# wangxb29/PPST

Hardware: AMD Instinct MI355X
Metric: 512x512 portrait swaps/sec/GPU (higher is better)
Workload: dtype bf16x3 (fp32 split into hi+lo bf16, 3 MFMA passes, fp32 accumulate); 1 GPU; simple_swapping 512x512 batch=8 per GPU, generator+encoders forward only (BASELINE configs[1]); image_parallel=1 batch per rank, no data-path collective

## Files before the change

include/ppst_hip.h:

```cpp
#ifndef PPST_HIP_H
#define PPST_HIP_H

#include <stddef.h>
#include <stdint.h>

#ifdef __cplusplus
extern "C" {
#endif

#define PPST_OK 0
#define PPST_EINVAL (-1)
#define PPST_EUNSUPPORTED (-2)
#define PPST_ENULL (-3)

enum { PPST_F32 = 0, PPST_F16 = 1, PPST_BF16 = 2, PPST_F64 = 3  };

enum { PPST_PAD_ZERO = 0, PPST_PAD_REFLECT = 1, PPST_PAD_REPLICATE = 2 };

enum { PPST_ACT_NONE = 0, PPST_ACT_LRELU = 1 , PPST_ACT_PRELU = 2 };

#define PPST_ABI_VERSION 3
int ppst_version(void);

#define PPST_ST_F32 0
#define PPST_ST_F16 1
#define PPST_ST_BF16 2

int ppst_upfirdn2d(const void* x, const void* k, void* y,
                   int major, int in_h, int in_w, int minor, int kh, int kw,
                   int up_x, int up_y, int down_x, int down_y,
                   int pad_x0, int pad_x1, int pad_y0, int pad_y1,
                   int dtype, void* stream);

int ppst_blur_nhwc(const void* x, const void* k, void* y, int B, int in_h, int in_w, int C,
                   int ksize, int pad0, int pad1, int pad_mode, int down, int s2d,
                   const void* in_scale_shift, int in_act, void* stream);
int ppst_blur_nhwc_st(const void* x, const void* k, void* y, int B, int in_h, int in_w, int C,
                      int ksize, int pad0, int pad1, int pad_mode, int down, int s2d,
                      const void* in_scale_shift, int in_act, int st , void* stream);

int ppst_fused_bias_act(const void* x, const void* b, const void* ref, void* y,
                        int64_t n, int step_b, int size_b, int act, int grad,
                        float alpha, float scale, int dtype, void* stream);

int ppst_nchw_to_nhwc(const void* x, void* y, int B, int C, int H, int W, void* stream);
int ppst_nhwc_to_nchw(const void* x, void* y, int B, int C, int H, int W, void* stream);


typedef struct ppst_conv_step {
  int32_t chan_off;
  int32_t dy, dx;
  int32_t new_chunk;
} ppst_conv_step;

int64_t ppst_conv_pack_up9_bytes(int cout, int cin);
int ppst_conv_pack_up9(const void* w, int64_t sn, int64_t sc, int64_t sy, int64_t sx, float scale, int cout, int cin,
                       void* out, void* stream);
int ppst_conv_pack_k64(const void* w, int64_t sn, int64_t sc, int64_t sy, int64_t sx, float scale, int cout, int bn,
                       const int32_t* src_c, const int32_t* src_ky, const int32_t* src_kx, int nsteps, int n_groups,
                       int precision, int dual, void* out, void* stream);
int ppst_conv_pack_dual(const void* w, int64_t sn, int64_t sc, int64_t sy, int64_t sx, float scale, int cout,
                        const int32_t* src_c, const int32_t* src_ky, const int32_t* src_kx, int nsteps, int n_groups,
                        int precision, void* out, void* stream);
int ppst_conv_pack(const void* w, int64_t sn, int64_t sc, int64_t sy, int64_t sx,
                   float scale, int cout, int bn,
                   const int32_t* src_c, const int32_t* src_ky, const int32_t* src_kx,
                   int nsteps, int n_groups, int precision, void* out, void* stream);
typedef struct ppst_pack_job {
  const void* w;
  int64_t sn, sc, sy, sx;
  const int32_t* src_c;
  const int32_t* src_ky;
  const int32_t* src_kx;
  void* out;
  int64_t total;
  int64_t block0;
  float scale;
  int32_t cout, bn, nsteps, n_groups, x3, f16, nblocks;
  int32_t dual;
} ppst_pack_job;
typedef struct ppst_upscale_job {
  const void* w;
  void* out;
  int64_t total, block0;
  float scale;
  int32_t cout, cin, nblocks;
} ppst_upscale_job;
int ppst_pack_job_blocks(int64_t total);
int ppst_conv_pack_batch(const void* jobs, int njobs, int total_blocks, void* stream);
int ppst_upscale_weight_batch(const void* jobs, int njobs, int total_blocks, void* stream);

int ppst_upscale_weight(const void* w, void* out, int cout, int cin, float scale, void* stream);
int ppst_dgrad_s2d_stack_weight(const void* w, void* out, int cout, int cin, void* stream);
int ppst_depth_to_space_st(const void* x, void* y, int B, int th, int tw, int oh, int ow, int C, int st, void* stream);

#define PPST_KSPLIT_SCRATCH_BYTES ((size_t)256 * 512 * 128 * 4)
#define PPST_KSPLIT_FLAG_WORDS 4096

typedef struct ppst_conv_args {
  const void* x;
  const void* wpack;
  const void* steps;
  void* y;
  const void* bias;
  const void* noise;
  const void* prelu;
  void* stats;
  const void* residual;
  float noise_weight;
  float out_scale;
  int32_t B, in_h, in_w, in_ld;
  int32_t out_h, out_w, out_ld, cout;
  int32_t nsteps, n_groups;
  int32_t pad_mode;
  int32_t in_off_y, in_off_x;
  int32_t out_sy, out_sx;
  int32_t act;
  int32_t precision;
  int32_t res_ld;
  int32_t tile_h, tile_w;
  int32_t halo;
  int32_t bn;
  const void* in_scale_shift;
  const void* in_prelu;
  int32_t in_c, in_act;
  int32_t flop_steps;
  int32_t tile_rows;
  int32_t a_slots;
  int32_t early_a;
  int32_t variant;
  int32_t in_presplit;
  int32_t dual_b;
  int32_t io_st;
  int32_t k64;
  const void* in_res;
  int32_t in_res_ld;
  int32_t ksplit;
  const int32_t* ksplit_starts;
  void* ksplit_scratch;
  unsigned* ksplit_flags;
  uint32_t ksplit_epoch;
} ppst_conv_args;

int ppst_conv2d_mfma(const ppst_conv_args* a, void* stream);
int64_t ppst_conv_pack_wino_bytes(int cout, int cin);
int ppst_conv_pack_wino(const void* w, int64_t sn, int64_t sc, int64_t sy, int64_t sx, float scale, int cout, int cin,
                        void* out, void* stream);
int ppst_presplit(const void* x, void* y, int64_t npix, int C, int x_ld, int y_ld, void* stream);
int ppst_has_experiments(void);
int ppst_conv2d_f32(const ppst_conv_args* a, const void* w, int64_t sn, int64_t sc, int64_t sy, int64_t sx, float wscale,
                    const int32_t* src_c, const int32_t* src_ky, const int32_t* src_kx, void* stream);
int ppst_conv_tiles(int tile_h, int tile_w, int tile_rows);

int ppst_conv1x1_small_cin(const void* x, const void* w, const void* bias, void* y,
                           int64_t npix, int cin, int in_ld, int cout, float wscale,
                           int act, void* stream);
int ppst_conv1x1_small_cin_st(const void* x, const void* w, const void* bias, void* y,
                              int64_t npix, int cin, int in_ld, int cout, float wscale,
                              int act, int y_st , void* stream);
int ppst_conv1x1_small_cout(const void* x, const void* w, const void* bias, void* y,
                            int64_t npix, int cin, int cout, float wscale, void* stream);
int ppst_conv1x1_small_cout_st(const void* x, const void* w, const void* bias, void* y,
                               int64_t npix, int cin, int cout, float wscale, int x_st , void* stream);
int ppst_torgb_apply_st(const void* x, const void* scale_shift, const void* res, int res_ld, float out_scale, const void* w,
                        const void* bias, void* y, int B, int H, int W, int cin, float wscale, int x_st, void* stream);

int ppst_in_stats(const void* x, void* partial, int B, int H, int W, int C, int ld,
                  int rep_pad, int* n_partials, void* stream);
int ppst_in_finalize(const void* partial, int n_partials, const void* style,
                     int style_ld ,
                     const void* post_bias ,
                     void* scale_shift , int B, int C, double count,
                     float eps, void* stream);
int ppst_affine_act(const void* x, const void* scale_shift, const void* res,
                    const void* res_scale_shift , void* y,
                    int B, int64_t hw, int C, int x_ld, int res_ld, int y_ld,
                    int act , const void* prelu,
                    float out_scale,
                    int res_up2_w ,
                    void* stream);
int ppst_affine_act_st(const void* x, const void* scale_shift, const void* res, const void* res_scale_shift, void* y,
                       int B, int64_t hw, int C, int x_ld, int res_ld, int y_ld, int act, const void* prelu,
                       float out_scale, int res_up2_w, int x_st, int y_st, void* stream);
int ppst_affine_act_stats(const void* x, const void* scale_shift, const void* res,
                          const void* res_scale_shift, void* y, void* partial,
                          int B, int H, int W, int C, int x_ld, int res_ld, int y_ld,
                          int act, const void* prelu, float out_scale, int rep_pad,
                          int res_up2 , void* stream);
int ppst_upsample_nearest2(const void* x, void* y, int B, int H, int W, int C, void* stream);
int ppst_upsample_nearest2_st(const void* x, void* y, int B, int H, int W, int C, int st, void* stream);

int64_t ppst_gap_gmp_ws(int B, int64_t hw, int C);
int ppst_gap_gmp(const void* x, const void* mask, void* out, void* ws, int B, int H, int W,
                 int C, int ld, void* stream);
int ppst_gap_gmp_st(const void* x, const void* mask, void* out, void* ws, int B, int H, int W,
                    int C, int ld, int x_st, void* stream);
int ppst_avgpool(const void* x, void* y, int B, int H, int W, int C, int x_ld, int f,
                 int y_ld, void* stream);
int ppst_bilinear(const void* x, void* y, int B, int H, int W, int C, int x_ld,
                  int OH, int OW, int y_ld, void* stream);
int ppst_head_tail(const void* x, const void* scale_shift, const void* prelu, void* feat, void* feat1,
                   int B, int H, int W, int C, int x_ld, int feat_ld, int feat1_ld, int P, int D, int act,
                   void* stream);
int ppst_maxpool2(const void* x, void* y, int B, int H, int W, int C, void* stream);

int ppst_linear(const void* x, const void* w, const void* bias, void* y,
                int B, int K, int N, float wscale, float bscale, int relu_in, int act,
                void* stream);
int ppst_l2norm_rows(const void* x, void* y, int B, int K, float eps, int mode, void* stream);
int ppst_lerp(const void* a, const void* b, void* y, int64_t n, float r, void* stream);
int ppst_spatial_modulation(const void* x, const void* scale, const void* bias, void* y,
                            int B, int64_t hw, int C, void* stream);
int ppst_spatial_modulation_st(const void* x, const void* scale, const void* bias, void* y,
                               int B, int64_t hw, int C, int y_st , void* stream);

int ppst_rselfcorr(const void* fea, void* out, int B, int H, int W, int C, int out_ld,
                   void* stream);
int ppst_corr_prep(const void* fea, void* out, int B, int P, int C, int ncenter, void* stream);
int ppst_unfold_rows(const void* x, void* out, int B, int H, int W, int C, int k, void* stream);
int ppst_unfold_rows_bwd(const void* g, void* dx, int B, int H, int W, int C, int k, void* stream);
int ppst_gemm_nt_f32(const void* A, const void* Bm, void* C, int batch, int M, int N, int K,
                     float alpha, void* stream);
int ppst_gemm_nn_f32(const void* A, const void* Bm, void* C, int batch, int M, int N, int K,
                     int ldb, int ldc, void* stream);
int ppst_gemm_nt_split(const void* A, const void* Bm, void* C, int batch, int M, int N, int K,
                       float alpha, int passes, void* stream);
int ppst_gemm_nn_split(const void* A, const void* Bm, void* C, int batch, int M, int N, int K,
                       int ldb, int ldc, int passes, void* stream);
int ppst_softmax_rows(void* x, int64_t rows, int cols, float div, void* stream);
int ppst_unfold_patches(const void* x, void* y, int B, int C, int H, int W, int s, void* stream);
int ppst_fold_patches(const void* x, void* y, int B, int C, int H, int W, int s, void* stream);

int ppst_resample_u8(const void* x, void* y, int B, int in_h, int in_w, int C, int out_size, int horizontal,
                     const void* bounds, const void* coef, int ksize, void* stream);
int ppst_u8_to_tensor(const void* x, void* y, int B, int H, int W, int C, float mean, float stdv, void* stream);

int ppst_tensor2im_u8(const void* x, void* y, int B, int C, int H, int W, void* stream);
int64_t ppst_guided_filter_ws(int B, int H, int W);
int ppst_guided_filter(const void* guide_u8, const void* src_u8, void* out, void* out_u8,
                       int B, int H, int W, int r, float eps, void* work, void* stream);
int ppst_guided_filter_tune(int vs1, int vs2);

int64_t ppst_smooth_local_affine_ws(int B, int H, int W);
int ppst_smooth_local_affine(const void* output, const void* input, void* result, void* model_ws, void* filtered_model,
                             int B, int H, int W, int patch_radius, int filter_radius, float sigma1, float sigma2,
                             void* stream);

int ppst_conv_wgrad_f32(const void* x, const void* dy, const void* steps, const void* chunk_start,
                        void* partial, int B, int in_h, int in_w, int in_ld, int oh, int ow,
                        int dy_ld, int cout, int nsteps, int nchunks, int splits, void* stream);
int ppst_conv_wgrad_bf16x3(const void* x, const void* dy, const void* steps, const void* chunk_start,
                           void* partial, int B, int in_h, int in_w, int in_ld, int oh, int ow,
                           int dy_ld, int cout, int nsteps, int nchunks, int splits, void* stream);
int ppst_conv_wgrad_tr(const void* x, const void* dy, const void* steps, const void* chunk_start, void* partial, void* csum,
                       int B, int in_h, int in_w, int in_ld, int oh, int ow, int dy_ld, int cout, int nsteps, int nchunks,
                       int splits, void* stream);
int ppst_conv_wgrad_tr2(const void* x, const void* dy, const void* steps, const void* chunk_start, void* partial, void* csum,
                        int B, int in_h, int in_w, int in_ld, int oh, int ow, int dy_ld, int cout, int nsteps, int nchunks,
                        int splits, int max_taps, int min_taps, int halo, int passes, void* stream);
int ppst_wgrad_scatter(const void* partial, const void* src_c, const void* src_ky, const void* src_kx,
                       void* dw, int64_t sn, int64_t sc, int64_t sy, int64_t sx, int cout, int nsteps,
                       int splits, float scale, int accumulate, const void* csum, void* db, int csum_rows, int db_accumulate,
                       void* stream);
int64_t ppst_wgrad_small_cin_ws(int64_t npix, int cin, int cout);
int ppst_wgrad_small_cin(const void* x, const void* dy, void* dw, void* ws, int64_t npix, int cin,
                         int in_ld, int cout, float scale, int accumulate, void* stream);
int64_t ppst_colsum_ws(int64_t rows, int C);
int ppst_colsum(const void* x, void* out, void* ws, int64_t rows, int C, int ld, float scale,
                int accumulate, void* stream);
int ppst_linear_wgrad(const void* dy, const void* x, void* dw, int B, int N, int K, float scale,
                      int accumulate, void* stream);
int64_t ppst_linear_dgrad_ws(int B, int N, int K);
int ppst_linear_dgrad(const void* dy, const void* w, void* dx, void* ws, int B, int N, int K, float scale,
                      void* stream);
int ppst_linear_wgrad_fused(const void* dy, const void* x, void* dw, void* db, int B, int N, int K, float scale, float bscale,
                            int accumulate, int b_accumulate, int relu_in, void* stream);
int ppst_linear_dgrad_gate(const void* dy, const void* w, void* dx, void* ws, const void* gate, int B, int N, int K, float scale,
                           void* stream);
int64_t ppst_l1_mean_ws(int64_t n);
int ppst_l1_mean(const void* a, const void* b, void* out, void* ws, int64_t n, float weight, void* stream);
int ppst_rscl_loss(const void* q, const void* k, const void* k0, const void* queue, void* out, void* ws,
                   int n, int n0, int C, int K, float nce_T, void* stream);
int ppst_lsgan(const void* pred, void* loss, void* grad, int n, float target, float weight, void* stream);
int ppst_adam_step(void* p, const void* g, void* m, void* v, int64_t n, float lr, float beta1,
                   float beta2, float eps, int step, void* stream);

int ppst_in_finalize_train(const void* partial, int n_partials, const void* style, int style_ld, const void* post_bias,
                           void* scale_shift, void* mean_rstd, int B, int C, double count, float eps, void* stream);
int ppst_dual_stats(const void* g, const void* y, const void* gate, void* partial, int B, int64_t hw, int C, int g_ld, int y_ld,
                    int gate_ld, int* n_partials, void* stream);
int ppst_in_bwd_finalize(const void* partial, int n_partials, const void* mean_rstd, const void* style, int style_ld, void* coef,
                         void* dstyle, int B, int C, double count, void* stream);
int ppst_in_bwd_apply(const void* g, const void* y, const void* gate, const void* coef, void* dx, int B, int64_t hw, int C, int g_ld,
                      int y_ld, int gate_ld, int dx_ld, int post_gate, void* stream);
int64_t ppst_prelu_bwd_ws(int64_t total_elements);
int ppst_prelu_bwd(const void* g, const void* y, const void* scale_shift, const void* res, const void* prelu, void* gpre, void* ws,
                   int B, int64_t hw, int C, int g_ld, int y_ld, int res_ld, void* stream);
int ppst_sum_partials(const void* partial, void* out, int n, float scale, void* stream);
int ppst_pad2d(const void* x, void* y, int B, int H, int W, int C, int x_ld, int py0, int py1, int px0, int px1, int mode,
               void* stream);
int ppst_pad2d_bwd(const void* dy, void* dx, int B, int H, int W, int C, int py0, int py1, int px0, int px1, int mode, void* stream);
int ppst_bilinear_bwd(const void* dy, void* dx, int B, int H, int W, int C, int dx_ld, int OH, int OW, int dy_ld, void* stream);
int ppst_avgpool_bwd(const void* dy, void* dx, int B, int H, int W, int C, int dx_ld, int f, int dy_ld, void* stream);
int ppst_gap_gmp_bwd(const void* x, const void* mask, const void* v, const void* g, void* dx, void* arg_ws , int B,
                     int64_t hw, int C, int ld, int accumulate, void* stream);
int64_t ppst_gap_gmp_multi_ws(int B, int64_t hw, int C, int heads);
int ppst_gap_gmp_multi(const void* x, const void* masks, void* out, void* ws, int B, int H, int W, int C, int ld, int nm,
                       int with_plain, int x_st, void* stream);
int ppst_gap_gmp_multi_bwd(const void* x, const void* masks, const void* v, const void* g, void* dx, void* arg_ws, int B, int64_t hw,
                           int C, int ld, int nm, int with_plain, int accumulate, int st , void* stream);
int ppst_l2norm_rows_bwd(const void* g, const void* x, void* dx, int B, int K, float eps, int mode, void* stream);
int ppst_softmax_rows_bwd(const void* p, void* g, int64_t rows, int cols, float div, void* stream);
int ppst_corr_prep_bwd(const void* g, const void* x, void* dx, int64_t rows, int C, int ncenter, float eps, void* stream);
int ppst_l1_grad(const void* a, const void* b, void* da, int64_t n, float weight, void* stream);
int ppst_rscl_loss_bwd(const void* q, const void* k, const void* k0, const void* queue, const void* gout, void* dq, int n, int n0,
                       int C, int K, float nce_T, void* stream);
int ppst_rselfcorr_bwd(const void* fea, const void* dout, void* dfea, int B, int H, int W, int C, int dout_ld, void* stream);
int ppst_scale_by(const void* x, const void* s, void* y, int64_t n, void* stream);
int64_t ppst_noise_wgrad_ws(int64_t npix);
int ppst_noise_wgrad(const void* dpre, const void* noise, void* out, void* ws, int64_t npix, int C, int ld, int accumulate, void* stream);
int ppst_upscale_weight_bwd(const void* dw4, void* dw, int cout, int cin, float scale, int accumulate, void* stream);
int ppst_space_to_depth(const void* x, void* y, int B, int H, int W, int C, int x_ld, void* stream);

int ppst_prof_enable(int on);
int ppst_prof_dropped(void);
int ppst_prof_collect(double* ms, int64_t* launches, double* flop);
int ppst_prof_detail(int idx, double* ms, double* flop, int32_t* info);
int ppst_wgrad_flop_steps(int flop_steps);

int ppst_dual_stats_st(const void* g, const void* y, const void* gate, void* partial, int B, int64_t hw, int C, int g_ld, int y_ld,
                       int gate_ld, int* n_partials, int st, void* stream);
int ppst_in_bwd_apply_st(const void* g, const void* y, const void* gate, const void* coef, void* dx, int B, int64_t hw, int C, int g_ld,
                         int y_ld, int gate_ld, int dx_ld, int post_gate, int st, void* stream);
int ppst_pad2d_st(const void* x, void* y, int B, int H, int W, int C, int x_ld, int py0, int py1, int px0, int px1, int mode, int st,
                  void* stream);
int ppst_pad2d_bwd_st(const void* dy, void* dx, int B, int H, int W, int C, int py0, int py1, int px0, int px1, int mode, int st,
                      void* stream);
int ppst_bilinear_bwd_st(const void* dy, void* dx, int B, int H, int W, int C, int dx_ld, int OH, int OW, int dy_ld, int st, void* stream);
int ppst_gap_gmp_bwd_st(const void* x, const void* mask, const void* v, const void* g, void* dx, void* arg_ws, int B, int64_t hw, int C,
                        int ld, int accumulate, int st, void* stream);
int ppst_noise_wgrad_st(const void* dpre, const void* noise, void* out, void* ws, int64_t npix, int C, int ld, int accumulate, int st,
                        void* stream);
int ppst_space_to_depth_st(const void* x, void* y, int B, int H, int W, int C, int x_ld, int st, void* stream);
int ppst_colsum_st(const void* x, void* out, void* ws, int64_t rows, int C, int ld, float scale, int accumulate, int st, void* stream);
int ppst_wgrad_small_cin_st(const void* x, const void* dy, void* dw, void* ws, int64_t npix, int cin, int in_ld, int cout, float scale,
                            int accumulate, int dy_st, void* stream);
int ppst_conv_wgrad_tr2_st(const void* x, const void* dy, const void* steps, const void* chunk_start, void* partial, void* csum, int B,
                           int in_h, int in_w, int in_ld, int oh, int ow, int dy_ld, int cout, int nsteps, int nchunks, int splits,
                           int max_taps, int min_taps, int halo, int passes, int st, void* stream);

#ifdef __cplusplus
}
#endif
#endif
```

ppst_amd/_lib.py:

```python
import ctypes
import os

import torch

HERE = os.path.dirname(os.path.abspath(__file__))
LIB_PATH = os.environ.get("PPST_HIP_LIB") or os.path.join(HERE, "libppst_hip.so")

if not os.path.exists(LIB_PATH):
    raise ImportError(
        "ppst_amd: %s is missing -- build it with `python -m ppst_amd.build` "
        "(hipcc --offload-arch=gfx950). There is no CPU fallback." % LIB_PATH)

lib = ctypes.CDLL(LIB_PATH)

vp, i32, i64, f32, f64 = ctypes.c_void_p, ctypes.c_int, ctypes.c_int64, ctypes.c_float, ctypes.c_double


class PackJob(ctypes.Structure):
    _fields_ = [("w", vp), ("sn", i64), ("sc", i64), ("sy", i64), ("sx", i64), ("src_c", vp), ("src_ky", vp), ("src_kx", vp),
                ("out", vp), ("total", i64), ("block0", i64), ("scale", f32), ("cout", i32), ("bn", i32), ("nsteps", i32),
                ("n_groups", i32), ("x3", i32), ("f16", i32), ("nblocks", i32), ("dual", i32)]


class UpscaleJob(ctypes.Structure):
    _fields_ = [("w", vp), ("out", vp), ("total", i64), ("block0", i64), ("scale", f32), ("cout", i32), ("cin", i32), ("nblocks", i32)]


class ConvArgs(ctypes.Structure):
    _fields_ = [
        ("x", vp), ("wpack", vp), ("steps", vp), ("y", vp), ("bias", vp), ("noise", vp),
        ("prelu", vp), ("stats", vp), ("residual", vp),
        ("noise_weight", f32), ("out_scale", f32),
        ("B", i32), ("in_h", i32), ("in_w", i32), ("in_ld", i32),
        ("out_h", i32), ("out_w", i32), ("out_ld", i32), ("cout", i32),
        ("nsteps", i32), ("n_groups", i32), ("pad_mode", i32),
        ("in_off_y", i32), ("in_off_x", i32), ("out_sy", i32), ("out_sx", i32),
        ("act", i32), ("precision", i32), ("res_ld", i32), ("tile_h", i32), ("tile_w", i32),
        ("halo", i32), ("bn", i32), ("in_scale_shift", vp), ("in_prelu", vp), ("in_c", i32), ("in_act", i32),
        ("flop_steps", i32), ("tile_rows", i32), ("a_slots", i32), ("early_a", i32), ("variant", i32), ("in_presplit", i32), ("dual_b", i32), ("io_st", i32), ("k64", i32),
        ("in_res", vp), ("in_res_ld", i32), ("ksplit", i32), ("ksplit_starts", vp),
        ("ksplit_scratch", vp), ("ksplit_flags", vp), ("ksplit_epoch", ctypes.c_uint32),
    ]


_SIGS = {
    "ppst_version": (i32, []),
    "ppst_guided_filter_tune": (i32, [i32, i32]),
    "ppst_upfirdn2d": (i32, [vp, vp, vp] + [i32] * 14 + [i32, vp]),
    "ppst_blur_nhwc": (i32, [vp, vp, vp] + [i32] * 10 + [vp, i32, vp]),
    "ppst_blur_nhwc_st": (i32, [vp, vp, vp] + [i32] * 10 + [vp, i32, i32, vp]),
    "ppst_fused_bias_act": (i32, [vp, vp, vp, vp, i64, i32, i32, i32, i32, f32, f32, i32, vp]),
    "ppst_nchw_to_nhwc": (i32, [vp, vp, i32, i32, i32, i32, vp]),
    "ppst_nhwc_to_nchw": (i32, [vp, vp, i32, i32, i32, i32, vp]),
    "ppst_conv_pack": (i32, [vp, i64, i64, i64, i64, f32, i32, i32, vp, vp, vp, i32, i32, i32, vp, vp]),
    "ppst_conv_pack_k64": (i32, [vp, i64, i64, i64, i64, f32, i32, i32, vp, vp, vp, i32, i32, i32, i32, vp, vp]),
    "ppst_conv_pack_up9_bytes": (i64, [i32, i32]),
    "ppst_conv_pack_up9": (i32, [vp, i64, i64, i64, i64, f32, i32, i32, vp, vp]),
    "ppst_conv_pack_wino_bytes": (i64, [i32, i32]),
    "ppst_conv_pack_wino": (i32, [vp, i64, i64, i64, i64, f32, i32, i32, vp, vp]),
    "ppst_conv_pack_dual": (i32, [vp, i64, i64, i64, i64, f32, i32, vp, vp, vp, i32, i32, i32, vp, vp]),
    "ppst_upscale_weight": (i32, [vp, vp, i32, i32, f32, vp]),
    "ppst_dgrad_s2d_stack_weight": (i32, [vp, vp, i32, i32, vp]),
    "ppst_depth_to_space_st": (i32, [vp, vp, i32, i32, i32, i32, i32, i32, i32, vp]),
    "ppst_pack_job_blocks": (i32, [i64]),
    "ppst_conv_pack_batch": (i32, [vp, i32, i32, vp]),
    "ppst_upscale_weight_batch": (i32, [vp, i32, i32, vp]),
    "ppst_conv2d_mfma": (i32, [ctypes.POINTER(ConvArgs), vp]),
    "ppst_has_experiments": (i32, []),
    "ppst_presplit": (i32, [vp, vp, i64, i32, i32, i32, vp]),
    "ppst_conv2d_f32": (i32, [ctypes.POINTER(ConvArgs), vp, i64, i64, i64, i64, f32, vp, vp, vp, vp]),
    "ppst_conv_tiles": (i32, [i32, i32, i32]),
    "ppst_conv1x1_small_cin": (i32, [vp, vp, vp, vp, i64, i32, i32, i32, f32, i32, vp]),
    "ppst_conv1x1_small_cin_st": (i32, [vp, vp, vp, vp, i64, i32, i32, i32, f32, i32, i32, vp]),
    "ppst_conv1x1_small_cout": (i32, [vp, vp, vp, vp, i64, i32, i32, f32, vp]),
    "ppst_conv1x1_small_cout_st": (i32, [vp, vp, vp, vp, i64, i32, i32, f32, i32, vp]),
    "ppst_torgb_apply_st": (i32, [vp, vp, vp, i32, f32, vp, vp, vp, i32, i32, i32, i32, f32, i32, vp]),
    "ppst_in_stats": (i32, [vp, vp, i32, i32, i32, i32, i32, i32, ctypes.POINTER(i32), vp]),
    "ppst_in_finalize": (i32, [vp, i32, vp, i32, vp, vp, i32, i32, f64, f32, vp]),
    "ppst_affine_act": (i32, [vp, vp, vp, vp, vp, i32, i64, i32, i32, i32, i32, i32, vp, f32, i32, vp]),
    "ppst_affine_act_st": (i32, [vp, vp, vp, vp, vp, i32, i64, i32, i32, i32, i32, i32, vp, f32, i32, i32, i32, vp]),
    "ppst_affine_act_stats": (i32, [vp, vp, vp, vp, vp, vp, i32, i32, i32, i32, i32, i32, i32, i32, vp, f32, i32, i32, vp]),
    "ppst_upsample_nearest2": (i32, [vp, vp, i32, i32, i32, i32, vp]),
    "ppst_upsample_nearest2_st": (i32, [vp, vp, i32, i32, i32, i32, i32, vp]),
    "ppst_gap_gmp_ws": (i64, [i32, i64, i32]),
    "ppst_gap_gmp": (i32, [vp, vp, vp, vp, i32, i32, i32, i32, i32, vp]),
    "ppst_gap_gmp_st": (i32, [vp, vp, vp, vp, i32, i32, i32, i32, i32, i32, vp]),
    "ppst_avgpool": (i32, [vp, vp, i32, i32, i32, i32, i32, i32, i32, vp]),
    "ppst_bilinear": (i32, [vp, vp, i32, i32, i32, i32, i32, i32, i32, i32, vp]),
    "ppst_head_tail": (i32, [vp, vp, vp, vp, vp] + [i32] * 10 + [vp]),
    "ppst_maxpool2": (i32, [vp, vp, i32, i32, i32, i32, vp]),
    "ppst_linear": (i32, [vp, vp, vp, vp, i32, i32, i32, f32, f32, i32, i32, vp]),
    "ppst_l2norm_rows": (i32, [vp, vp, i32, i32, f32, i32, vp]),
    "ppst_lerp": (i32, [vp, vp, vp, i64, f32, vp]),
    "ppst_spatial_modulation": (i32, [vp, vp, vp, vp, i32, i64, i32, vp]),
    "ppst_spatial_modulation_st": (i32, [vp, vp, vp, vp, i32, i64, i32, i32, vp]),
    "ppst_rselfcorr": (i32, [vp, vp, i32, i32, i32, i32, i32, vp]),
    "ppst_corr_prep": (i32, [vp, vp, i32, i32, i32, i32, vp]),
    "ppst_gemm_nt_f32": (i32, [vp, vp, vp, i32, i32, i32, i32, f32, vp]),
    "ppst_gemm_nn_f32": (i32, [vp, vp, vp, i32, i32, i32, i32, i32, i32, vp]),
    "ppst_unfold_rows": (i32, [vp, vp, i32, i32, i32, i32, i32, vp]),
    "ppst_unfold_rows_bwd": (i32, [vp, vp, i32, i32, i32, i32, i32, vp]),
    "ppst_gemm_nt_split": (i32, [vp, vp, vp, i32, i32, i32, i32, f32, i32, vp]),
    "ppst_gemm_nn_split": (i32, [vp, vp, vp, i32, i32, i32, i32, i32, i32, i32, vp]),
    "ppst_softmax_rows": (i32, [vp, i64, i32, f32, vp]),
    "ppst_unfold_patches": (i32, [vp, vp, i32, i32, i32, i32, i32, vp]),
    "ppst_fold_patches": (i32, [vp, vp, i32, i32, i32, i32, i32, vp]),
    "ppst_tensor2im_u8": (i32, [vp, vp, i32, i32, i32, i32, vp]),
    "ppst_resample_u8": (i32, [vp, vp, i32, i32, i32, i32, i32, i32, vp, vp, i32, vp]),
    "ppst_u8_to_tensor": (i32, [vp, vp, i32, i32, i32, i32, f32, f32, vp]),
    "ppst_guided_filter_ws": (i64, [i32, i32, i32]),
    "ppst_guided_filter": (i32, [vp, vp, vp, vp, i32, i32, i32, i32, f32, vp, vp]),
    "ppst_smooth_local_affine_ws": (i64, [i32, i32, i32]),
    "ppst_smooth_local_affine": (i32, [vp, vp, vp, vp, vp, i32, i32, i32, i32, i32, f32, f32, vp]),
    "ppst_conv_wgrad_f32": (i32, [vp, vp, vp, vp, vp] + [i32] * 11 + [vp]),
    "ppst_conv_wgrad_bf16x3": (i32, [vp, vp, vp, vp, vp] + [i32] * 11 + [vp]),
    "ppst_conv_wgrad_tr": (i32, [vp, vp, vp, vp, vp, vp, i32, i32, i32, i32, i32, i32, i32, i32, i32, i32, i32, vp]),
    "ppst_conv_wgrad_tr2": (i32, [vp, vp, vp, vp, vp, vp, i32, i32, i32, i32, i32, i32, i32, i32, i32, i32, i32, i32, i32, i32, i32, vp]),
    "ppst_wgrad_scatter": (i32, [vp, vp, vp, vp, vp, i64, i64, i64, i64, i32, i32, i32, f32, i32, vp, vp, i32, i32, vp]),
    "ppst_wgrad_small_cin_ws": (i64, [i64, i32, i32]),
    "ppst_wgrad_small_cin": (i32, [vp, vp, vp, vp, i64, i32, i32, i32, f32, i32, vp]),
    "ppst_colsum_ws": (i64, [i64, i32]),
    "ppst_colsum": (i32, [vp, vp, vp, i64, i32, i32, f32, i32, vp]),
    "ppst_linear_wgrad": (i32, [vp, vp, vp, i32, i32, i32, f32, i32, vp]),
    "ppst_linear_dgrad_ws": (i64, [i32, i32, i32]),
    "ppst_linear_dgrad": (i32, [vp, vp, vp, vp, i32, i32, i32, f32, vp]),
    "ppst_linear_wgrad_fused": (i32, [vp, vp, vp, vp, i32, i32, i32, f32, f32, i32, i32, i32, vp]),
    "ppst_linear_dgrad_gate": (i32, [vp, vp, vp, vp, vp, i32, i32, i32, f32, vp]),
    "ppst_lsgan": (i32, [vp, vp, vp, i32, f32, f32, vp]),
    "ppst_l1_mean_ws": (i64, [i64]),
    "ppst_l1_mean": (i32, [vp, vp, vp, vp, i64, f32, vp]),
    "ppst_rscl_loss": (i32, [vp, vp, vp, vp, vp, vp, i32, i32, i32, i32, f32, vp]),
    "ppst_adam_step": (i32, [vp, vp, vp, vp, i64, f32, f32, f32, f32, i32, vp]),
    "ppst_in_finalize_train": (i32, [vp, i32, vp, i32, vp, vp, vp, i32, i32, f64, f32, vp]),
    "ppst_dual_stats": (i32, [vp, vp, vp, vp, i32, i64, i32, i32, i32, i32, ctypes.POINTER(i32), vp]),
    "ppst_in_bwd_finalize": (i32, [vp, i32, vp, vp, i32, vp, vp, i32, i32, f64, vp]),
    "ppst_in_bwd_apply": (i32, [vp, vp, vp, vp, vp, i32, i64, i32, i32, i32, i32, i32, i32, vp]),
    "ppst_prelu_bwd_ws": (i64, [i64]),
    "ppst_prelu_bwd": (i32, [vp, vp, vp, vp, vp, vp, vp, i32, i64, i32, i32, i32, i32, vp]),
    "ppst_sum_partials": (i32, [vp, vp, i32, f32, vp]),
    "ppst_pad2d": (i32, [vp, vp] + [i32] * 10 + [vp]),
    "ppst_pad2d_bwd": (i32, [vp, vp] + [i32] * 9 + [vp]),
    "ppst_bilinear_bwd": (i32, [vp, vp] + [i32] * 8 + [vp]),
    "ppst_avgpool_bwd": (i32, [vp, vp] + [i32] * 7 + [vp]),
    "ppst_gap_gmp_bwd": (i32, [vp, vp, vp, vp, vp, vp, i32, i64, i32, i32, i32, vp]),
    "ppst_gap_gmp_multi_ws": (i64, [i32, i64, i32, i32]),
    "ppst_gap_gmp_multi": (i32, [vp, vp, vp, vp, i32, i32, i32, i32, i32, i32, i32, i32, vp]),
    "ppst_gap_gmp_multi_bwd": (i32, [vp, vp, vp, vp, vp, vp, i32, i64, i32, i32, i32, i32, i32, i32, vp]),
    "ppst_gap_gmp_bwd_st": (i32, [vp, vp, vp, vp, vp, vp, i32, i64, i32, i32, i32, i32, vp]),
    "ppst_dual_stats_st": (i32, [vp, vp, vp, vp, i32, i64, i32, i32, i32, i32, ctypes.POINTER(i32), i32, vp]),
    "ppst_in_bwd_apply_st": (i32, [vp, vp, vp, vp, vp, i32, i64, i32, i32, i32, i32, i32, i32, i32, vp]),
    "ppst_pad2d_st": (i32, [vp, vp] + [i32] * 11 + [vp]),
    "ppst_pad2d_bwd_st": (i32, [vp, vp] + [i32] * 10 + [vp]),
    "ppst_bilinear_bwd_st": (i32, [vp, vp] + [i32] * 9 + [vp]),
    "ppst_noise_wgrad_st": (i32, [vp, vp, vp, vp, i64, i32, i32, i32, i32, vp]),
    "ppst_space_to_depth_st": (i32, [vp, vp, i32, i32, i32, i32, i32, i32, vp]),
    "ppst_colsum_st": (i32, [vp, vp, vp, i64, i32, i32, f32, i32, i32, vp]),
    "ppst_wgrad_small_cin_st": (i32, [vp, vp, vp, vp, i64, i32, i32, i32, f32, i32, i32, vp]),
    "ppst_conv_wgrad_tr2_st": (i32, [vp, vp, vp, vp, vp, vp] + [i32] * 16 + [vp]),
    "ppst_l2norm_rows_bwd": (i32, [vp, vp, vp, i32, i32, f32, i32, vp]),
    "ppst_softmax_rows_bwd": (i32, [vp, vp, i64, i32, f32, vp]),
    "ppst_corr_prep_bwd": (i32, [vp, vp, vp, i64, i32, i32, f32, vp]),
    "ppst_l1_grad": (i32, [vp, vp, vp, i64, f32, vp]),
    "ppst_scale_by": (i32, [vp, vp, vp, i64, vp]),
    "ppst_rscl_loss_bwd": (i32, [vp, vp, vp, vp, vp, vp, i32, i32, i32, i32, f32, vp]),
    "ppst_rselfcorr_bwd": (i32, [vp, vp, vp, i32, i32, i32, i32, i32, vp]),
    "ppst_noise_wgrad_ws": (i64, [i64]),
    "ppst_noise_wgrad": (i32, [vp, vp, vp, vp, i64, i32, i32, i32, vp]),
    "ppst_upscale_weight_bwd": (i32, [vp, vp, i32, i32, f32, i32, vp]),
    "ppst_space_to_depth": (i32, [vp, vp, i32, i32, i32, i32, i32, vp]),
    "ppst_prof_enable": (i32, [i32]),
    "ppst_prof_dropped": (i32, []),
    "ppst_wgrad_flop_steps": (i32, [i32]),
    "ppst_prof_collect": (i32, [ctypes.POINTER(f64), ctypes.POINTER(i64), ctypes.POINTER(f64)]),
    "ppst_prof_detail": (i32, [i32, ctypes.POINTER(f64), ctypes.POINTER(f64), ctypes.POINTER(i32)]),
}

for _name, (_res, _args) in _SIGS.items():
    _fn = getattr(lib, _name)
    _fn.restype = _res
    _fn.argtypes = _args

ABI_VERSION = 3
if lib.ppst_version() != ABI_VERSION:
    raise ImportError("ppst_amd: %s reports ABI revision %d, this binding is written for %d -- rebuild the library "
                      "(python -m ppst_amd.build)" % (LIB_PATH, lib.ppst_version(), ABI_VERSION))

_ERR = {-1: "PPST_EINVAL (bad size / flag combination)", -2: "PPST_EUNSUPPORTED", -3: "PPST_ENULL"}


def check(rc, what):
    if rc != 0:
        raise RuntimeError("%s failed: %s" % (what, _ERR.get(rc, "hipError_t %d" % rc)))


def exported_symbols():
    return sorted(_SIGS)
```

ppst_amd/build.py:

```python
import os
import subprocess
import sys
from concurrent.futures import ThreadPoolExecutor

HERE = os.path.dirname(os.path.abspath(__file__))
CSRC = os.path.join(HERE, "csrc")
OBJ = os.path.join(HERE, "csrc", "_obj")
LIB = os.path.join(HERE, "libppst_hip.so")
EXPERIMENTS = os.environ.get("PPST_EXPERIMENTS") == "1"
SOURCES = ["upfirdn2d.hip", "fused_bias_act.hip", "elementwise.hip", "linear.hip", "conv_mfma.hip", "conv_mfma2.hip", "conv1x1.hip", "conv_wino.hip", "conv_f32.hip",
           "corr.hip", "guided_filter.hip", "train.hip", "train_g.hip", "imageio.hip", "smooth_filter.hip"] + (["conv_ksplit.hip"] if EXPERIMENTS else [])
FLAGS = ["--offload-arch=gfx950", "-O3", "-fPIC", "-std=c++17", "-Wno-unused-result"] + (["-DPPST_EXPERIMENTS"] if EXPERIMENTS else [])
FILE_FLAGS = {"conv_wino.hip": ["-fno-slp-vectorize"]}
MODE_STAMP = os.path.join(HERE, ".libmode")


def _hipcc():
    for c in (os.environ.get("HIPCC"), "/opt/rocm/bin/hipcc", "hipcc"):
        if c and (os.path.isabs(c) and os.path.exists(c) or not os.path.isabs(c)):
            return c
    return "hipcc"


HEADERS = [os.path.join(CSRC, "common.h"), os.path.join(CSRC, "rscl_common.h"), os.path.join(HERE, "..", "include", "ppst_hip.h")]


def _stale(target, deps):
    return not os.path.exists(target) or any(os.path.getmtime(d) > os.path.getmtime(target) for d in deps)


def _mode():
    return "experiments" if EXPERIMENTS else "production"


def _lib_flavour():
    try:
        return open(MODE_STAMP).read().strip()
    except OSError:
        pass
    if not os.path.exists(LIB):
        return None
    try:
        return "experiments" if b"conv_ksplit_kernel" in open(LIB, "rb").read() else "production"
    except OSError:
        return None


def _mode_changed():
    have = _lib_flavour()
    if have is None:
        return os.path.exists(LIB)
    return have != _mode()


def needs_build():
    return (_mode_changed() or _stale(LIB, [os.path.join(CSRC, s) for s in SOURCES] + HEADERS) or
            any(_stale(os.path.join(OBJ, s.replace(".hip", ".o")), [os.path.join(CSRC, s)]) for s in SOURCES if os.path.isdir(OBJ)))


def build(force=False, verbose=True):
    if not force and not needs_build():
        return LIB
    os.makedirs(OBJ, exist_ok=True)
    force = force or _mode_changed()
    hipcc = _hipcc()

    def cc(src):
        obj = os.path.join(OBJ, src.replace(".hip", ".o"))
        if not force and not _stale(obj, [os.path.join(CSRC, src)] + HEADERS):
            return obj
        cmd = [hipcc] + FLAGS + FILE_FLAGS.get(src, []) + ["-c", os.path.join(CSRC, src), "-o", obj]
        r = subprocess.run(cmd, capture_output=True, text=True)
        if r.returncode != 0:
            raise RuntimeError("hipcc failed for %s:\n%s" % (src, r.stderr))
        return obj

    order = sorted(SOURCES, key=lambda f: 0 if f.startswith("conv") else 1)
    with ThreadPoolExecutor(max_workers=8) as ex:
        objs = dict(zip(order, ex.map(cc, order)))
    cmd = [hipcc, "--offload-arch=gfx950", "-shared", "-fPIC", "-o", LIB] + [objs[s_] for s_ in SOURCES]
    r = subprocess.run(cmd, capture_output=True, text=True)
    if r.returncode != 0:
        raise RuntimeError("link failed:\n%s" % r.stderr)
    with open(MODE_STAMP, "w") as f:
        f.write(_mode() + "\n")
    if verbose:
        print("built", LIB, "(%s)" % _mode())
    return LIB


if __name__ == "__main__":
    build(force="--force" in sys.argv)
```

ppst_amd/csrc/conv1x1.hip:

```cpp
#include "common.h"

struct C1Args {
  const float* x;
  const unsigned char* wpack;
  const int4* steps;
  float* y;
  const float* bias;
  const float* noise;
  const float* prelu;
  float* stats;
  const float* residual;
  float noise_weight, out_scale;
  int B, hw, in_ld, out_ld, cout, nsteps, act, res_ld, n_tiles, tiles;
  int in_h, in_w, out_h, out_w, tiles_x, pad_mode;
  const float* in_ss;
  const float* in_prelu;
  int in_c, in_act;
  const float* in_res;
  int in_res_ld;
};

#define C1_GROUP 8
#define C1_BLOB 8192

typedef _Float16 __attribute__((ext_vector_type(8))) c1_half8;
template <int PREC>
__device__ __forceinline__ void c1_cvt(float v, unsigned short& h, unsigned short& l) {
  if (PREC == 0) split_bf16(v, h, l);
  else if (PREC == 3) { h = __builtin_bit_cast(unsigned short, (_Float16)v); l = 0; }
  else { h = f2bf(v); l = 0; }
}
template <int PREC>
__device__ __forceinline__ void c1_cvt8(const float (&v)[8], bf16x8& hi, bf16x8& lo) {
  if (PREC == 3) {
#pragma unroll
    for (int j = 0; j < 8; ++j) {
      unsigned short h, l;
      c1_cvt<PREC>(v[j], h, l);
      hi[j] = (short)h;
      lo[j] = (short)l;
    }
    return;
  }
  uint2 h0, l0 = make_uint2(0u, 0u), h1, l1 = make_uint2(0u, 0u);
  if (PREC == 0) {
    split_bf16x4(make_float4(v[0], v[1], v[2], v[3]), h0, l0);
    split_bf16x4(make_float4(v[4], v[5], v[6], v[7]), h1, l1);
  } else {
    h0 = f2bf_x4(make_float4(v[0], v[1], v[2], v[3]));
    h1 = f2bf_x4(make_float4(v[4], v[5], v[6], v[7]));
  }
  hi = __builtin_bit_cast(bf16x8, make_uint4(h0.x, h0.y, h1.x, h1.y));
  lo = __builtin_bit_cast(bf16x8, make_uint4(l0.x, l0.y, l1.x, l1.y));
}
template <int IOS>
__device__ __forceinline__ void c1_unpack8(float4 r, float (&v)[8]) {
  const float4 a = st_unpack4<IOS>(make_uint2(__float_as_uint(r.x), __float_as_uint(r.y)));
  const float4 b = st_unpack4<IOS>(make_uint2(__float_as_uint(r.z), __float_as_uint(r.w)));
  v[0] = a.x; v[1] = a.y; v[2] = a.z; v[3] = a.w; v[4] = b.x; v[5] = b.y; v[6] = b.z; v[7] = b.w;
}
template <int PREC>
__device__ __forceinline__ f32x4 c1_mfma(bf16x8 bh, bf16x8 bl, bf16x8 xh, bf16x8 xl, f32x4 acc) {
  if (PREC == 0) {
    acc = __builtin_amdgcn_mfma_f32_16x16x32_bf16(bh, xl, acc, 0, 0, 0);
    acc = __builtin_amdgcn_mfma_f32_16x16x32_bf16(bl, xh, acc, 0, 0, 0);
    return __builtin_amdgcn_mfma_f32_16x16x32_bf16(bh, xh, acc, 0, 0, 0);
  }
  if (PREC == 3) return __builtin_amdgcn_mfma_f32_16x16x32_f16(__builtin_bit_cast(c1_half8, bh), __builtin_bit_cast(c1_half8, xh), acc, 0, 0, 0);
  return __builtin_amdgcn_mfma_f32_16x16x32_bf16(bh, xh, acc, 0, 0, 0);
}

__device__ __forceinline__ int c1_pad(int i, int n, int mode) {
  if (mode == PPST_PAD_REFLECT) {
    if (i < 0) i = -i;
    if (i >= n) i = 2 * (n - 1) - i;
  }
  return i < 0 ? 0 : (i >= n ? n - 1 : i);
}

template <int MT, int NT, bool TAPS, bool SPEC = true, int IOS = PPST_ST_F32>
__device__ __forceinline__ void c1_epilogue(const C1Args& a, f32x4 (&acc)[MT][NT], float (&red)[8][NT > 4 ? 128 : 64][2], int b, int mblk,
                                            int ntile, int pbase, int oy0, int ox, int tid, int wave, int r16, int g) {
  const int act = a.act & 0xff;
  const bool res_after = (a.act >> 8) & 1;
  const float slope = (act == PPST_ACT_PRELU && a.prelu) ? a.prelu[0] : 0.f;
  float4 s1[NT], s2[NT];
#pragma unroll
  for (int nt = 0; nt < NT; ++nt) { s1[nt] = make_float4(0.f, 0.f, 0.f, 0.f); s2[nt] = s1[nt]; }
  const int64_t img = (int64_t)b * (TAPS ? a.out_h * a.out_w : a.hw);
  constexpr int ES = IOS == PPST_ST_F32 ? 4 : 2;
  unsigned char* const yb = (unsigned char*)a.y + img * a.out_ld * ES;
  const float* const nzb = a.noise ? a.noise + img : nullptr;
  const unsigned char* const rb = a.residual ? (const unsigned char*)a.residual + img * a.res_ld * ES : nullptr;
  const int nbase = ntile * (NT > 4 ? 128 : 64) + g * 4;
  float nzv[MT];
  float4 bva[NT];
  const __amdgpu_buffer_rsrc_t nrs = __builtin_amdgcn_make_buffer_rsrc((void*)(nzb ? (const void*)nzb : (const void*)yb), 0,
                                                                       nzb ? (TAPS ? a.out_h * a.out_w : a.hw) * 4 : 0, 0x00020000);
#pragma unroll
  for (int mt = 0; mt < MT; ++mt) {
    const int p = pbase + mt * 16 + r16;
    const bool ok = TAPS ? (oy0 + mt < a.out_h && ox < a.out_w) : p < a.hw;
    nzv[mt] = a.noise_weight * __builtin_bit_cast(float, __builtin_amdgcn_raw_buffer_load_b32(
                                   nrs, ok ? (TAPS ? (oy0 + mt) * a.out_w + ox : p) * 4 : (int)0x80000000, 0, 0));
  }
#pragma unroll
  for (int nt = 0; nt < NT; ++nt)
    bva[nt] = __builtin_bit_cast(float4, __builtin_amdgcn_raw_buffer_load_b128(__builtin_amdgcn_make_buffer_rsrc((void*)(a.bias ? (const void*)a.bias : (const void*)a.y), 0, a.bias ? a.cout * 4 : 0, 0x00020000), (nbase + nt * 16) * 4, 0, 0));
  auto epi_passes = [&](auto act_c, auto res_c) {
#pragma clang fp contract(off)
    const int ACT = act_c.value, RES = res_c.value;
#pragma unroll
  for (int mt = 0; mt < MT; ++mt) {
    const int p = pbase + mt * 16 + r16;
    if (TAPS ? (oy0 + mt >= a.out_h || ox >= a.out_w) : p >= a.hw) continue;
    const int pin = TAPS ? (oy0 + mt) * a.out_w + ox : p;
    const int yo = pin * a.out_ld, ro = pin * a.res_ld;
    const float nz = nzv[mt];
#pragma unroll
    for (int nt = 0; nt < NT; ++nt) {
      const int n0 = nbase + nt * 16;
      if (n0 >= a.cout) continue;
      float4 rv = make_float4(0.f, 0.f, 0.f, 0.f);
      const float4 bv = bva[nt];
      if (RES) rv = st_ld4<IOS>(rb, ro + n0);
      float o[4] = {acc[mt][nt][0] + bv.x + nz, acc[mt][nt][1] + bv.y + nz, acc[mt][nt][2] + bv.z + nz, acc[mt][nt][3] + bv.w + nz};
      const float r4[4] = {rv.x, rv.y, rv.z, rv.w};
#pragma unroll
      for (int c = 0; c < 4; ++c) {
        float t = o[c];
        if (RES == 1) t += r4[c];
        if (ACT == PPST_ACT_LRELU) t = (t > 0.f ? t : t * 0.2f) * 1.41421356237309515f;
        else if (ACT == PPST_ACT_PRELU) t = t >= 0.f ? t : t * slope;
        if (RES == 2) t += r4[c];
        o[c] = t * a.out_scale;
      }
      st_st4<IOS>(yb, yo + n0, make_float4(o[0], o[1], o[2], o[3]));
      s1[nt].x += o[0]; s1[nt].y += o[1]; s1[nt].z += o[2]; s1[nt].w += o[3];
      s2[nt].x += o[0] * o[0]; s2[nt].y += o[1] * o[1]; s2[nt].z += o[2] * o[2]; s2[nt].w += o[3] * o[3];
    }
  }
  };
  {
    const int resm = a.residual ? (res_after ? 2 : 1) : 0;
#define EPI_GO(A_)                                                                                    \
  do {                                                                                                \
    if (resm == 0) epi_passes(EpiC<A_>{}, EpiC<0>{});                                                 \
    else if (resm == 1) epi_passes(EpiC<A_>{}, EpiC<1>{});                                            \
    else epi_passes(EpiC<A_>{}, EpiC<2>{});                                                           \
  } while (0)
    if (!SPEC) epi_passes(EpiR{act}, EpiR{resm});
    else if (act == PPST_ACT_LRELU) EPI_GO(PPST_ACT_LRELU);
    else if (act == PPST_ACT_PRELU) EPI_GO(PPST_ACT_PRELU);
    else EPI_GO(PPST_ACT_NONE);
#undef EPI_GO
  }
  if (a.stats) {
#pragma unroll
    for (int nt = 0; nt < NT; ++nt) {
      float4 u = s1[nt], w = s2[nt];
      float* uv[8] = {&u.x, &u.y, &u.z, &u.w, &w.x, &w.y, &w.z, &w.w};
#pragma unroll
      for (int q = 0; q < 8; ++q) {
        float t = *uv[q];
        t += __builtin_bit_cast(float, __builtin_amdgcn_mov_dpp(__builtin_bit_cast(int, t), 0xB1, 0xf, 0xf, true));
        t += __builtin_bit_cast(float, __builtin_amdgcn_mov_dpp(__builtin_bit_cast(int, t), 0x4E, 0xf, 0xf, true));
        t += __builtin_bit_cast(float, __builtin_amdgcn_mov_dpp(__builtin_bit_cast(int, t), 0x141, 0xf, 0xf, true));
        t += __builtin_bit_cast(float, __builtin_amdgcn_mov_dpp(__builtin_bit_cast(int, t), 0x140, 0xf, 0xf, true));
        *uv[q] = t;
      }
      if (r16 == 0) {
        float* r = &red[wave][nt * 16 + g * 4][0];
        r[0] = u.x; r[1] = w.x; r[2] = u.y; r[3] = w.y; r[4] = u.z; r[5] = w.z; r[6] = u.w; r[7] = w.w;
      }
    }
    __syncthreads();
    if (tid < (NT > 4 ? 128 : 64)) {
      const int n = ntile * (NT > 4 ? 128 : 64) + tid;
      if (n < a.cout) {
        float t0 = 0.f, t1 = 0.f;
#pragma unroll
        for (int wv = 0; wv < 8; ++wv) { t0 += red[wv][tid][0]; t1 += red[wv][tid][1]; }
        float* o = a.stats + (((int64_t)b * a.tiles + mblk) * a.cout + n) * 2;
        o[0] = t0;
        o[1] = t1;
      }
    }
  }
}

template <int INSS, bool TAPS = false, int NT_ = 4, int PREC = 0, int IOS = PPST_ST_F32>
__global__ __launch_bounds__(512, 4) void conv1x1_stream_kernel(C1Args a) {
  constexpr int MT = 2, NT = NT_;
  constexpr bool X3 = PREC == 0;
  static_assert(IOS == PPST_ST_F32 || IOS == (PREC == 3 ? PPST_ST_F16 : PREC == 1 ? PPST_ST_BF16 : -1), "half storage: single-pass modes");
  constexpr int ES = IOS == PPST_ST_F32 ? 4 : 2;
  constexpr int BLOB1 = X3 ? C1_BLOB : C1_BLOB / 2;
  __shared__ uint4 sB[C1_GROUP * BLOB1 / 16];
  __shared__ float red[8][64][2];

  const int nwg = gridDim.x;
  int wid;
  {
    int id = blockIdx.x, q = nwg >> 3, r = nwg & 7, xcd = id & 7;
    wid = (xcd < r ? xcd * (q + 1) : r * (q + 1) + (xcd - r) * q) + (id >> 3);
  }
  const int ntile = wid % a.n_tiles;
  int mblk = wid / a.n_tiles;
  const int b = mblk / a.tiles;
  mblk -= b * a.tiles;
  const int tid = threadIdx.x, lane = tid & 63, wave = __builtin_amdgcn_readfirstlane(tid >> 6);
  const int r16 = lane & 15, g = lane >> 4;
  const int pbase = mblk * 256 + wave * 32;
  const int tyi = TAPS ? mblk / a.tiles_x : 0, txi = TAPS ? mblk - tyi * a.tiles_x : 0;
  const int oy0 = tyi * 16 + wave * 2, ox = txi * 16 + r16;
  const unsigned char* xb = (const unsigned char*)a.x + (int64_t)b * (TAPS ? a.in_h * a.in_w : a.hw) * a.in_ld * ES;
  const unsigned char* wblob = a.wpack + (int64_t)ntile * a.nsteps * BLOB1;
#if defined(__HIP_DEVICE_COMPILE__)
  typedef const __attribute__((address_space(4))) int4* StepPtr;
#else
  typedef const int4* StepPtr;
#endif
  StepPtr steps = (StepPtr)a.steps;

  int64_t aoff[MT];
  bool pok[MT];
#pragma unroll
  for (int mt = 0; mt < MT; ++mt) {
    const int p = pbase + mt * 16 + r16;
    pok[mt] = TAPS ? true : p < a.hw;
    aoff[mt] = TAPS ? 0 : (int64_t)(pok[mt] ? p : 0) * a.in_ld + g * 8;
  }
  const float in_slope = (INSS && a.in_act == PPST_ACT_PRELU && a.in_prelu) ? a.in_prelu[0] : 0.f;
  auto in_act = [&](float t) -> float {
    if (a.in_act == PPST_ACT_LRELU) return (t > 0.f ? t : t * 0.2f) * 1.41421356237309515f;
    if (a.in_act == PPST_ACT_PRELU) return t >= 0.f ? t : t * in_slope;
    return t;
  };

  f32x4 acc[MT][NT];
#pragma unroll
  for (int i = 0; i < MT; ++i)
#pragma unroll
    for (int j = 0; j < NT; ++j) acc[i][j] = (f32x4){0.f, 0.f, 0.f, 0.f};

  float4 raw[MT][2], ss[4];
  float4 rres[INSS == 2 ? MT : 1][2];
  auto a_load = [&](int4 d) {
    const int chan = d.x;
    if (TAPS) {
      int ix = ox + d.z;
      bool xok = ix >= 0 && ix < a.in_w;
      ix = c1_pad(ix, a.in_w, a.pad_mode);
#pragma unroll
      for (int mt = 0; mt < MT; ++mt) {
        int iy = oy0 + mt + d.y;
        const bool yok = iy >= 0 && iy < a.in_h;
        iy = c1_pad(iy, a.in_h, a.pad_mode);
        pok[mt] = a.pad_mode != PPST_PAD_ZERO || (xok && yok);
        aoff[mt] = ((int64_t)iy * a.in_w + ix) * a.in_ld + g * 8;
      }
    }
#pragma unroll
    for (int mt = 0; mt < MT; ++mt) {
      const float4* p = (const float4*)(xb + (aoff[mt] + chan) * ES);
      raw[mt][0] = p[0];
      if (IOS == PPST_ST_F32) raw[mt][1] = p[1];
      if (INSS == 2) {
        const int pp = pbase + mt * 16 + r16;
        const float4* q = (const float4*)(a.in_res + ((int64_t)b * a.hw + (pok[mt] ? pp : 0)) * a.in_res_ld + g * 8 + chan);
        rres[mt][0] = q[0];
        rres[mt][1] = q[1];
      }
    }
    if (INSS) {
      const float4* q = (const float4*)(a.in_ss + ((int64_t)b * a.in_c + chan + g * 8) * 2);
      ss[0] = q[0]; ss[1] = q[1]; ss[2] = q[2]; ss[3] = q[3];
    }
  };
  a_load(steps[0]);

  for (int s0 = 0; s0 < a.nsteps; s0 += C1_GROUP) {
    const int ng = a.nsteps - s0 < C1_GROUP ? a.nsteps - s0 : C1_GROUP;
    if (s0) __syncthreads();
    for (int i = tid; i < ng * (BLOB1 / 16); i += 512) sB[i] = ((const uint4*)(wblob + (int64_t)s0 * BLOB1))[i];
    __syncthreads();
    for (int sl = 0; sl < ng; ++sl) {
      const int s = s0 + sl;
      bf16x8 ah[MT], al[MT];
      bool vok[MT];
#pragma unroll
      for (int mt = 0; mt < MT; ++mt) vok[mt] = pok[mt];
#pragma unroll
      for (int mt = 0; mt < MT; ++mt) {
        if (IOS != PPST_ST_F32 && !INSS) {
          const float4 z = vok[mt] ? raw[mt][0] : make_float4(0.f, 0.f, 0.f, 0.f);
          ah[mt] = __builtin_bit_cast(bf16x8, z);
          al[mt] = ah[mt];
          continue;
        }
        float v[8] = {raw[mt][0].x, raw[mt][0].y, raw[mt][0].z, raw[mt][0].w, raw[mt][1].x, raw[mt][1].y, raw[mt][1].z, raw[mt][1].w};
        if (IOS != PPST_ST_F32) c1_unpack8<IOS>(raw[mt][0], v);
        if (INSS) {
          const float sc[8] = {ss[0].x, ss[0].z, ss[1].x, ss[1].z, ss[2].x, ss[2].z, ss[3].x, ss[3].z};
          const float sh[8] = {ss[0].y, ss[0].w, ss[1].y, ss[1].w, ss[2].y, ss[2].w, ss[3].y, ss[3].w};
#pragma unroll
          for (int j = 0; j < 8; ++j) {
            float t = sc[j] * v[j] + sh[j];
            if (INSS == 2) {
              const float4 r4 = rres[mt][j >> 2];
              t += (j & 3) == 0 ? r4.x : (j & 3) == 1 ? r4.y : (j & 3) == 2 ? r4.z : r4.w;
            }
            v[j] = in_act(t);
          }
        }
#pragma unroll
        for (int j = 0; j < 8; ++j)
          if (!vok[mt]) v[j] = 0.f;
        c1_cvt8<PREC>(v, ah[mt], al[mt]);
      }
      if (s + 1 < a.nsteps) a_load(steps[s + 1]);
      const unsigned char* bs = (const unsigned char*)sB + sl * BLOB1 + g * 1024 + r16 * 16;
#pragma unroll
      for (int nt = 0; nt < NT; ++nt) {
        const bf16x8 bh = *(const bf16x8*)(bs + nt * 256);
        bf16x8 bl = bh;
        if (X3) bl = *(const bf16x8*)(bs + nt * 256 + 4096);
#pragma unroll
        for (int mt = 0; mt < MT; ++mt) acc[mt][nt] = c1_mfma<PREC>(bh, bl, ah[mt], al[mt], acc[mt][nt]);
      }
    }
  }

  c1_epilogue<MT, NT, TAPS, X3, IOS>(a, acc, red, b, mblk, ntile, pbase, oy0, ox, tid, wave, r16, g);
}

#define C3_GROUP 9
template <int CTRL>
__device__ __forceinline__ bf16x8 c3_shift(bf16x8 edge, bf16x8 centre) {
  typedef int __attribute__((ext_vector_type(4))) i4;
  const i4 e = __builtin_bit_cast(i4, edge), c = __builtin_bit_cast(i4, centre);
  i4 r;
#pragma unroll
  for (int i = 0; i < 4; ++i) r[i] = __builtin_amdgcn_update_dpp(e[i], c[i], CTRL, 0xf, 0xf, false);
  return __builtin_bit_cast(bf16x8, r);
}

template <bool INSS, int NT_, int PREC = 0, int IOS = PPST_ST_F32>
__global__ __launch_bounds__(512, NT_ > 4 ? 2 : 4) void conv3x3_direct_kernel(C1Args a) {
  constexpr int MT = 2, NT = NT_;
  constexpr bool X3 = PREC == 0;
  static_assert(IOS == PPST_ST_F32 || IOS == (PREC == 3 ? PPST_ST_F16 : PREC == 1 ? PPST_ST_BF16 : -1), "half storage: single-pass modes");
  constexpr int ES = IOS == PPST_ST_F32 ? 4 : 2;
  constexpr int PSTR = (NT > 4 ? 128 : 64) * 16;
  constexpr int BLOB = (X3 ? 8 : 4) * PSTR;
  __shared__ uint4 sB[C3_GROUP * BLOB / 16];
  __shared__ float red[8][NT > 4 ? 128 : 64][2];
  const int tid = threadIdx.x, lane = tid & 63, wave = __builtin_amdgcn_readfirstlane(tid >> 6);
  const int r16 = lane & 15, g = lane >> 4;
  const int total = a.B * a.tiles * a.n_tiles;
  const int per = (total + (int)gridDim.x - 1) / (int)gridDim.x;
  const int w_beg = blockIdx.x * per, w_end = w_beg + per < total ? w_beg + per : total;
  const int nchunks = a.nsteps / 9;
  const bool keep_b = nchunks == 1 && a.n_tiles == 1;
  for (int wid = w_beg; wid < w_end; ++wid) {
  const int ntile = wid % a.n_tiles;
  int mblk = wid / a.n_tiles;
  const int b = mblk / a.tiles;
  mblk -= b * a.tiles;
  const int tyi = mblk / a.tiles_x, txi = mblk - tyi * a.tiles_x;
  const int oy0 = tyi * 16 + wave * 2, ox = txi * 16 + r16;
  const unsigned char* xb = (const unsigned char*)a.x + (int64_t)b * a.in_h * a.in_w * a.in_ld * ES;
  const unsigned char* wblob = a.wpack + (int64_t)ntile * a.nsteps * BLOB;
  if (wid > w_beg) __syncthreads();
#if defined(__HIP_DEVICE_COMPILE__)
  typedef const __attribute__((address_space(4))) int4* StepPtr;
#else
  typedef const int4* StepPtr;
#endif
  StepPtr steps = (StepPtr)a.steps;
  const float in_slope = (INSS && a.in_act == PPST_ACT_PRELU && a.in_prelu) ? a.in_prelu[0] : 0.f;
  auto in_act = [&](float t) -> float {
    if (a.in_act == PPST_ACT_LRELU) return (t > 0.f ? t : t * 0.2f) * 1.41421356237309515f;
    if (a.in_act == PPST_ACT_PRELU) return t >= 0.f ? t : t * in_slope;
    return t;
  };
  const int xe_raw = r16 == 0 ? ox - 1 : (r16 == 15 ? ox + 1 : ox);
  const bool cx_ok = ox < a.in_w, ex_ok = xe_raw >= 0 && xe_raw < a.in_w;
  const int cx = c1_pad(ox, a.in_w, a.pad_mode), ex = c1_pad(xe_raw, a.in_w, a.pad_mode);

  f32x4 acc[MT][NT];
#pragma unroll
  for (int i = 0; i < MT; ++i)
#pragma unroll
    for (int j = 0; j < NT; ++j) acc[i][j] = (f32x4){0.f, 0.f, 0.f, 0.f};

  float4 rawc[2], rawe[2], ss[4];
  bool okc = false, oke = false;
  auto row_load = [&](int chan, int r) {
    int iy = oy0 - 1 + r;
    const bool yok = iy >= 0 && iy < a.in_h;
    iy = c1_pad(iy, a.in_h, a.pad_mode);
    okc = a.pad_mode != PPST_PAD_ZERO || (yok && cx_ok);
    oke = a.pad_mode != PPST_PAD_ZERO || (yok && ex_ok);
    const float4* pc = (const float4*)(xb + (((int64_t)iy * a.in_w + cx) * a.in_ld + chan + g * 8) * ES);
    const float4* pe = (const float4*)(xb + (((int64_t)iy * a.in_w + ex) * a.in_ld + chan + g * 8) * ES);
    rawc[0] = pc[0];
    rawe[0] = pe[0];
    if (IOS == PPST_ST_F32) { rawc[1] = pc[1]; rawe[1] = pe[1]; }
  };
  auto ss_load = [&](int chan) {
    if (INSS) {
      const float4* q = (const float4*)(a.in_ss + ((int64_t)b * a.in_c + chan + g * 8) * 2);
      ss[0] = q[0]; ss[1] = q[1]; ss[2] = q[2]; ss[3] = q[3];
    }
  };
  auto convert = [&](const float4 (&raw)[2], bool ok, bf16x8& hi, bf16x8& lo) {
    if (IOS != PPST_ST_F32 && !INSS) {
      hi = __builtin_bit_cast(bf16x8, ok ? raw[0] : make_float4(0.f, 0.f, 0.f, 0.f));
      lo = hi;
      return;
    }
    float v[8] = {raw[0].x, raw[0].y, raw[0].z, raw[0].w, raw[1].x, raw[1].y, raw[1].z, raw[1].w};
    if (IOS != PPST_ST_F32) c1_unpack8<IOS>(raw[0], v);
    if (INSS) {
      const float sc[8] = {ss[0].x, ss[0].z, ss[1].x, ss[1].z, ss[2].x, ss[2].z, ss[3].x, ss[3].z};
      const float sh[8] = {ss[0].y, ss[0].w, ss[1].y, ss[1].w, ss[2].y, ss[2].w, ss[3].y, ss[3].w};
#pragma unroll
      for (int j = 0; j < 8; ++j) v[j] = in_act(sc[j] * v[j] + sh[j]);
    }
#pragma unroll
    for (int j = 0; j < 8; ++j)
      if (!ok) v[j] = 0.f;
    c1_cvt8<PREC>(v, hi, lo);
  };

  int chan = steps[0].x;
  ss_load(chan);
  row_load(chan, 0);
  for (int c = 0; c < nchunks; ++c) {
    if (!keep_b || wid == w_beg) {
      if (c) __syncthreads();
      for (int i = tid; i < C3_GROUP * (BLOB / 16); i += 512) sB[i] = ((const uint4*)(wblob + (int64_t)c * C3_GROUP * BLOB))[i];
      __syncthreads();
    }
    const int chan_next = c + 1 < nchunks ? steps[(c + 1) * 9].x : chan;
#pragma unroll
    for (int r = 0; r < 4; ++r) {
      bf16x8 ch, cl, eh, el;
      convert(rawc, okc, ch, cl);
      convert(rawe, oke, eh, el);
      if (r < 3) row_load(chan, r + 1);
      else if (c + 1 < nchunks) { ss_load(chan_next); row_load(chan_next, 0); }
#pragma unroll
      for (int dxi = 0; dxi < 3; ++dxi) {
        const bf16x8 fh = dxi == 0 ? c3_shift<0x111>(eh, ch) : (dxi == 1 ? ch : c3_shift<0x101>(eh, ch));
        const bf16x8 fl = dxi == 0 ? c3_shift<0x111>(el, cl) : (dxi == 1 ? cl : c3_shift<0x101>(el, cl));
#pragma unroll
        for (int mt = 0; mt < MT; ++mt) {
          const int dyi = r - mt;
          if (dyi < 0 || dyi > 2) continue;
          const unsigned char* bs = (const unsigned char*)sB + (dyi * 3 + dxi) * BLOB + g * PSTR + r16 * 16;
#pragma unroll
          for (int nt = 0; nt < NT; ++nt) {
            const bf16x8 bh = *(const bf16x8*)(bs + nt * 256);
            bf16x8 bl = bh;
            if (X3) bl = *(const bf16x8*)(bs + nt * 256 + 4 * PSTR);
            acc[mt][nt] = c1_mfma<PREC>(bh, bl, fh, fl, acc[mt][nt]);
          }
        }
        __builtin_amdgcn_sched_barrier(0);
      }
    }
    chan = chan_next;
  }
  c1_epilogue<MT, NT, true, (X3 && NT <= 4), IOS>(a, acc, red, b, mblk, ntile, 0, oy0, ox, tid, wave, r16, g);
  }
}

static inline int64_t blocks_of(const ppst_conv_args* a, int tiles, int n_tiles) { return (int64_t)a->B * tiles * n_tiles; }
int ppst_conv1x1_stream_launch(const ppst_conv_args* a, int n_tiles, int tiles, hipStream_t st) {
  C1Args k;
  k.x = (const float*)a->x; k.wpack = (const unsigned char*)a->wpack; k.steps = (const int4*)a->steps; k.y = (float*)a->y;
  k.bias = (const float*)a->bias; k.noise = (const float*)a->noise; k.prelu = (const float*)a->prelu;
  k.stats = (float*)a->stats; k.residual = (const float*)a->residual;
  k.noise_weight = a->noise_weight; k.out_scale = a->out_scale;
  k.B = a->B; k.hw = a->out_h * a->out_w; k.in_ld = a->in_ld; k.out_ld = a->out_ld; k.cout = a->cout; k.nsteps = a->nsteps;
  k.act = a->act; k.res_ld = a->res_ld; k.n_tiles = n_tiles; k.tiles = tiles;
  k.in_ss = (const float*)a->in_scale_shift; k.in_prelu = (const float*)a->in_prelu; k.in_c = a->in_c; k.in_act = a->in_act;
  k.in_res = (const float*)a->in_res; k.in_res_ld = a->in_res_ld;
  if ((int64_t)tiles * 256 < k.hw) return PPST_EINVAL;
  if (k.in_res) {
    PPST_LAUNCH((conv1x1_stream_kernel<2, false, 4, 0, PPST_ST_F32>), dim3((unsigned)blocks_of(a, tiles, n_tiles)), dim3(512), 0, st, k);
    return PPST_LAUNCH_CHECK();
  }
  const int64_t blocks = (int64_t)a->B * tiles * n_tiles;
  if (blocks > 0x7fffffff) return PPST_EINVAL;
#define LS(PREC_, IOS_)                                                                                               \
  do {                                                                                                                \
    if (k.in_ss) PPST_LAUNCH((conv1x1_stream_kernel<1, false, 4, PREC_, IOS_>), dim3((unsigned)blocks), dim3(512), 0, st, k);   \
    else PPST_LAUNCH((conv1x1_stream_kernel<0, false, 4, PREC_, IOS_>), dim3((unsigned)blocks), dim3(512), 0, st, k);          \
  } while (0)
  if (a->precision == 1) { if (a->io_st) LS(1, PPST_ST_BF16); else LS(1, PPST_ST_F32); }
  else if (a->precision == 3) { if (a->io_st) LS(3, PPST_ST_F16); else LS(3, PPST_ST_F32); }
  else LS(0, PPST_ST_F32);
#undef LS
  return PPST_LAUNCH_CHECK();
}

int ppst_conv_direct_launch(const ppst_conv_args* a, int n_tiles, int tiles_y, int tiles_x, hipStream_t st) {
  C1Args k;
  k.x = (const float*)a->x; k.wpack = (const unsigned char*)a->wpack; k.steps = (const int4*)a->steps; k.y = (float*)a->y;
  k.bias = (const float*)a->bias; k.noise = (const float*)a->noise; k.prelu = (const float*)a->prelu;
  k.stats = (float*)a->stats; k.residual = (const float*)a->residual;
  k.noise_weight = a->noise_weight; k.out_scale = a->out_scale;
  k.B = a->B; k.hw = a->out_h * a->out_w; k.in_ld = a->in_ld; k.out_ld = a->out_ld; k.cout = a->cout; k.nsteps = a->nsteps;
  k.act = a->act; k.res_ld = a->res_ld; k.n_tiles = n_tiles; k.tiles = tiles_y * tiles_x;
  k.in_ss = (const float*)a->in_scale_shift; k.in_prelu = (const float*)a->in_prelu; k.in_c = a->in_c; k.in_act = a->in_act;
  k.in_h = a->in_h; k.in_w = a->in_w; k.out_h = a->out_h; k.out_w = a->out_w; k.tiles_x = tiles_x; k.pad_mode = a->pad_mode;
  const int64_t blocks = (int64_t)a->B * k.tiles * n_tiles;
  if (blocks > 0x7fffffff) return PPST_EINVAL;
  const bool nt2 = a->cout <= 32;
#define LD(INSS_, PREC_, IOS_)                                                                                       \
  do {                                                                                                               \
    if (nt2) PPST_LAUNCH((conv1x1_stream_kernel<INSS_, true, 2, PREC_, IOS_>), dim3((unsigned)blocks), dim3(512), 0, st, k);       \
    else PPST_LAUNCH((conv1x1_stream_kernel<INSS_, true, 4, PREC_, IOS_>), dim3((unsigned)blocks), dim3(512), 0, st, k);           \
  } while (0)
#define LDP(PREC_, IOS_) do { if (k.in_ss) LD(1, PREC_, IOS_); else LD(0, PREC_, IOS_); } while (0)
  if (a->precision == 1) { if (a->io_st) LDP(1, PPST_ST_BF16); else LDP(1, PPST_ST_F32); }
  else if (a->precision == 3) { if (a->io_st) LDP(3, PPST_ST_F16); else LDP(3, PPST_ST_F32); }
  else LDP(0, PPST_ST_F32);
#undef LDP
#undef LD
  return PPST_LAUNCH_CHECK();
}

int ppst_conv3x3_direct_launch(const ppst_conv_args* a, int n_tiles, int tiles_y, int tiles_x, hipStream_t st) {
  if (a->nsteps % 9) return PPST_EINVAL;
  C1Args k;
  k.x = (const float*)a->x; k.wpack = (const unsigned char*)a->wpack; k.steps = (const int4*)a->steps; k.y = (float*)a->y;
  k.bias = (const float*)a->bias; k.noise = (const float*)a->noise; k.prelu = (const float*)a->prelu;
  k.stats = (float*)a->stats; k.residual = (const float*)a->residual;
  k.noise_weight = a->noise_weight; k.out_scale = a->out_scale;
  k.B = a->B; k.hw = a->out_h * a->out_w; k.in_ld = a->in_ld; k.out_ld = a->out_ld; k.cout = a->cout; k.nsteps = a->nsteps;
  k.act = a->act; k.res_ld = a->res_ld; k.n_tiles = n_tiles; k.tiles = tiles_y * tiles_x;
  k.in_ss = (const float*)a->in_scale_shift; k.in_prelu = (const float*)a->in_prelu; k.in_c = a->in_c; k.in_act = a->in_act;
  k.in_h = a->in_h; k.in_w = a->in_w; k.out_h = a->out_h; k.out_w = a->out_w; k.tiles_x = tiles_x; k.pad_mode = a->pad_mode;
  int64_t blocks = (int64_t)a->B * k.tiles * n_tiles;
  if (blocks > 0x7fffffff) return PPST_EINVAL;
  if (a->nsteps == 9 && n_tiles == 1 && blocks > 512) blocks = 512;
  const bool nt2 = a->cout <= 32, nt8 = a->bn == 128;
#define LD3(INSS_, PREC_, IOS_)                                                                                      \
  do {                                                                                                               \
    if (nt8 && PREC_ == 0) PPST_LAUNCH((conv3x3_direct_kernel<INSS_, 8, 0>), dim3((unsigned)blocks), dim3(512), 0, st, k);   \
    else if (nt8) return PPST_EUNSUPPORTED;                                                                          \
    else if (nt2) PPST_LAUNCH((conv3x3_direct_kernel<INSS_, 2, PREC_, IOS_>), dim3((unsigned)blocks), dim3(512), 0, st, k); \
    else PPST_LAUNCH((conv3x3_direct_kernel<INSS_, 4, PREC_, IOS_>), dim3((unsigned)blocks), dim3(512), 0, st, k);          \
  } while (0)
#define LD3P(PREC_, IOS_) do { if (k.in_ss) LD3(true, PREC_, IOS_); else LD3(false, PREC_, IOS_); } while (0)
  if (a->precision == 1) { if (a->io_st) LD3P(1, PPST_ST_BF16); else LD3P(1, PPST_ST_F32); }
  else if (a->precision == 3) { if (a->io_st) LD3P(3, PPST_ST_F16); else LD3P(3, PPST_ST_F32); }
  else LD3P(0, PPST_ST_F32);
#undef LD3P
#undef LD3
  return PPST_LAUNCH_CHECK();
}
```

ppst_amd/networks/base_network.py:

```python
import math

import torch
from torch import nn

from .. import ops, weights

SQRT2 = math.sqrt(2.0)
INV_SQRT2 = 1.0 / SQRT2


class _Node(nn.Module):
    """parameter container (no behaviour)."""


def to_nhwc(x):
    if x.dim() != 4:
        raise RuntimeError("expected a 4-D NCHW tensor")
    v = x.permute(0, 2, 3, 1)
    if v.is_contiguous():
        ops._chk(v, "input")
        return v
    return ops.nchw_to_nhwc(x)


def as_nchw(x_nhwc):
    return x_nhwc.permute(0, 3, 1, 2)


class BaseNetwork(nn.Module):
    prefix = ""

    @staticmethod
    def modify_commandline_options(parser, is_train):
        return parser

    def __init__(self, opt=None, size=512, seed=0):
        super().__init__()
        self.opt = opt
        self._flat = {}
        self._cache = {}
        specs = [s for s in weights.param_specs(size=size) if s[0].startswith(self.prefix)]
        for name, shape, kind, aux in specs:
            parts = name[len(self.prefix):].split(".")
            node = self
            for part in parts[:-1]:
                if part not in node._modules:
                    node.add_module(part, _Node())
                node = node._modules[part]
            t = weights._draw(name, shape, kind, aux, seed, 0.0, 0.0)
            if kind in (weights.BLUR3, weights.BLUR4, weights.UP4):
                node.register_buffer(parts[-1], t)
            else:
                node.register_parameter(parts[-1], nn.Parameter(t, requires_grad=False))

    def p(self, name):
        t = self._flat.get(name)
        if t is None:
            node = self
            parts = name.split(".")
            for part in parts[:-1]:
                node = node._modules[part]
            t = node._parameters.get(parts[-1])
            if t is None:
                t = node._buffers[parts[-1]]
            self._flat[name] = t
        return t

    def _apply(self, fn, *a, **k):
        self._flat.clear()
        self._cache.clear()
        return super()._apply(fn, *a, **k)

    def load_state_dict(self, *a, **k):
        self._flat.clear()
        self._cache.clear()
        return super().load_state_dict(*a, **k)

    def cached(self, key, params, build):
        ver = tuple((id(t), t._version, t.data_ptr()) for t in params) + (ops.PRECISION["value"],)
        hit = self._cache.get(key)
        if hit is not None and hit[0] == ver:
            return hit[1]
        val = build()
        self._cache[key] = (ver, val)
        return val

    def plan(self, wname, kind="conv", scale=1.0):
        w = self.p(wname)
        return self.cached(("plan", wname, kind), [w], lambda: ops.ConvPlan(w, kind=kind, scale=scale))

    def refresh_plans(self):
        plans, keep = [], {}
        for key, (ver, val) in self._cache.items():
            if isinstance(key, tuple) and key and key[0] == "plan" and isinstance(val, ops.ConvPlan) and val.precision != 2 \
                    and val.wparam.data_ptr() == self.p(key[1]).data_ptr():
                plans.append(val)
                keep[key] = (ver, val)
        self._cache.clear()
        if not plans:
            return
        sig = tuple((id(pl), tuple(sorted(map(str, pl._packs)))) for pl in plans)
        hit = self.__dict__.get("_repack")
        if hit is not None and hit[0] == sig:
            ops.run_repack(hit[1])
        else:
            self.__dict__["_repack"] = (sig, ops.repack_plans(plans), plans)
        self._cache.update(keep)

    def print_architecture(self, verbose=False):
        n = sum(p.numel() for p in self.parameters())
        print("[Network %s] Total number of parameters : %.3f M" % (type(self).__name__, n / 1e6))

    def from_rgb(self, x, p, out_dtype=torch.float32):
        w = self.p(p + "Conv.weight")
        return ops.conv1x1_small_cin(x, w, self.p(p + "Act.bias"), 1.0 / math.sqrt(w.shape[1]), ops.ACT_LRELU, out_dtype=out_dtype)

    def _norm_act(self, y, st, count, act_bias=None, act=ops.ACT_NONE, **kw):
        ss = ops.in_finalize(st, count, post_bias=act_bias)
        return ops.affine_act(y, ss, act=act, **kw), ss

    def res_block(self, x, p, blur_pad_mode, norm):
        B, H, W, cin = x.shape
        k = self.p(p + "conv2.Blur.kernel")
        ks = k.shape[0]
        w1, w2, ws = self.p(p + "conv1.Conv.weight"), self.p(p + "conv2.Conv.weight"), self.p(p + "skip.Conv.weight")
        sc1 = 1.0 / math.sqrt(cin * 9)
        scs = 1.0 / math.sqrt(cin)
        conv_pad = ops.PAD_REFLECT if blur_pad_mode == ops.PAD_REFLECT else ops.PAD_ZERO
        pad_c = (ks - 2) + 2
        pad_s = (ks - 2) + 0
        xs, _ = ops.blur_nhwc(x, self.p(p + "skip.Blur.kernel"), (pad_s + 1) // 2, pad_s // 2, ops.PAD_ZERO, down=2)
        if not norm:
            y1 = self.plan(p + "conv1.Conv.weight", scale=sc1)(x, bias=self.p(p + "conv1.Act.bias"), act=ops.ACT_LRELU,
                                                                pad_mode=conv_pad)
            skip = self.plan(p + "skip.Conv.weight", scale=scs)(xs)
            xb, bhw = ops.blur_nhwc(y1, k, (pad_c + 1) // 2, pad_c // 2, blur_pad_mode, s2d=True)
            ohw = ((bhw[0] - 3) // 2 + 1, (bhw[1] - 3) // 2 + 1)
            return self.plan(p + "conv2.Conv.weight", "s2d", sc1)(
                xb, bias=self.p(p + "conv2.Act.bias"), act=ops.ACT_LRELU, residual=skip, res_after_act=True,
                out_scale=INV_SQRT2, out_hw=ohw)
        y1, st1 = self.plan(p + "conv1.Conv.weight", scale=sc1)(x, stats=True, pad_mode=conv_pad)
        ss1 = ops.in_finalize(st1, H * W, post_bias=self.p(p + "conv1.Act.bias"))
        ys, sts = self.plan(p + "skip.Conv.weight", scale=scs)(xs, stats=True)
        xb, bhw = ops.blur_nhwc(y1, k, (pad_c + 1) // 2, pad_c // 2, blur_pad_mode, s2d=True, in_ss=ss1, in_act=ops.ACT_LRELU)
        ohw = ((bhw[0] - 3) // 2 + 1, (bhw[1] - 3) // 2 + 1)
        y2, st2 = self.plan(p + "conv2.Conv.weight", "s2d", sc1)(xb, stats=True, out_hw=ohw)
        cnt = ohw[0] * ohw[1]
        ss_s = ops.in_finalize(sts, cnt)
        ss2 = ops.in_finalize(st2, cnt, post_bias=self.p(p + "conv2.Act.bias"))
        return ops.affine_act(y2, ss2, res=ys, res_scale_shift=ss_s, act=ops.ACT_LRELU, out_scale=INV_SQRT2)
```

ppst_amd/ops.py:

```python
import ctypes
import math
import os
import threading

import torch

from . import _lib
from ._lib import lib, check

PAD_ZERO, PAD_REFLECT, PAD_REPLICATE = 0, 1, 2
ACT_NONE, ACT_LRELU, ACT_PRELU = 0, 1, 2
RES_BEFORE_ACT = 1 << 8

PRECISION = {"value": 0}
TILE_ROWS = {"value": 16}
CONV_VARIANT = {"value": 2}
DUAL_CONVT = {"value": True, "min_blocks": 32}
UP9 = {"value": True, "min_blocks": 64, "min_fill": 0.85}
DIRECT_MAX = {"cout": 64, "nsteps": 40, "cout3x3": 64}
WGRAD_SPLIT = {"blocks": 1024, "min_tiles": 4}
WGRAD_X3 = {"value": True}
STREAM_1X1 = {"value": True}
KSPLIT = {"value": os.environ.get("PPST_KSPLIT", "1") != "0", "max_blocks": 256, "min_steps": 16, "variants": (0, 2, 10)}
KSPLIT_SCRATCH_BYTES = 256 * 512 * 128 * 4
KSPLIT_FLAG_WORDS = 4096
KSPLIT_128 = {"value": False, "min_blocks": 32}
TALL_TILE_128 = {"value": False, "min_blocks": 32}
TALL_TILE_SINGLE = {"value": True, "min_blocks": 64}
K64 = {"value": True}
TILE24_128 = {"value": False, "min_blocks": 32, "max_waste": 0.04}
TWO_BLOCK_128 = {"value": False}
TWO_BLOCK_8ROW = {"value": False, "min_blocks": 64}
BATCH_AWARE = {"value": False, "fill": 192}


class batch_aware:

    def __enter__(self):
        self.prev = BATCH_AWARE["value"]
        BATCH_AWARE["value"] = True

    def __exit__(self, *exc):
        BATCH_AWARE["value"] = self.prev
WINO = {"value": True, "min_blocks": 16, "fill": 0, "ksplit_fill": 64}
FUSE_TAIL = {"value": os.environ.get("PPST_FUSE_TAIL", "1") != "0", "torgb": os.environ.get("PPST_FUSE_TORGB", "0") == "1"}
FAT_MIN_BLOCKS = 32


EXPERIMENTS = bool(lib.ppst_has_experiments())


def _need_experiments(what):
    if not EXPERIMENTS:
        raise RuntimeError("%s is an experiment kernel: rebuild the library with PPST_EXPERIMENTS=1 (python -m ppst_amd.build)" % what)


def set_precision(p):
    assert p in (0, 1, 2, 3, 4)
    if p == 4:
        _need_experiments("precision 4 (two-pass fp16)")
    PRECISION["value"] = p


_raw_stream = getattr(torch._C, "_cuda_getCurrentRawStream", None)
_cur_device = getattr(torch._C, "_cuda_getDevice", None)


def _stream():
    if _raw_stream is not None and _cur_device is not None:
        return ctypes.c_void_p(_raw_stream(_cur_device()))
    return ctypes.c_void_p(torch.cuda.current_stream().cuda_stream)


def _chk(t, name="tensor"):
    if t is None:
        return
    if not isinstance(t, torch.Tensor) or not t.is_cuda:
        raise RuntimeError("%s must be a CUDA (HIP) tensor" % name)
    if t.dtype != torch.float32:
        raise RuntimeError("%s must be float32, got %s" % (name, t.dtype))


def _p(t):
    return None if t is None else ctypes.c_void_p(t.data_ptr())


_ST = {torch.float32: 0, torch.float16: 1, torch.bfloat16: 2}
HALF_STORE = {"value": os.environ.get("PPST_HALF_STORE", "1") != "0"}


def act_dtype():
    if HALF_STORE["value"] and not torch.is_grad_enabled():
        return {1: torch.bfloat16, 3: torch.float16}.get(PRECISION["value"], torch.float32)
    return torch.float32


TRAIN_HALF = {"value": os.environ.get("PPST_TRAIN_HALF", "1") != "0"}


def train_dtype():
    return torch.bfloat16 if (TRAIN_HALF["value"] and PRECISION["value"] == 1) else torch.float32


def _chk_act(t, name="activation"):
    if t is None:
        return
    if not isinstance(t, torch.Tensor) or not t.is_cuda:
        raise RuntimeError("%s must be a CUDA (HIP) tensor" % name)
    if t.dtype not in _ST:
        raise RuntimeError("%s must be float32, float16 or bfloat16, got %s" % (name, t.dtype))


def _nhwc_ld(t, name="activation", half_ok=False):
    if half_ok:
        _chk_act(t, name)
    else:
        _chk(t, name)
    B, H, W, C = t.shape
    ld = t.stride(2)
    if t.stride(3) != 1 or t.stride(1) != W * ld or (B > 1 and t.stride(0) != H * W * ld):
        raise RuntimeError("%s must be NHWC-contiguous (or a channel slice of one)" % name)
    return ld


def empty_nhwc(B, H, W, C, like):
    return torch.empty((B, H, W, C), device=like.device, dtype=torch.float32)


def nchw_to_nhwc(x):
    _chk(x, "x")
    x = x.contiguous()
    B, C, H, W = x.shape
    y = torch.empty((B, H, W, C), device=x.device, dtype=torch.float32)
    check(lib.ppst_nchw_to_nhwc(_p(x), _p(y), B, C, H, W, _stream()), "ppst_nchw_to_nhwc")
    return y


def nhwc_to_nchw(x):
    ld = _nhwc_ld(x)
    B, H, W, C = x.shape
    if ld != C:
        raise RuntimeError("nhwc_to_nchw needs a dense tensor")
    y = torch.empty((B, C, H, W), device=x.device, dtype=torch.float32)
    check(lib.ppst_nhwc_to_nchw(_p(x), _p(y), B, C, H, W, _stream()), "ppst_nhwc_to_nchw")
    return y


_DT_F64 = 3


def _chk_op(t, name):
    if t is None:
        return
    if not isinstance(t, torch.Tensor) or not t.is_cuda:
        raise RuntimeError("%s must be a CUDA (HIP) tensor" % name)
    if t.dtype not in _ST and t.dtype != torch.float64:
        raise RuntimeError("%s must be float32, float16, bfloat16 or float64, got %s" % (name, t.dtype))


def upfirdn2d_raw(x4, kernel, up_x, up_y, down_x, down_y, px0, px1, py0, py1):
    _chk_op(x4, "input")
    _chk_op(kernel, "kernel")
    x4 = x4.contiguous()
    f64 = x4.dtype == torch.float64
    kernel = (kernel.double() if f64 else kernel.float()).contiguous()
    major, in_h, in_w, minor = x4.shape
    kh, kw = kernel.shape
    out_h = (in_h * up_y + py0 + py1 - kh + down_y) // down_y
    out_w = (in_w * up_x + px0 + px1 - kw + down_x) // down_x
    y = torch.empty((major, out_h, out_w, minor), device=x4.device, dtype=x4.dtype)
    check(lib.ppst_upfirdn2d(_p(x4), _p(kernel), _p(y), major, in_h, in_w, minor, kh, kw, up_x, up_y, down_x, down_y,
                             px0, px1, py0, py1, _DT_F64 if f64 else _ST[x4.dtype], _stream()), "ppst_upfirdn2d")
    return y


def blur_nhwc(x, kernel, pad0, pad1, pad_mode=PAD_ZERO, down=1, s2d=False, in_ss=None, in_act=ACT_NONE):
    ld = _nhwc_ld(x, half_ok=True)
    B, H, W, C = x.shape
    if ld != C:
        raise RuntimeError("blur_nhwc needs a dense tensor")
    _chk(kernel, "kernel")
    ks = kernel.shape[0]
    oh = (H + pad0 + pad1 - ks + down) // down
    ow = (W + pad0 + pad1 - ks + down) // down
    if s2d:
        y = torch.empty((B, (oh + 1) // 2, (ow + 1) // 2, 4 * C), device=x.device, dtype=x.dtype)
    else:
        y = torch.empty((B, oh, ow, C), device=x.device, dtype=x.dtype)
    _chk(in_ss, "in_ss")
    check(lib.ppst_blur_nhwc_st(_p(x), _p(kernel.contiguous()), _p(y), B, H, W, C, ks, pad0, pad1, pad_mode, down,
                                1 if s2d else 0, _p(in_ss), in_act, _ST[x.dtype], _stream()), "ppst_blur_nhwc")
    return y, (oh, ow)


def fused_bias_act_raw(x, b, ref, act, grad, alpha, scale):
    _chk_op(x, "input")
    x = x.contiguous()
    b = None if (b is None or b.numel() == 0) else b.to(x.dtype).contiguous()
    ref = None if (ref is None or ref.numel() == 0) else ref.to(x.dtype).contiguous()
    _chk_op(b, "bias")
    _chk_op(ref, "refer")
    y = torch.empty_like(x)
    step_b = 1
    for i in range(2, x.dim()):
        step_b *= x.size(i)
    size_b = b.numel() if b is not None else 1
    check(lib.ppst_fused_bias_act(_p(x), _p(b), _p(ref), _p(y), x.numel(), step_b, size_b, act, grad, float(alpha),
                                  float(scale), _DT_F64 if x.dtype == torch.float64 else _ST[x.dtype], _stream()), "ppst_fused_bias_act")
    return y


class ConvPlan:

    _GEOMETRY = {}
    _GEOM_ATTRS = ("kind", "cout", "cin", "k", "bn", "n_groups", "halo", "src", "max_chan", "wstrides", "nsteps", "flop_steps",
                   "early_a", "ksplit_ok", "chunk_starts0", "chunk_starts0_k64", "steps", "src_dev", "chunk_start", "chunks_per_group", "w4_shape", "max_chunk_steps",
                   "min_chunk_steps", "full_cover", "steps_dual", "src_dual", "steps_up9", "steps_k64", "src_k64", "steps_dual_k64",
                   "src_dual_k64")

    def __init__(self, weight, kind="conv", scale=1.0, chan_base=0, precision=None):
        _chk(weight, "weight")
        w = weight.detach().contiguous()
        gkey = (kind, tuple(w.shape), int(chan_base), str(w.device))
        geom = ConvPlan._GEOMETRY.get(gkey)
        if geom is None:
            self._build(w, kind, scale, chan_base, precision)
            ConvPlan._GEOMETRY[gkey] = {a: getattr(self, a) for a in ConvPlan._GEOM_ATTRS if hasattr(self, a)}
            return
        self.__dict__.update(geom)
        self.precision = PRECISION["value"] if precision is None else precision
        self.wparam, self.up_scale = w, float(scale)
        cout, cin, k, _ = w.shape
        if kind in ("convT", "dgradT"):
            wsrc = torch.empty((cin, cout, 4, 4), device=w.device, dtype=torch.float32)
            check(lib.ppst_upscale_weight(_p(w), _p(wsrc), cout, cin, float(scale), _stream()), "ppst_upscale_weight")
            if kind == "dgradT":
                self.fwd_scale = float(scale)
            scale = 1.0
        elif kind == "dgrad":
            wsrc = w.view(-1)[k * k - 1:]
        elif kind == "dgrad_s2ds":
            wsrc = torch.empty((4 * cin, cout, 2, 2), device=w.device, dtype=torch.float32)
            check(lib.ppst_dgrad_s2d_stack_weight(_p(w), _p(wsrc), cout, cin, _stream()), "ppst_dgrad_s2d_stack_weight")
        else:
            wsrc = w
        self.scale = float(scale)
        self.wsrc = wsrc
        if self.precision == 2:
            self.wpack = None
            return
        self._packs = {}
        self.wpack = self.pack_for(self.bn)

    def _build(self, w, kind, scale, chan_base, precision):
        self.kind = kind
        self.wparam, self.up_scale = w, float(scale)
        self.precision = PRECISION["value"] if precision is None else precision
        cout, cin, k, _ = w.shape
        assert cin % 32 == 0, "fused conv needs Cin % 32 == 0 (got %d)" % cin
        self.cout, self.cin, self.k = cout, cin, k
        self.bn = 128 if cout >= 128 else 64
        steps, src = [], []
        nchunk = cin // 32
        if kind == "conv":
            assert k in (1, 3)
            self.n_groups = 1
            self.halo = 0 if k == 1 else 1
            for c in range(nchunk):
                first = True
                for ky in range(k):
                    for kx in range(k):
                        steps.append((chan_base + 32 * c, ky - k // 2, kx - k // 2, 1 if first else 0))
                        src.append((32 * c, ky, kx))
                        first = False
            sn, sc, sy, sx = cin * k * k, k * k, k, 1
            wsrc = w
        elif kind == "s2d":
            assert k == 3
            self.n_groups = 1
            self.halo = 1
            for py in range(2):
                for px in range(2):
                    for c in range(nchunk):
                        first = True
                        for ey in range(2):
                            for ex in range(2):
                                ky, kx = 2 * ey + py, 2 * ex + px
                                if ky > 2 or kx > 2:
                                    continue
                                steps.append(((py * 2 + px) * cin + 32 * c, ey, ex, 1 if first else 0))
                                src.append((32 * c, ky, kx))
                                first = False
                        if py == 1 and px == 1:
                            steps.append(((py * 2 + px) * cin + 32 * c, 0, 0, 0))
                            src.append((-1, 0, 0))
            sn, sc, sy, sx = cin * 9, 9, 3, 1
            wsrc = w
        elif kind == "convT":
            assert k == 3
            self.n_groups = 4
            self.halo = 1
            wsrc = torch.empty((cin, cout, 4, 4), device=w.device, dtype=torch.float32)
            check(lib.ppst_upscale_weight(_p(w), _p(wsrc), cout, cin, float(scale), _stream()), "ppst_upscale_weight")
            scale = 1.0
            taps = {0: [(-1, 3), (0, 1)], 1: [(0, 2), (1, 0)]}
            for a in range(2):
                for b in range(2):
                    for c in range(nchunk):
                        first = True
                        for dy, ky in taps[a]:
                            for dx, kx in taps[b]:
                                steps.append((chan_base + 32 * c, dy, dx, 1 if first else 0))
                                src.append((32 * c, ky, kx))
                                first = False
            sn, sc, sy, sx = 16, cout * 16, 4, 1
            if cout % 128 == 0 and chan_base % 1 == 0:
                dsteps, dsrc = [], []
                for a in range(2):
                    for c in range(nchunk):
                        first = True
                        for dy, ky in taps[a]:
                            for j in range(2):
                                (dx0, kx0), (dx1, kx1) = taps[0][j], taps[1][j]
                                dsteps.append((chan_base + 32 * c, dy, (dx0 + 1) | ((dx1 + 1) << 8), 1 if first else 0))
                                dsrc.append((32 * c, ky, kx0 | (kx1 << 8)))
                                first = False
                self._dual_tmp = (dsteps, dsrc)
            if cout % 64 == 0:
                self._up9_tmp = [(chan_base + 32 * c, dy, dx, 1 if (dy, dx) == (0, 0) else 0)
                                 for c in range(nchunk) for dy, dx in ((0, 0), (-1, 0), (0, -1), (-1, -1))]
        elif kind == "dgrad":
            assert k in (1, 3)
            self.n_groups = 1
            self.halo = 0 if k == 1 else 1
            nchunk = cout // 32
            assert cout % 32 == 0
            for c in range(nchunk):
                first = True
                for ky in range(k):
                    for kx in range(k):
                        steps.append((32 * c, ky - k // 2, kx - k // 2, 1 if first else 0))
                        src.append((32 * c, ky, kx))
                        first = False
            wsrc = w.view(-1)[k * k - 1:]
            sn, sc, sy, sx = k * k, cin * k * k, -k, -1
            self.cout, self.cin = cin, cout
            cout, cin = cin, cout
            self.bn = 128 if cout >= 128 else 64
        elif kind == "dgrad_s2d":
            assert k == 3 and cout % 32 == 0
            self.n_groups = 4
            self.halo = 1
            taps = {0: [(0, 0), (-1, 2)], 1: [(0, 1)]}
            for py in range(2):
                for px in range(2):
                    for c in range(cout // 32):
                        tl = [(dy, dx, ky, kx) for dy, ky in taps[py] for dx, kx in taps[px]]
                        for i in range(4):
                            if i < len(tl):
                                dy, dx, ky, kx = tl[i]
                                steps.append((32 * c, dy, dx, 1 if i == 0 else 0))
                                src.append((32 * c, ky, kx))
                            else:
                                steps.append((32 * c, 0, 0, 0))
                                src.append((-1, 0, 0))
            wsrc = w
            sn, sc, sy, sx = 9, cin * 9, 3, 1
            self.cout, self.cin = cin, cout
            cout, cin = cin, cout
            self.bn = 128 if cout >= 128 else 64
        elif kind == "dgrad_s2ds":
            assert k == 3 and cout % 32 == 0
            self.n_groups = 1
            self.halo = 1
            for c in range(cout // 32):
                for i, (ty, tx) in enumerate(((0, 0), (0, 1), (1, 0), (1, 1))):
                    steps.append((32 * c, -ty, -tx, 1 if i == 0 else 0))
                    src.append((32 * c, ty, tx))
            wsrc = torch.empty((4 * cin, cout, 2, 2), device=w.device, dtype=torch.float32)
            check(lib.ppst_dgrad_s2d_stack_weight(_p(w), _p(wsrc), cout, cin, _stream()), "ppst_dgrad_s2d_stack_weight")
            sn, sc, sy, sx = cout * 4, 4, 2, 1
            self.cout, self.cin = 4 * cin, cout
            cout, cin = 4 * cin, cout
            self.bn = 128 if cout >= 128 else 64
        elif kind == "dgradT":
            assert k == 3 and cout % 32 == 0
            self.n_groups = 1
            self.halo = 1
            wsrc = torch.empty((cin, cout, 4, 4), device=w.device, dtype=torch.float32)
            check(lib.ppst_upscale_weight(_p(w), _p(wsrc), cout, cin, float(scale), _stream()), "ppst_upscale_weight")
            self.fwd_scale = float(scale)
            scale = 1.0
            taps = {0: [(0, 1), (1, 3)], 1: [(-1, 0), (0, 2)]}
            for py in range(2):
                for px in range(2):
                    for c in range(cout // 32):
                        first = True
                        for dqy, ky in taps[py]:
                            for dqx, kx in taps[px]:
                                steps.append(((py * 2 + px) * cout + 32 * c, dqy, dqx, 1 if first else 0))
                                src.append((32 * c, ky, kx))
                                first = False
            sn, sc, sy, sx = cout * 16, 16, 4, 1
            self.w4_shape = (cin, cout, 4, 4)
            self.cout, self.cin = cin, cout
            cout, cin = cin, cout
            self.bn = 128 if cout >= 128 else 64
        else:
            raise ValueError(kind)
        self.src = src
        self.max_chan = max(t[0] for t in steps)
        self.wstrides = (sn, sc, sy, sx)
        self.nsteps = len(steps) // self.n_groups
        self.flop_steps = sum(1 for t in src if t[0] >= 0) // self.n_groups
        live = [tuple(t[:3]) for t in src if t[0] >= 0]
        target = math.prod(self.w4_shape) if kind == "dgradT" else w.numel()
        self.full_cover = bool(self.n_groups == 1 and len(set(live)) == len(live) and len(live) * 32 * cout == target)
        dev = w.device
        ns_ = self.nsteps

        def encode(steps_):
            enc, chunk_idx = [], -1
            for i, (c_, dy_, dx_, f_) in enumerate(steps_):
                if i % ns_ == 0:
                    chunk_idx = -1
                chunk_idx += 1 if f_ else 0
                nxt = steps_[i + 1] if (i + 1) % ns_ != 0 else None
                w_ = f_ | ((2 | (nxt[0] << 8)) if (nxt is not None and nxt[3]) else 0) | ((chunk_idx & 1) << 2)
                enc.append((c_, dy_, dx_, w_))
            return enc
        enc = encode(steps)
        starts = [i for i, t in enumerate(steps) if t[3] == 1] + [len(steps)]
        lens = [b_ - a_ for a_, b_ in zip(starts[:-1], starts[1:])]
        self.chunk_starts0 = [i for i in starts if i < ns_] + [ns_]
        self.chunk_starts0_k64 = None
        self.early_a = 1 if (min(lens) >= 2 and ns_ >= 3) else 0
        self.max_chunk_steps = max(lens)
        self.min_chunk_steps = min(lens)
        self.ksplit_ok = bool(self.early_a and all(l_ >= 3 or (a_ % ns_) % 2 == 0 for a_, l_ in zip(starts[:-1], lens)))
        self.steps = torch.tensor(enc + [(0, 0, 0, 0)] * 4, dtype=torch.int32, device=dev).contiguous()
        self.steps_dual = self.src_dual = None
        dual = self.__dict__.pop("_dual_tmp", None)
        if dual is not None:
            self.steps_dual = torch.tensor(encode(dual[0]) + [(0, 0, 0, 0)] * 4, dtype=torch.int32, device=dev).contiguous()
            sd_ = torch.tensor(dual[1], dtype=torch.int32, device=dev)
            self.src_dual = (sd_[:, 0].contiguous(), sd_[:, 1].contiguous(), sd_[:, 2].contiguous())
        self.steps_k64 = self.src_k64 = self.steps_dual_k64 = self.src_dual_k64 = None

        def k64_tables(steps_, src_, ngroups):
            per = len(steps_) // ngroups
            keep, chunk = [], -1
            for i, t in enumerate(steps_):
                if i % per == 0:
                    chunk = -1
                chunk += 1 if t[3] else 0
                if chunk % 2 == 0:
                    keep.append(i)
            st = [steps_[i] for i in keep]
            per2 = len(st) // ngroups
            enc2, ci = [], -1
            for i, (c_, dy_, dx_, f_) in enumerate(st):
                if i % per2 == 0:
                    ci = -1
                ci += 1 if f_ else 0
                nxt = st[i + 1] if (i + 1) % per2 != 0 else None
                enc2.append((c_, dy_, dx_, f_ | ((2 | (nxt[0] << 8)) if (nxt is not None and nxt[3]) else 0) | ((ci & 1) << 2)))
            if ngroups == self.n_groups:
                self.chunk_starts0_k64 = [i for i, t in enumerate(st[:per2]) if t[3]] + [per2]
            sr = torch.tensor([src_[i] for i in keep], dtype=torch.int32, device=dev)
            return (torch.tensor(enc2 + [(0, 0, 0, 0)] * 4, dtype=torch.int32, device=dev).contiguous(),
                    (sr[:, 0].contiguous(), sr[:, 1].contiguous(), sr[:, 2].contiguous()))
        if kind in ("conv", "s2d", "convT") and self.halo == 1 and cin % 64 == 0 and cout >= 128 and self.early_a:
            self.steps_k64, self.src_k64 = k64_tables(steps, src, self.n_groups)
            if dual is not None:
                self.steps_dual_k64, self.src_dual_k64 = k64_tables(dual[0], dual[1], 2)
        up9 = self.__dict__.pop("_up9_tmp", None)
        self.steps_up9 = None
        if up9 is not None:
            self.steps_up9 = torch.tensor(encode(up9) + [(0, 0, 0, 0)] * 4, dtype=torch.int32, device=dev).contiguous()
        s = torch.tensor(src, dtype=torch.int32, device=dev)
        src_c, src_ky, src_kx = s[:, 0].contiguous(), s[:, 1].contiguous(), s[:, 2].contiguous()
        self.src_dev = (src_c, src_ky, src_kx)
        cs = [i for i, t in enumerate(steps) if t[3] == 1] + [len(steps)]
        self.chunk_start = torch.tensor(cs, dtype=torch.int32, device=dev)
        self.chunks_per_group = (len(cs) - 1) // self.n_groups
        self.scale = float(scale)
        self.wsrc = wsrc
        if self.precision == 2:
            self.wpack = None
            return
        self._packs = {}
        self.wpack = self.pack_for(self.bn)

    def pack_for(self, bn):
        hit = self._packs.get(bn)
        if hit is not None:
            return hit
        cout = self.cout
        sn, sc, sy, sx = self.wstrides
        src_c, src_ky, src_kx = self.src_dev
        n_tiles = (cout + bn - 1) // bn
        npl = 8 if self.precision == 0 else 4
        wpack = torch.empty(self.n_groups * n_tiles * self.nsteps * npl * bn * 8, dtype=torch.int16, device=self.steps.device)
        check(lib.ppst_conv_pack(_p(self.wsrc), sn, sc, sy, sx, float(self.scale), cout, bn, _p(src_c), _p(src_ky), _p(src_kx),
                                 self.nsteps, self.n_groups, self.precision, _p(wpack), _stream()), "ppst_conv_pack")
        self._packs[bn] = wpack
        return wpack

    def pack_dual(self):
        hit = self._packs.get("dual")
        if hit is not None:
            return hit
        sn, sc, sy, sx = self.wstrides
        c_, ky_, kx_ = self.src_dual
        n_tiles = (self.cout + 127) // 128
        npl = 8 if self.precision == 0 else 4
        wpack = torch.empty(2 * n_tiles * self.nsteps * npl * 256 * 8, dtype=torch.int16, device=self.steps.device)
        check(lib.ppst_conv_pack_dual(_p(self.wsrc), sn, sc, sy, sx, float(self.scale), self.cout, _p(c_), _p(ky_), _p(kx_),
                                      self.nsteps, 2, self.precision, _p(wpack), _stream()), "ppst_conv_pack_dual")
        self._packs["dual"] = wpack
        return wpack

    def pack_k64(self, bn, dual=False):
        key = "k64_dual" if dual else "k64_%d" % bn
        hit = self._packs.get(key)
        if hit is not None:
            return hit
        sn, sc, sy, sx = self.wstrides
        c_, ky_, kx_ = self.src_dual_k64 if dual else self.src_k64
        ng = 2 if dual else self.n_groups
        nst = c_.numel() // ng
        n_tiles = (self.cout + (bn // 2 if dual else bn) - 1) // (bn // 2 if dual else bn)
        wpack = torch.empty(ng * n_tiles * nst * 8 * bn * 8, dtype=torch.int16, device=self.steps.device)
        check(lib.ppst_conv_pack_k64(_p(self.wsrc), sn, sc, sy, sx, float(self.scale), self.cout, bn, _p(c_), _p(ky_), _p(kx_), nst, ng,
                                     self.precision, 1 if dual else 0, _p(wpack), _stream()), "ppst_conv_pack_k64")
        self._packs[key] = wpack
        return wpack

    def pack_up9(self):
        hit = self._packs.get("up9")
        if hit is not None:
            return hit
        w = self.wparam
        nbytes = lib.ppst_conv_pack_up9_bytes(self.cout, self.cin)
        wpack = torch.empty(nbytes // 2, dtype=torch.int16, device=self.steps.device)
        check(lib.ppst_conv_pack_up9(_p(w), self.cin * 9, 9, 3, 1, float(self.up_scale), self.cout, self.cin, _p(wpack), _stream()),
              "ppst_conv_pack_up9")
        self._packs["up9"] = wpack
        return wpack

    def pack_wino(self):
        hit = self._packs.get("wino")
        if hit is not None:
            return hit
        sn, sc, sy, sx = self.wstrides
        nbytes = lib.ppst_conv_pack_wino_bytes(self.cout, self.cin)
        wpack = torch.empty(nbytes // 2, dtype=torch.int16, device=self.steps.device)
        check(lib.ppst_conv_pack_wino(_p(self.wsrc), sn, sc, sy, sx, float(self.scale), self.cout, self.cin, _p(wpack), _stream()),
              "ppst_conv_pack_wino")
        self._packs["wino"] = wpack
        return wpack

    def takes_in_res(self, H, W):
        return (self.precision == 0 and self.kind == "conv" and self.k == 1 and
                self.choose_kernel(H, W, H, W, H, W, 1)[0] == 4)

    def wino_ok(self, th, tw, oh, ow, H, W, osy):
        return (self.precision == 0 and self.kind in ("conv", "dgrad") and self.k == 3 and self.cout >= 128 and osy == 1
                and (th, tw) == (oh, ow) == (H, W)
                and ((th + 15) // 16) * ((tw + 15) // 16) * ((self.cout + 127) // 128) >= WINO["min_blocks"])

    def choose_kernel(self, th, tw, oh, ow, H, W, osy, B=None, allow_up9=True):
        rows = TILE_ROWS["value"]
        variant, bn = 0, self.bn
        single = self.precision in (1, 3)
        if self.precision not in (0, 1, 3):
            return variant, bn, rows
        if WINO["value"] and self.wino_ok(th, tw, oh, ow, H, W, osy):
            wblocks = ((th + 15) // 16) * ((tw + 15) // 16) * ((self.cout + 127) // 128) * (B or 1)
            aware_b = BATCH_AWARE["value"] and B is not None
            if not (aware_b and (wblocks < WINO["fill"] or (KSPLIT["value"] and 0 in KSPLIT["variants"] and self.cout <= 256
                                                             and wblocks <= WINO["ksplit_fill"]))):
                return 10, 128, 16
        tiles16 = ((th + 15) // 16) * ((tw + 15) // 16) * self.n_groups
        cv = CONV_VARIANT["value"]
        if cv in (1, 3) or TWO_BLOCK_128["value"] or KSPLIT_128["value"] or TILE24_128["value"] or TALL_TILE_128["value"]:
            _need_experiments("the requested conv variant")
        if (UP9["value"] and allow_up9 and self.kind == "convT" and self.precision == 0 and getattr(self, "steps_up9", None) is not None
                and self.early_a and ((th + 14) // 15) * ((tw + 14) // 15) * (self.cout // 64) >= UP9["min_blocks"]
                and th * tw >= UP9["min_fill"] * (((th + 14) // 15) * 15) * (((tw + 14) // 15) * 15)):
            return "up9", 256, 15
        if (DUAL_CONVT["value"] and self.kind == "convT" and getattr(self, "steps_dual", None) is not None
                and self.cout % 256 != 0 and CONV_VARIANT["value"] == 2 and self.early_a
                and ((th + 15) // 16) * ((tw + 15) // 16) * 2 * (self.cout // 128) >= DUAL_CONVT["min_blocks"]):
            return "dual", 256, 16
        n256_ok = self.cout % 256 == 0 and tiles16 * (self.cout // 256) >= FAT_MIN_BLOCKS
        aware = BATCH_AWARE["value"] and B is not None and not single and self.bn == 128 and self.early_a and self.halo == 1
        if aware and n256_ok and tiles16 * (self.cout // 256) * B < BATCH_AWARE["fill"]:
            n256_ok = False
        small = (aware and tiles16 * ((self.cout + 127) // 128) * B < BATCH_AWARE["fill"]
                 and not (KSPLIT["value"] and 0 in KSPLIT["variants"]))
        if cv == 1 and not single and self.early_a and self.cout >= 128:
            variant, bn = 1, (256 if n256_ok else 128)
        elif cv in (2, 3) and self.early_a:
            force3 = cv == 3
            if n256_ok and not force3:
                variant, bn = 2, 256
            elif single:
                if (self.bn == 128 and self.halo == 1 and self.n_groups == 1 and TALL_TILE_SINGLE["value"] and
                        ((th + 31) // 32) * ((tw + 15) // 16) * ((self.cout + 127) // 128) >= TALL_TILE_SINGLE["min_blocks"]):
                    variant, rows = 7, 32
            elif self.bn == 128 and (force3 or (TWO_BLOCK_128["value"] and
                                                tiles16 * ((self.cout + 127) // 128) >= 2 * FAT_MIN_BLOCKS)):
                variant = 3
            elif (self.bn == 128 and self.halo == 1 and (small or (TWO_BLOCK_8ROW["value"] and
                  ((th + 7) // 8) * ((tw + 15) // 16) * self.n_groups * ((self.cout + 127) // 128) >= TWO_BLOCK_8ROW["min_blocks"]))):
                rows = 8
            elif (self.bn == 128 and KSPLIT_128["value"] and getattr(self, "ksplit_ok", False)
                  and tiles16 * ((self.cout + 127) // 128) >= KSPLIT_128["min_blocks"]):
                variant = 8
            elif (self.bn == 128 and TILE24_128["value"] and ((th + 23) // 24) * 24 <= th * (1.0 + TILE24_128["max_waste"]) and
                  ((th + 23) // 24) * ((tw + 15) // 16) * self.n_groups * ((self.cout + 127) // 128) >= TILE24_128["min_blocks"]):
                variant, rows = 9, 24
            elif (self.bn == 128 and TALL_TILE_128["value"] and
                  ((th + 31) // 32) * ((tw + 15) // 16) * self.n_groups * ((self.cout + 127) // 128) >= TALL_TILE_128["min_blocks"]):
                variant, rows = 7, 32
        same = (th, tw) == (oh, ow)
        if STREAM_1X1["value"] and self.halo == 0 and self.n_groups == 1 and osy == 1 and same and (oh, ow) == (H, W):
            variant, bn, rows = 4, 64, TILE_ROWS["value"]
        elif (self.halo == 1 and self.n_groups == 1 and osy == 1 and same and self.cout <= DIRECT_MAX["cout"]
              and self.nsteps <= DIRECT_MAX["nsteps"]):
            variant, bn, rows = (6 if (self.kind in ("conv", "dgrad") and self.k == 3) else 5), 64, TILE_ROWS["value"]
        elif (not single and self.kind in ("conv", "dgrad") and self.k == 3 and 64 < self.cout <= DIRECT_MAX["cout3x3"] and same):
            variant, bn, rows = 6, 128, TILE_ROWS["value"]
        return variant, bn, rows

    def _ksplit(self, variant, a, skip):
        if (skip or variant not in KSPLIT["variants"] or a.in_presplit
                or not (a.tile_rows == 16 or (variant == 0 and a.tile_rows == 8))):
            return 0, None
        cs = self.chunk_starts0_k64 if a.k64 else self.chunk_starts0
        if cs is None or cs[-1] != a.nsteps:
            return 0, None
        if a.dual_b or (variant == 2 and ((self.precision == 0) != (a.io_st == 0) or (a.k64 and not a.halo))):
            return 0, None
        n_tiles = -(-self.cout // a.bn)
        blocks = a.B * lib.ppst_conv_tiles(a.tile_h, a.tile_w, a.tile_rows) * a.n_groups * n_tiles
        max_s, min_steps = {0: (8, KSPLIT["min_steps"]), 2: (4, 24), 10: (2, 36)}[variant]
        return _ksplit_choice(blocks, cs, KSPLIT["max_blocks"], min_steps, max_s)

    def __call__(self, x, bias=None, noise=None, noise_weight=0.0, act=ACT_NONE, prelu=None, stats=False,
                 residual=None, out=None, out_scale=1.0, pad_mode=PAD_ZERO, out_hw=None, res_after_act=False,
                 in_ss=None, in_act=ACT_NONE, in_prelu=None, presplit=False, in_res=None):
        in_ld = _nhwc_ld(x, "conv input", half_ok=True)
        B, H, W, xc = x.shape
        if x.dtype != torch.float32 and {torch.float16: 3, torch.bfloat16: 1}[x.dtype] != self.precision:
            raise RuntimeError("conv input stored as %s needs a plan of the matching single-pass precision mode (plan: mode %d)"
                               % (x.dtype, self.precision))
        need_c = self.max_chan + 32
        if xc < need_c:
            raise RuntimeError("conv input has %d channels (pixel stride %d); the %s plan reads %d" % (xc, in_ld, self.kind, need_c))
        if in_ss is not None and (in_ss.dim() != 3 or in_ss.shape[0] != B or in_ss.shape[1] < need_c or in_ss.shape[2] != 2
                                  or not in_ss.is_contiguous()):
            raise RuntimeError("in_ss must be a contiguous (B=%d, >=%d, 2) table, got %s" % (B, need_c, tuple(in_ss.shape)))
        if self.kind == "convT":
            th, tw, oh, ow, osy = H, W, 2 * H, 2 * W, 2
        elif self.kind == "dgrad_s2d":
            oh, ow = out_hw
            th, tw, osy = (oh + 1) // 2, (ow + 1) // 2, 2
        elif self.kind in ("s2d", "dgrad_s2ds"):
            oh, ow = out_hw
            th, tw, osy = oh, ow, 1
        else:
            th, tw, oh, ow, osy = H, W, H, W, 1
        if out is None:
            out = torch.empty((B, oh, ow, self.cout), device=x.device, dtype=x.dtype)
        out_ld = _nhwc_ld(out, "conv output", half_ok=True)
        if out.dtype != x.dtype or (residual is not None and residual.dtype != x.dtype):
            raise RuntimeError("conv input, residual and output share one storage type (ppst_conv_args.io_st): got %s / %s / %s"
                               % (x.dtype, None if residual is None else residual.dtype, out.dtype))
        if tuple(out.shape) != (B, oh, ow, self.cout):
            raise RuntimeError("conv output must be %s, got %s" % ((B, oh, ow, self.cout), tuple(out.shape)))
        if noise is not None and (noise.numel() != B * oh * ow or not noise.is_contiguous()):
            raise RuntimeError("noise must be a contiguous (B,1,%d,%d) tensor with B = %d rows, got %s" % (oh, ow, B, tuple(noise.shape)))
        if residual is not None and tuple(residual.shape) != (B, oh, ow, self.cout):
            raise RuntimeError("residual must match the output shape %s, got %s" % ((B, oh, ow, self.cout), tuple(residual.shape)))
        for t, n in ((bias, "bias"), (noise, "noise"), (prelu, "prelu")):
            _chk(t, n)
        up9_ok = in_ss is None and residual is None and act != ACT_PRELU and pad_mode == PAD_ZERO
        variant, bn, rows = self.choose_kernel(th, tw, oh, ow, H, W, osy, B, allow_up9=up9_ok)
        if variant == 10 and in_ss is not None and self.cin > 1024:
            WINO["value"], prev = False, WINO["value"]
            try:
                variant, bn, rows = self.choose_kernel(th, tw, oh, ow, H, W, osy, B, allow_up9=up9_ok)
            finally:
                WINO["value"] = prev
        k64 = (K64["value"] and x.dtype != torch.float32 and self.precision in (1, 3) and variant in (2, 7, "dual")
               and (self.steps_dual_k64 if variant == "dual" else self.steps_k64) is not None)
        if k64 and variant == 7:
            variant, rows = 9, 24
        st = None
        if stats:
            tiles = lib.ppst_conv_tiles(th, tw, rows)
            st = torch.empty((B, (1 if variant == "up9" else self.n_groups) * tiles, self.cout, 2), device=x.device, dtype=torch.float32)
        a = _lib.ConvArgs()
        dual, up9 = variant == "dual", variant == "up9"
        if dual:
            variant = 2
        if up9:
            variant = 11
        if k64:
            wp = self.pack_k64(bn, dual)
            steps_t = self.steps_dual_k64 if dual else self.steps_k64
        else:
            wp = None if self.precision == 2 else (self.pack_wino() if variant == 10 else self.pack_up9() if up9 else self.pack_dual() if dual
                                                   else self.pack_for(bn))
            steps_t = self.steps_up9 if up9 else self.steps_dual if dual else self.steps
        a.x, a.wpack, a.steps, a.y = _p(x), _p(wp), _p(steps_t), _p(out)
        a.k64 = 1 if k64 else 0
        a.variant = variant
        a.dual_b = 1 if dual else 0
        a.bias, a.noise, a.prelu, a.stats = _p(bias), _p(noise), _p(prelu), _p(st)
        a.residual = _p(residual)
        a.res_ld = _nhwc_ld(residual, "residual", half_ok=True) if residual is not None else 0
        a.io_st = _ST[x.dtype]
        a.noise_weight, a.out_scale = float(noise_weight), float(out_scale)
        a.B, a.in_h, a.in_w, a.in_ld = B, H, W, in_ld
        a.out_h, a.out_w, a.out_ld, a.cout = oh, ow, out_ld, self.cout
        a.nsteps, a.n_groups, a.pad_mode = (self.nsteps // 2 if k64 else self.nsteps), (1 if up9 else 2 if dual else self.n_groups), pad_mode
        a.in_off_y = a.in_off_x = 0
        a.out_sy = a.out_sx = osy
        a.act, a.precision = act | (0x100 if res_after_act else 0), self.precision
        a.tile_h, a.tile_w, a.halo, a.bn, a.tile_rows = th, tw, self.halo, bn, rows
        _chk(in_ss, "in_ss"); _chk(in_prelu, "in_prelu")
        a.in_scale_shift, a.in_prelu, a.in_act = _p(in_ss), _p(in_prelu), in_act
        a.in_c = in_ss.shape[1] if in_ss is not None else 0
        if in_res is not None:
            if variant != 4 or in_ss is None or self.precision != 0 or x.dtype != torch.float32:
                raise RuntimeError("in_res needs a 1x1 plan on the streaming kernel (ops.STREAM_1X1), in_ss, precision 0 and fp32 storage")
            if tuple(in_res.shape) != tuple(x.shape):
                raise RuntimeError("in_res must have the conv input's shape %s, got %s" % (tuple(x.shape), tuple(in_res.shape)))
            a.in_res, a.in_res_ld = _p(in_res), _nhwc_ld(in_res, "in_res")
        a.flop_steps = self.flop_steps
        a.a_slots = min(3, self.chunks_per_group)
        a.early_a = self.early_a
        if presplit:
            _need_experiments("pre-split conv input")
            if variant != 0 or bn != 128 or in_ss is not None or self.nsteps // max(1, self.chunks_per_group) < 4:
                raise RuntimeError("pre-split input: tile kernel (bn 128) plans with chunks of >= 4 steps and no in_ss only")
            a.in_presplit = 1
        ks_S, ks_cuts = self._ksplit(variant, a, self.precision == 2) if (KSPLIT["value"] and BATCH_AWARE["value"]) else (0, None)
        stream = _stream()
        if ks_S:
            ks_arr = (ctypes.c_int32 * (ks_S + 1))(*ks_cuts)
            a.ksplit, a.ksplit_starts = ks_S, ctypes.cast(ks_arr, ctypes.c_void_p)
            a.ksplit_scratch, a.ksplit_flags, a.ksplit_epoch = _ksplit_next(stream)
        if self.precision == 2:
            sn, sc, sy, sx = self.wstrides
            c_, ky_, kx_ = self.src_dev
            check(lib.ppst_conv2d_f32(ctypes.byref(a), _p(self.wsrc), sn, sc, sy, sx, self.scale, _p(c_), _p(ky_), _p(kx_), stream),
                  "ppst_conv2d_f32")
        else:
            check(lib.ppst_conv2d_mfma(ctypes.byref(a), stream), "ppst_conv2d_mfma")
        if stats:
            return out, st
        return out


class _KsWorkspace:
    __slots__ = ("scratch", "flags", "ptrs", "launches")

    def __init__(self):
        self.scratch = torch.empty(KSPLIT_SCRATCH_BYTES, dtype=torch.uint8, device="cuda")
        self.flags = torch.zeros(KSPLIT_FLAG_WORDS, dtype=torch.int32, device="cuda")
        self.ptrs = self.scratch.data_ptr(), self.flags.data_ptr()
        self.launches = 0


_ks_ws = {}
_ks_lock = threading.Lock()


def _ks_key(stream):
    return (_cur_device() if _cur_device is not None else torch.cuda.current_device()), stream.value


def _ksplit_next(stream):
    key = _ks_key(stream)
    with _ks_lock:
        ws = _ks_ws.get(key)
        if ws is None:
            ws = _ks_ws[key] = _KsWorkspace()
        ws.launches += 1
        epoch = (ws.launches - 1) % 0xFFFFFFFF + 1
    return ws.ptrs + (epoch,)


def ksplit_launches():
    ws = _ks_ws.get(_ks_key(_stream()))
    return ws.launches if ws is not None else 0


def ksplit_check():
    ws = _ks_ws.get(_ks_key(_stream()))
    if ws is None:
        torch.cuda.current_stream().synchronize()
        return True
    marker = ws.flags[KSPLIT_FLAG_WORDS - 1:]
    if marker.item() == 0:
        return True
    marker.zero_()
    return False


def _ksplit_choice(blocks, chunk_starts, max_blocks, min_steps, max_s=8):
    nsteps = chunk_starts[-1]
    for S in (8, 4, 2):
        if S > max_s or blocks * S > max_blocks or (S - 1) * blocks > 256 or len(chunk_starts) - 1 < S:
            continue
        cuts = [0]
        for i in range(1, S):
            t = i * nsteps / S
            cuts.append(min(chunk_starts, key=lambda c: (abs(c - t), c)))
        cuts.append(nsteps)
        if all(b_ - a_ >= min_steps for a_, b_ in zip(cuts[:-1], cuts[1:])):
            return S, cuts
    return 0, None


def repack_plans(plans):
    import numpy as np
    up, pk, wino = [], [], []
    for pl in plans:
        if pl.precision == 2:
            continue
        if pl.kind == "dgrad_s2ds":
            wino.append(("s2ds", pl.wparam, pl.wsrc, pl.wparam.shape[0], pl.wparam.shape[1], None))
        if pl.kind in ("convT", "dgradT"):
            cin4, cout4 = pl.wsrc.shape[0], pl.wsrc.shape[1]
            up.append((pl.wparam.data_ptr(), pl.wsrc.data_ptr(), cin4 * cout4 * 16, float(pl.up_scale), cout4, cin4))
        sn, sc, sy, sx = pl.wstrides
        c_, ky_, kx_ = pl.src_dev
        for bn, wpack in pl._packs.items():
            if bn == "wino":
                wino.append((pl.wsrc, pl.wstrides, float(pl.scale), pl.cout, pl.cin, wpack))
                continue
            if isinstance(bn, str) and bn.startswith("k64_"):
                kd = bn == "k64_dual"
                kc, kky, kkx = pl.src_dual_k64 if kd else pl.src_k64
                kbn = 256 if kd else int(bn[4:])
                kng = 2 if kd else pl.n_groups
                knt = (pl.cout + (kbn // 2 if kd else kbn) - 1) // (kbn // 2 if kd else kbn)
                pk.append((pl.wsrc.data_ptr(), sn, sc, sy, sx, kc.data_ptr(), kky.data_ptr(), kkx.data_ptr(), wpack.data_ptr(),
                           kng * knt * (kc.numel() // kng) * 4 * kbn, float(pl.scale), pl.cout, kbn, kc.numel() // kng, kng,
                           2, 1 if pl.precision == 3 else 0, 1 if kd else 0))
                continue
            if bn == "up9":
                wino.append(("up9", pl.wparam, float(pl.up_scale), pl.cout, pl.cin, wpack))
                continue
            if bn == "dual":
                dc, dky, dkx = pl.src_dual
                pk.append((pl.wsrc.data_ptr(), sn, sc, sy, sx, dc.data_ptr(), dky.data_ptr(), dkx.data_ptr(), wpack.data_ptr(),
                           2 * ((pl.cout + 127) // 128) * pl.nsteps * 4 * 256, float(pl.scale), pl.cout, 256, pl.nsteps, 2,
                           1 if pl.precision == 0 else 0, 1 if pl.precision == 3 else 0, 1))
                continue
            n_tiles = (pl.cout + bn - 1) // bn
            pk.append((pl.wsrc.data_ptr(), sn, sc, sy, sx, c_.data_ptr(), ky_.data_ptr(), kx_.data_ptr(), wpack.data_ptr(),
                       pl.n_groups * n_tiles * pl.nsteps * 4 * bn, float(pl.scale), pl.cout, bn, pl.nsteps, pl.n_groups,
                       1 if pl.precision == 0 else 0, 1 if pl.precision in (3, 4) else 0, 0))
    dev = plans[0].steps.device if plans else None

    def table(cls, rows, fill):
        if not rows:
            return None, 0
        arr = (cls * len(rows))()
        b0 = 0
        for j, r in zip(arr, rows):
            nb = lib.ppst_pack_job_blocks(fill(j, r))
            j.block0, j.nblocks = b0, nb
            b0 += nb
        buf = torch.frombuffer(bytearray(bytes(arr)), dtype=torch.uint8).to(dev)
        return buf, b0

    def fill_up(j, r):
        j.w, j.out, j.total, j.scale, j.cout, j.cin = r
        return j.total

    def fill_pk(j, r):
        (j.w, j.sn, j.sc, j.sy, j.sx, j.src_c, j.src_ky, j.src_kx, j.out, j.total, j.scale, j.cout, j.bn, j.nsteps, j.n_groups,
         j.x3, j.f16, j.dual) = r
        return j.total
    tu, nbu = table(_lib.UpscaleJob, up, fill_up)
    tp, nbp = table(_lib.PackJob, pk, fill_pk)
    tables = (tu, len(up), nbu, tp, len(pk), nbp, wino)
    run_repack(tables)
    return tables


def run_repack(tables):
    tu, nu, nbu, tp, npk, nbp, wino = tables
    if nu:
        check(lib.ppst_upscale_weight_batch(_p(tu), nu, nbu, _stream()), "ppst_upscale_weight_batch")
    for e in wino:
        if isinstance(e[0], str) and e[0] == "s2ds":
            check(lib.ppst_dgrad_s2d_stack_weight(_p(e[1]), _p(e[2]), e[3], e[4], _stream()), "ppst_dgrad_s2d_stack_weight")
    if npk:
        check(lib.ppst_conv_pack_batch(_p(tp), npk, nbp, _stream()), "ppst_conv_pack_batch")
    for wsrc, strides, scale, cout, cin, wpack in wino:
        if isinstance(wsrc, str) and wsrc == "s2ds":
            continue
        if isinstance(wsrc, str):
            check(lib.ppst_conv_pack_up9(_p(strides), cin * 9, 9, 3, 1, scale, cout, cin, _p(wpack), _stream()), "ppst_conv_pack_up9")
            continue
        sn, sc, sy, sx = strides
        check(lib.ppst_conv_pack_wino(_p(wsrc), sn, sc, sy, sx, scale, cout, cin, _p(wpack), _stream()), "ppst_conv_pack_wino")


def _grad_out(out, shape, like):
    if out is None:
        return torch.empty(shape, device=like.device, dtype=torch.float32)
    n = 1
    for d in shape:
        n *= d
    if out.numel() != n or not out.is_contiguous() or out.dtype != torch.float32 or not out.is_cuda:
        raise RuntimeError("gradient destination must be a contiguous float32 CUDA tensor of %d elements, got %s" % (n, tuple(out.shape)))
    return out


WGRAD_TR = {"value": True, "blocks": 256, "min_tiles": 8, "form": 2, "blocks2": 512, "pair": True, "bf16_single_pass": True, "exact": True, "nohalo": True}


def presplit(x):
    ld = _nhwc_ld(x)
    B, H, W, C = x.shape
    y = torch.empty((B, H, W, C), device=x.device, dtype=torch.float32)
    check(lib.ppst_presplit(_p(x), _p(y), B * H * W, C, ld, C, _stream()), "ppst_presplit")
    return y


def conv_wgrad(plan, x, dy, splits=None, out=None, accumulate=False, bias_out=None, bias_accumulate=False, want_bias=False, dy_scale=1.0):
    assert plan.kind in ("conv", "s2d", "dgradT")
    assert dy_scale == 1.0 or not (want_bias or bias_out is not None)
    in_ld = _nhwc_ld(x, "x", half_ok=True)
    dy_ld = _nhwc_ld(dy, "dy", half_ok=True)
    half = x.dtype != torch.float32 or dy.dtype != torch.float32
    if half and not (x.dtype == dy.dtype == torch.bfloat16 and PRECISION["value"] == 1 and WGRAD_X3["value"] and WGRAD_TR["value"]
                     and WGRAD_TR["form"] == 2 and WGRAD_TR["bf16_single_pass"]):
        raise RuntimeError("conv_wgrad on half-stored operands: both bfloat16, precision mode 1, the single-pass transposed-read kernel "
                           "(got %s / %s, mode %d)" % (x.dtype, dy.dtype, PRECISION["value"]))
    B, H, W, _ = x.shape
    _, oh, ow, cout = dy.shape
    assert cout == plan.cout
    nchunks = plan.chunk_start.numel() - 1
    want_bias = want_bias or bias_out is not None
    aligned = cout % 4 == 0 and dy_ld % 4 == 0 and in_ld % 4 == 0 and x.data_ptr() % 16 == 0 and dy.data_ptr() % 16 == 0
    if half and not (aligned and cout % 8 == 0 and dy_ld % 8 == 0 and in_ld % 8 == 0):
        raise RuntimeError("conv_wgrad on bfloat16 operands needs channel counts / strides divisible by 8 and 16-byte aligned tensors")
    x3 = WGRAD_X3["value"] and plan.precision != 2 and aligned
    use_tr = x3 and WGRAD_TR["value"]
    per = nchunks * ((cout + 127) // 128)
    tiles_total = B * ((oh + 1) // 2) * ((ow + 31) // 32)
    csum = None
    if use_tr:
        form2 = WGRAD_TR["form"] == 2
        if form2 and WGRAD_TR["pair"] and plan.max_chunk_steps <= 4 and nchunks % 2 == 0:
            per = (nchunks // 2) * ((cout + 127) // 128)
            if (WGRAD_TR["nohalo"] and WGRAD_TR["exact"] and plan.kind == "conv" and plan.k == 1 and plan.halo == 0 and nchunks % 4 == 0
                    and (H, W) == (oh, ow)):
                per = (nchunks // 4) * ((cout + 127) // 128)
        if form2:
            gz = splits if splits is not None else max(1, min(max(1, WGRAD_TR["blocks2"] // per), max(1, tiles_total // WGRAD_TR["min_tiles"]), 2048))
            splits = gz
        else:
            gz = splits // 2 if splits is not None else max(1, min(max(1, WGRAD_TR["blocks"] // per), max(1, tiles_total // WGRAD_TR["min_tiles"]), 1024))
            splits = 2 * gz
        if want_bias:
            csum = torch.empty((gz, cout), device=x.device, dtype=torch.float32)
    elif splits is None:
        splits = max(1, min((WGRAD_SPLIT["blocks"] + per - 1) // per, max(1, tiles_total // WGRAD_SPLIT["min_tiles"]), 2048))
    partial = torch.empty((splits, plan.nsteps, cout, 32), device=x.device, dtype=torch.float32)
    if PROF_ON["value"]:
        lib.ppst_wgrad_flop_steps(int(plan.flop_steps))
    if use_tr:
        if WGRAD_TR["form"] == 2:
            check(lib.ppst_conv_wgrad_tr2_st(_p(x), _p(dy), _p(plan.steps), _p(plan.chunk_start), _p(partial), _p(csum), B, H, W, in_ld, oh, ow,
                                             dy_ld, cout, plan.nsteps, nchunks, splits, plan.max_chunk_steps if WGRAD_TR["pair"] else 0,
                                             plan.min_chunk_steps if WGRAD_TR["exact"] else 0,
                                             0 if (WGRAD_TR["nohalo"] and plan.kind == "conv" and plan.k == 1 and plan.halo == 0) else 1,
                                             1 if (PRECISION["value"] == 1 and WGRAD_TR["bf16_single_pass"]) else 3,
                                             _ST[x.dtype], _stream()), "ppst_conv_wgrad_tr2")
        else:
            check(lib.ppst_conv_wgrad_tr(_p(x), _p(dy), _p(plan.steps), _p(plan.chunk_start), _p(partial), _p(csum), B, H, W, in_ld, oh, ow,
                                         dy_ld, cout, plan.nsteps, nchunks, splits, _stream()), "ppst_conv_wgrad_tr")
    else:
        fn, name = ((lib.ppst_conv_wgrad_bf16x3, "ppst_conv_wgrad_bf16x3") if x3 else (lib.ppst_conv_wgrad_f32, "ppst_conv_wgrad_f32"))
        check(fn(_p(x), _p(dy), _p(plan.steps), _p(plan.chunk_start), _p(partial), B, H, W, in_ld, oh, ow, dy_ld,
                 cout, plan.nsteps, nchunks, splits, _stream()), name)
    shape = plan.w4_shape if plan.kind == "dgradT" else (plan.cout, plan.cin, plan.k, plan.k)
    cover = getattr(plan, "full_cover", False)
    if out is None:
        dw = (torch.empty if cover else torch.zeros)(shape, device=x.device, dtype=torch.float32)
    else:
        dw = _grad_out(out, shape, x)
        if not accumulate and not cover:
            dw.zero_()
    sn, sc, sy, sx = plan.wstrides
    c_, ky_, kx_ = plan.src_dev
    db = None
    if csum is not None:
        db = _grad_out(bias_out, (cout,), x)
    check(lib.ppst_wgrad_scatter(_p(partial), _p(c_), _p(ky_), _p(kx_), _p(dw), sn, sc, sy, sx, cout, plan.nsteps, splits,
                                 plan.scale * float(dy_scale), 1 if (accumulate and out is not None) else 0, _p(csum), _p(db),
                                 csum.shape[0] if csum is not None else 0, 1 if (bias_accumulate and bias_out is not None) else 0,
                                 _stream()), "ppst_wgrad_scatter")
    if not want_bias:
        return dw
    if csum is None:
        db = colsum(dy.as_strided((dy.shape[0] * oh * ow, cout), (dy_ld, 1)), out=bias_out, accumulate=bias_accumulate)
    return dw, db


def wgrad_small_cin(x, dy, scale, out=None, accumulate=False):
    in_ld = _nhwc_ld(x)
    B, H, W, cin = x.shape
    cout = dy.shape[3]
    assert _nhwc_ld(dy, "dy", half_ok=True) == cout
    ws = torch.empty(lib.ppst_wgrad_small_cin_ws(B * H * W, cin, cout) // 4, device=x.device, dtype=torch.float32)
    dw = _grad_out(out, (cout, cin, 1, 1), x)
    check(lib.ppst_wgrad_small_cin_st(_p(x), _p(dy), _p(dw), _p(ws), B * H * W, cin, in_ld, cout, float(scale),
                                      1 if (accumulate and out is not None) else 0, _ST[dy.dtype], _stream()), "ppst_wgrad_small_cin")
    return dw


def colsum(x2d, scale=1.0, out=None, accumulate=False):
    _chk_act(x2d)
    rows, C = x2d.shape
    ld = x2d.stride(0)
    assert x2d.stride(1) == 1
    ws = torch.empty(lib.ppst_colsum_ws(rows, C) // 4, device=x2d.device, dtype=torch.float32)
    dst = _grad_out(out, (C,), x2d)
    check(lib.ppst_colsum_st(_p(x2d), _p(dst), _p(ws), rows, C, ld, float(scale), 1 if (accumulate and out is not None) else 0,
                             _ST[x2d.dtype], _stream()), "ppst_colsum")
    return dst


def linear_wgrad(dy, x, scale=1.0, out=None, accumulate=False):
    _chk(dy); _chk(x)
    dy, x = dy.contiguous(), x.contiguous()
    B, N = dy.shape
    K = x.shape[1]
    dw = _grad_out(out, (N, K), x)
    check(lib.ppst_linear_wgrad(_p(dy), _p(x), _p(dw), B, N, K, float(scale), 1 if (accumulate and out is not None) else 0, _stream()),
          "ppst_linear_wgrad")
    return dw


def linear_wgrad_fused(dy, x, scale=1.0, out=None, accumulate=False, relu_in=False, bias_out=None, bias_scale=1.0, bias_accumulate=False,
                       want_bias=False):
    _chk(dy); _chk(x)
    dy, x = dy.contiguous(), x.contiguous()
    B, N = dy.shape
    K = x.shape[1]
    dw = _grad_out(out, (N, K), x)
    db = _grad_out(bias_out, (N,), x) if (want_bias or bias_out is not None) else None
    check(lib.ppst_linear_wgrad_fused(_p(dy), _p(x), _p(dw), _p(db), B, N, K, float(scale), float(bias_scale),
                                      1 if (accumulate and out is not None) else 0, 1 if (bias_accumulate and bias_out is not None) else 0,
                                      1 if relu_in else 0, _stream()), "ppst_linear_wgrad_fused")
    return dw, db


def linear_dgrad_gate(dy, w, gate, scale=1.0):
    _chk(dy); _chk(w); _chk(gate)
    dy, w, gate = dy.contiguous(), w.detach().contiguous(), gate.contiguous()
    B, N = dy.shape
    K = w.shape[1]
    assert tuple(gate.shape) == (B, K)
    dx = torch.empty((B, K), device=dy.device, dtype=torch.float32)
    ws = torch.empty(lib.ppst_linear_dgrad_ws(B, N, K) // 4, device=dy.device, dtype=torch.float32)
    check(lib.ppst_linear_dgrad_gate(_p(dy), _p(w), _p(dx), _p(ws), _p(gate), B, N, K, float(scale), _stream()), "ppst_linear_dgrad_gate")
    return dx


def linear_dgrad(dy, w, scale=1.0):
    _chk(dy); _chk(w)
    dy, w = dy.contiguous(), w.detach().contiguous()
    B, N = dy.shape
    K = w.shape[1]
    dx = torch.empty((B, K), device=dy.device, dtype=torch.float32)
    ws = torch.empty(lib.ppst_linear_dgrad_ws(B, N, K) // 4, device=dy.device, dtype=torch.float32)
    check(lib.ppst_linear_dgrad(_p(dy), _p(w), _p(dx), _p(ws), B, N, K, float(scale), _stream()), "ppst_linear_dgrad")
    return dx


def lsgan(pred, target, weight):
    _chk(pred)
    pred = pred.contiguous()
    loss = torch.empty((1,), device=pred.device, dtype=torch.float32)
    grad = torch.empty_like(pred)
    check(lib.ppst_lsgan(_p(pred), _p(loss), _p(grad), pred.numel(), float(target), float(weight), _stream()), "ppst_lsgan")
    return loss, grad


def l1_mean(a, b, weight=1.0):
    _chk(a); _chk(b)
    a, b = a.contiguous(), b.contiguous()
    assert a.shape == b.shape
    n = a.numel()
    ws = torch.empty(lib.ppst_l1_mean_ws(n) // 4, device=a.device, dtype=torch.float32)
    out = torch.empty((1,), device=a.device, dtype=torch.float32)
    check(lib.ppst_l1_mean(_p(a), _p(b), _p(out), _p(ws), n, float(weight), _stream()), "ppst_l1_mean")
    return out


def rscl_loss(q, k, k0, queue, nce_T=0.07):
    for t in (q, k, k0, queue):
        _chk(t)
    q, k, k0, queue = q.contiguous(), k.contiguous(), k0.contiguous(), queue.contiguous()
    n, C = q.shape
    ws = torch.empty((n,), device=q.device, dtype=torch.float32)
    out = torch.empty((1,), device=q.device, dtype=torch.float32)
    check(lib.ppst_rscl_loss(_p(q), _p(k), _p(k0), _p(queue), _p(out), _p(ws), n, k0.shape[0], C, queue.shape[1], float(nce_T), _stream()),
          "ppst_rscl_loss")
    return out


def adam_step_(p, g, m, v, lr, beta1, beta2, eps, step):
    for t in (p, g, m, v):
        _chk(t)
        assert t.is_contiguous()
    check(lib.ppst_adam_step(_p(p), _p(g), _p(m), _p(v), p.numel(), float(lr), float(beta1), float(beta2), float(eps), int(step),
                             _stream()), "ppst_adam_step")


def conv1x1_small_cin(x, w, bias, wscale, act, out_dtype=torch.float32):
    ld = _nhwc_ld(x)
    B, H, W, cin = x.shape
    cout = w.shape[0]
    y = torch.empty((B, H, W, cout), device=x.device, dtype=out_dtype)
    w2 = w.detach().reshape(cout, cin).contiguous()
    check(lib.ppst_conv1x1_small_cin_st(_p(x), _p(w2), _p(bias), _p(y), B * H * W, cin, ld, cout, float(wscale), act,
                                        _ST[out_dtype], _stream()), "ppst_conv1x1_small_cin")
    return y


def conv1x1_small_cout(x, w, bias, wscale):
    ld = _nhwc_ld(x, half_ok=True)
    B, H, W, cin = x.shape
    assert ld == cin
    cout = w.shape[0]
    y = torch.empty((B, H, W, cout), device=x.device, dtype=torch.float32)
    w2 = w.detach().reshape(cout, cin).contiguous()
    check(lib.ppst_conv1x1_small_cout_st(_p(x), _p(w2), _p(bias), _p(y), B * H * W, cin, cout, float(wscale), _ST[x.dtype], _stream()),
          "ppst_conv1x1_small_cout")
    return y


def torgb_apply(x, scale_shift, res, out_scale, w, bias, wscale):
    ld = _nhwc_ld(x, half_ok=True)
    B, H, W, cin = x.shape
    if ld != cin or w.shape[0] != 3:
        raise RuntimeError("torgb_apply needs a dense input and a 3-channel weight")
    _chk(scale_shift, "scale_shift"); _chk(bias, "bias")
    res_ld = 0
    if res is not None:
        res_ld = _nhwc_ld(res, "res", half_ok=True)
        if res.dtype != x.dtype or tuple(res.shape) != (B, H // 2, W // 2, cin):
            raise RuntimeError("torgb_apply: res must be the half-resolution tensor of x's type")
    if tuple(scale_shift.shape) != (B, cin, 2) or not scale_shift.is_contiguous():
        raise RuntimeError("torgb_apply: scale_shift must be a contiguous (B, C, 2) table")
    y = torch.empty((B, H, W, 3), device=x.device, dtype=torch.float32)
    w2 = w.detach().reshape(3, cin).contiguous()
    check(lib.ppst_torgb_apply_st(_p(x), _p(scale_shift), _p(res), res_ld, float(out_scale), _p(w2), _p(bias), _p(y), B, H, W, cin,
                                  float(wscale), _ST[x.dtype], _stream()), "ppst_torgb_apply")
    return y


def upscale_weight_bwd(dw4, cout, cin, scale=1.0, out=None, accumulate=False):
    _chk(dw4)
    dw = _grad_out(out, (cout, cin, 3, 3), dw4)
    check(lib.ppst_upscale_weight_bwd(_p(dw4.contiguous()), _p(dw), cout, cin, float(scale), 1 if (accumulate and out is not None) else 0,
                                      _stream()), "ppst_upscale_weight_bwd")
    return dw


DGRAD_S2D_STACK = {"value": os.environ.get("PPST_DGRAD_S2D_STACK", "1") != "0", "max_cin": int(os.environ.get("PPST_DGRAD_S2D_MAXCIN", "64"))}


def depth_to_space(x, out_hw):
    ld = _nhwc_ld(x, "depth_to_space input", half_ok=True)
    B, th, tw, c4 = x.shape
    if ld != c4 or c4 % 4:
        raise RuntimeError("depth_to_space needs a dense tensor with 4 C channels")
    oh, ow = out_hw
    y = torch.empty((B, oh, ow, c4 // 4), device=x.device, dtype=x.dtype)
    check(lib.ppst_depth_to_space_st(_p(x), _p(y), B, th, tw, oh, ow, c4 // 4, _ST[x.dtype], _stream()), "ppst_depth_to_space_st")
    return y


def dgrad_s2d(net, wname, scale, g, out_hw):
    cin = net.p(wname).shape[1]
    per = 8 if g.dtype != torch.float32 else 4
    if DGRAD_S2D_STACK["value"] and cin <= DGRAD_S2D_STACK["max_cin"] and cin % per == 0:
        oh, ow = out_hw
        ys = net.plan(wname, "dgrad_s2ds", scale)(g, out_hw=((oh + 1) // 2, (ow + 1) // 2))
        return depth_to_space(ys, out_hw)
    return net.plan(wname, "dgrad_s2d", scale)(g, out_hw=out_hw)


def space_to_depth(x):
    ld = _nhwc_ld(x, half_ok=True)
    B, H, W, C = x.shape
    y = torch.empty((B, (H + 1) // 2, (W + 1) // 2, 4 * C), device=x.device, dtype=x.dtype)
    check(lib.ppst_space_to_depth_st(_p(x), _p(y), B, H, W, C, ld, _ST[x.dtype], _stream()), "ppst_space_to_depth")
    return y


def in_stats(x, rep_pad=False):
    ld = _nhwc_ld(x)
    B, H, W, C = x.shape
    n = ctypes.c_int(0)
    check(lib.ppst_in_stats(None, None, B, H, W, C, ld, 0, ctypes.byref(n), None), "ppst_in_stats(size)")
    part = torch.empty((B, n.value, C, 2), device=x.device, dtype=torch.float32)
    check(lib.ppst_in_stats(_p(x), _p(part), B, H, W, C, ld, 1 if rep_pad else 0, ctypes.byref(n), _stream()), "ppst_in_stats")
    return part


def in_finalize(partial, count, style=None, post_bias=None, eps=1e-5):
    _chk(partial)
    _chk(style, "style")
    _chk(post_bias, "post_bias")
    B, n, C, _ = partial.shape
    style_ld = 0
    if style is not None:
        assert style.shape == (B, 2 * C) and style.stride(1) == 1
        style_ld = style.stride(0) if B > 1 else max(style.stride(0), 2 * C)
    ss = torch.empty((B, C, 2), device=partial.device, dtype=torch.float32)
    check(lib.ppst_in_finalize(_p(partial), n, _p(style), style_ld, _p(post_bias), _p(ss), B, C, float(count), float(eps),
                               _stream()), "ppst_in_finalize")
    return ss


def in_finalize_train(partial, count, style=None, post_bias=None, eps=1e-5):
    _chk(partial); _chk(style, "style"); _chk(post_bias, "post_bias")
    B, n, C, _ = partial.shape
    style_ld = 0
    if style is not None:
        assert style.shape == (B, 2 * C) and style.stride(1) == 1
        style_ld = style.stride(0) if B > 1 else max(style.stride(0), 2 * C)
    ss = torch.empty((B, C, 2), device=partial.device, dtype=torch.float32)
    mr = torch.empty((B, C, 2), device=partial.device, dtype=torch.float32)
    check(lib.ppst_in_finalize_train(_p(partial), n, _p(style), style_ld, _p(post_bias), _p(ss), _p(mr), B, C, float(count), float(eps),
                                     _stream()), "ppst_in_finalize_train")
    return ss, mr


def dual_stats(g, y, gate=None):
    g_ld, y_ld = _nhwc_ld(g, "g", half_ok=True), _nhwc_ld(y, "y", half_ok=True)
    gate_ld = _nhwc_ld(gate, "gate", half_ok=True) if gate is not None else 0
    B, H, W, C = g.shape
    assert y.shape == g.shape
    if y.dtype != g.dtype or (gate is not None and gate.dtype != g.dtype):
        raise RuntimeError("dual_stats: g, y and gate share one storage type (got %s / %s / %s)" % (g.dtype, y.dtype, None if gate is None else gate.dtype))
    n = ctypes.c_int(0)
    check(lib.ppst_dual_stats(None, None, None, None, B, H * W, C, g_ld, y_ld, gate_ld, ctypes.byref(n), None), "ppst_dual_stats(size)")
    part = torch.empty((B, n.value, C, 2), device=g.device, dtype=torch.float32)
    check(lib.ppst_dual_stats_st(_p(g), _p(y), _p(gate), _p(part), B, H * W, C, g_ld, y_ld, gate_ld, ctypes.byref(n), _ST[g.dtype], _stream()),
          "ppst_dual_stats")
    return part


def in_bwd_finalize(partial, count, mean_rstd=None, style=None, want_dstyle=False):
    _chk(partial); _chk(mean_rstd); _chk(style)
    B, n, C, _ = partial.shape
    style_ld = 0
    if style is not None:
        assert style.shape[0] == B and style.shape[1] >= C and style.stride(1) == 1
        style_ld = style.stride(0) if B > 1 else max(style.stride(0), C)
    coef = torch.empty((B, C, 4), device=partial.device, dtype=torch.float32) if mean_rstd is not None else None
    dstyle = torch.empty((B, 2 * C), device=partial.device, dtype=torch.float32) if (want_dstyle or mean_rstd is None) else None
    check(lib.ppst_in_bwd_finalize(_p(partial), n, _p(mean_rstd), _p(style), style_ld, _p(coef), _p(dstyle), B, C, float(count),
                                   _stream()), "ppst_in_bwd_finalize")
    return coef, dstyle


def in_bwd_apply(g, y, coef, gate=None, post_gate=False):
    g_ld, y_ld = _nhwc_ld(g, "g", half_ok=True), _nhwc_ld(y, "y", half_ok=True)
    gate_ld = _nhwc_ld(gate, "gate", half_ok=True) if gate is not None else 0
    B, H, W, C = g.shape
    if y.dtype != g.dtype or (gate is not None and gate.dtype != g.dtype):
        raise RuntimeError("in_bwd_apply: g, y and gate share one storage type")
    dx = torch.empty((B, H, W, C), device=g.device, dtype=g.dtype)
    check(lib.ppst_in_bwd_apply_st(_p(g), _p(y), _p(gate), _p(coef), _p(dx), B, H * W, C, g_ld, y_ld, gate_ld, C, 1 if post_gate else 0,
                                   _ST[g.dtype], _stream()), "ppst_in_bwd_apply")
    return dx


def prelu_bwd(g, y, prelu, scale_shift=None, res=None):
    g_ld, y_ld = _nhwc_ld(g, "g"), _nhwc_ld(y, "y")
    res_ld = _nhwc_ld(res, "res") if res is not None else 0
    _chk(prelu); _chk(scale_shift)
    B, H, W, C = g.shape
    total = B * H * W * C
    ws = torch.empty(lib.ppst_prelu_bwd_ws(total) // 4, device=g.device, dtype=torch.float32)
    gpre = torch.empty((B, H, W, C), device=g.device, dtype=torch.float32)
    check(lib.ppst_prelu_bwd(_p(g), _p(y), _p(scale_shift), _p(res), _p(prelu), _p(gpre), _p(ws), B, H * W, C, g_ld, y_ld, res_ld,
                             _stream()), "ppst_prelu_bwd")
    ds = torch.empty((1,), device=g.device, dtype=torch.float32)
    check(lib.ppst_sum_partials(_p(ws), _p(ds), ws.numel(), 1.0, _stream()), "ppst_sum_partials")
    return gpre, ds


def pad2d(x, py0, py1, px0, px1, mode):
    ld = _nhwc_ld(x, half_ok=True)
    B, H, W, C = x.shape
    y = torch.empty((B, H + py0 + py1, W + px0 + px1, C), device=x.device, dtype=x.dtype)
    check(lib.ppst_pad2d_st(_p(x), _p(y), B, H, W, C, ld, py0, py1, px0, px1, mode, _ST[x.dtype], _stream()), "ppst_pad2d")
    return y


def pad2d_bwd(dy, py0, py1, px0, px1, mode):
    _chk_act(dy)
    dy = dy.contiguous()
    B, OH, OW, C = dy.shape
    H, W = OH - py0 - py1, OW - px0 - px1
    dx = torch.empty((B, H, W, C), device=dy.device, dtype=dy.dtype)
    check(lib.ppst_pad2d_bwd_st(_p(dy), _p(dx), B, H, W, C, py0, py1, px0, px1, mode, _ST[dy.dtype], _stream()), "ppst_pad2d_bwd")
    return dx


def bilinear_bwd(dy, H, W):
    dy_ld = _nhwc_ld(dy, half_ok=True)
    B, OH, OW, C = dy.shape
    dx = torch.zeros((B, H, W, C), device=dy.device, dtype=dy.dtype)
    check(lib.ppst_bilinear_bwd_st(_p(dy), _p(dx), B, H, W, C, C, OH, OW, dy_ld, _ST[dy.dtype], _stream()), "ppst_bilinear_bwd")
    return dx


def avgpool_bwd(dy, f):
    dy_ld = _nhwc_ld(dy)
    B, oh, ow, C = dy.shape
    dx = torch.empty((B, oh * f, ow * f, C), device=dy.device, dtype=torch.float32)
    check(lib.ppst_avgpool_bwd(_p(dy), _p(dx), B, oh * f, ow * f, C, C, f, dy_ld, _stream()), "ppst_avgpool_bwd")
    return dx


def gap_gmp_bwd(x, mask, v, g, out=None):
    ld = _nhwc_ld(x, half_ok=True)
    B, H, W, C = x.shape
    _chk(mask); _chk(v); _chk(g)
    acc = out is not None
    if out is None:
        out = torch.empty((B, H, W, C), device=x.device, dtype=x.dtype)
    arg = torch.empty((B, C), device=x.device, dtype=torch.int32)
    check(lib.ppst_gap_gmp_bwd_st(_p(x), _p(mask), _p(v.contiguous()), _p(g.contiguous()), _p(out), ctypes.c_void_p(arg.data_ptr()), B, H * W, C,
                                  ld, 1 if acc else 0, _ST[x.dtype], _stream()), "ppst_gap_gmp_bwd")
    return out


def gap_gmp_multi(x, masks, with_plain=True):
    ld = _nhwc_ld(x, half_ok=True)
    B, H, W, C = x.shape
    _chk(masks, "masks")
    masks = masks.contiguous()
    nm = masks.shape[3]
    assert tuple(masks.shape[:3]) == (B, H, W) and 1 <= nm <= 3
    heads = nm + (1 if with_plain else 0)
    ws = torch.empty(lib.ppst_gap_gmp_multi_ws(B, H * W, C, heads) // 4, device=x.device, dtype=torch.float32)
    out = torch.empty((heads * B, 2 * C), device=x.device, dtype=torch.float32)
    check(lib.ppst_gap_gmp_multi(_p(x), _p(masks), _p(out), _p(ws), B, H, W, C, ld, nm, 1 if with_plain else 0, _ST[x.dtype], _stream()),
          "ppst_gap_gmp_multi")
    return out


def gap_gmp_multi_bwd(x, masks, v, g, with_plain=True, out=None):
    ld = _nhwc_ld(x, half_ok=True)
    B, H, W, C = x.shape
    _chk(masks); _chk(v); _chk(g)
    masks = masks.contiguous()
    nm = masks.shape[3]
    heads = nm + (1 if with_plain else 0)
    acc = out is not None
    if out is None:
        out = torch.empty((B, H, W, C), device=x.device, dtype=x.dtype)
    arg = torch.empty((heads * B, C), device=x.device, dtype=torch.int32)
    check(lib.ppst_gap_gmp_multi_bwd(_p(x), _p(masks), _p(v.contiguous()), _p(g.contiguous()), _p(out), ctypes.c_void_p(arg.data_ptr()), B,
                                     H * W, C, ld, nm, 1 if with_plain else 0, 1 if acc else 0, _ST[x.dtype], _stream()),
          "ppst_gap_gmp_multi_bwd")
    return out


def l2norm_rows_bwd(g, x, eps, mode):
    _chk(g); _chk(x)
    g, x = g.contiguous(), x.contiguous()
    B, K = x.shape
    dx = torch.empty_like(x)
    check(lib.ppst_l2norm_rows_bwd(_p(g), _p(x), _p(dx), B, K, float(eps), mode, _stream()), "ppst_l2norm_rows_bwd")
    return dx


def softmax_rows_bwd_(p, g, div=1.0):
    _chk(p); _chk(g)
    assert p.is_contiguous() and g.is_contiguous() and p.shape == g.shape
    cols = p.shape[-1]
    check(lib.ppst_softmax_rows_bwd(_p(p), _p(g), p.numel() // cols, cols, float(div), _stream()), "ppst_softmax_rows_bwd")
    return g


def corr_prep_bwd(g, x, ncenter=256):
    _chk(g); _chk(x)
    g, x = g.contiguous(), x.contiguous()
    B, P, C = x.shape
    dx = torch.empty_like(x)
    check(lib.ppst_corr_prep_bwd(_p(g), _p(x), _p(dx), B * P, C, ncenter, 2.220446049250313e-16, _stream()), "ppst_corr_prep_bwd")
    return dx


def l1_grad(a, b, weight=1.0):
    _chk(a); _chk(b)
    a, b = a.contiguous(), b.contiguous()
    da = torch.empty_like(a)
    check(lib.ppst_l1_grad(_p(a), _p(b), _p(da), a.numel(), float(weight), _stream()), "ppst_l1_grad")
    return da


def rscl_loss_bwd(q, k, k0, queue, gout, nce_T=0.07):
    for t in (q, k, k0, queue, gout):
        _chk(t)
    q, k, k0, queue = q.contiguous(), k.contiguous(), k0.contiguous(), queue.contiguous()
    n, C = q.shape
    dq = torch.empty_like(q)
    check(lib.ppst_rscl_loss_bwd(_p(q), _p(k), _p(k0), _p(queue), _p(gout.contiguous()), _p(dq), n, k0.shape[0], C, queue.shape[1],
                                 float(nce_T), _stream()), "ppst_rscl_loss_bwd")
    return dq


def rselfcorr_bwd(fea, dout):
    ld = _nhwc_ld(fea)
    B, H, W, C = fea.shape
    assert ld == C
    dout_ld = _nhwc_ld(dout)
    dfea = torch.empty_like(fea)
    check(lib.ppst_rselfcorr_bwd(_p(fea), _p(dout), _p(dfea), B, H, W, C, dout_ld, _stream()), "ppst_rselfcorr_bwd")
    return dfea


def transpose_last2(x):
    _chk(x)
    x = x.contiguous()
    b, M, N = x.shape
    y = torch.empty((b, N, M), device=x.device, dtype=torch.float32)
    check(lib.ppst_nchw_to_nhwc(_p(x), _p(y), b, M, 1, N, _stream()), "ppst_nchw_to_nhwc")
    return y


def scale_by(x, s):
    _chk(x); _chk(s)
    x = x.contiguous()
    y = torch.empty_like(x)
    check(lib.ppst_scale_by(_p(x), _p(s.contiguous()), _p(y), x.numel(), _stream()), "ppst_scale_by")
    return y


def noise_wgrad(dpre, noise, out=None, accumulate=False):
    ld = _nhwc_ld(dpre, half_ok=True)
    B, H, W, C = dpre.shape
    _chk(noise)
    noise = noise.contiguous()
    assert noise.numel() == B * H * W
    ws = torch.empty(lib.ppst_noise_wgrad_ws(B * H * W) // 4, device=dpre.device, dtype=torch.float32)
    dst = _grad_out(out, (1,), dpre)
    check(lib.ppst_noise_wgrad_st(_p(dpre), _p(noise), _p(dst), _p(ws), B * H * W, C, ld, 1 if (accumulate and out is not None) else 0,
                                  _ST[dpre.dtype], _stream()), "ppst_noise_wgrad")
    return dst


def affine_act(x, scale_shift=None, res=None, act=ACT_NONE, prelu=None, out_scale=1.0, res_before_act=False, out=None,
               res_scale_shift=None, res_up2=False, out_dtype=None):
    x_ld = _nhwc_ld(x, half_ok=True)
    B, H, W, C = x.shape
    if out is None:
        out = torch.empty((B, H, W, C), device=x.device, dtype=out_dtype or x.dtype)
    y_ld = _nhwc_ld(out, half_ok=True)
    res_ld = _nhwc_ld(res, "res", half_ok=True) if res is not None else 0
    if res is not None and res.dtype != x.dtype:
        raise RuntimeError("affine_act: res must have the storage type of x (%s), got %s" % (x.dtype, res.dtype))
    _chk(scale_shift, "scale_shift")
    _chk(res_scale_shift, "res_scale_shift")
    _chk(prelu, "prelu")
    if res_up2:
        assert res.shape[1] * 2 == H and res.shape[2] * 2 == W
    flag = act | (RES_BEFORE_ACT if res_before_act else 0)
    check(lib.ppst_affine_act_st(_p(x), _p(scale_shift), _p(res), _p(res_scale_shift), _p(out), B, H * W, C, x_ld, res_ld, y_ld,
                                 flag, _p(prelu), float(out_scale), W if res_up2 else 0, _ST[x.dtype], _ST[out.dtype], _stream()),
          "ppst_affine_act")
    return out


def affine_act_stats(x, scale_shift=None, res=None, act=ACT_NONE, prelu=None, out_scale=1.0, res_before_act=False,
                     res_scale_shift=None, rep_pad=False, res_up2=False):
    x_ld = _nhwc_ld(x)
    B, H, W, C = x.shape
    out = torch.empty((B, H, W, C), device=x.device, dtype=torch.float32)
    res_ld = _nhwc_ld(res, "res") if res is not None else 0
    for t in (scale_shift, res_scale_shift, prelu):
        _chk(t)
    n = ctypes.c_int(0)
    check(lib.ppst_in_stats(None, None, B, H, W, C, x_ld, 0, ctypes.byref(n), None), "ppst_in_stats(size)")
    part = torch.empty((B, n.value, C, 2), device=x.device, dtype=torch.float32)
    flag = act | (RES_BEFORE_ACT if res_before_act else 0)
    check(lib.ppst_affine_act_stats(_p(x), _p(scale_shift), _p(res), _p(res_scale_shift), _p(out), _p(part), B, H, W, C, x_ld,
                                    res_ld, C, flag, _p(prelu), float(out_scale), 1 if rep_pad else 0, 1 if res_up2 else 0,
                                    _stream()),
          "ppst_affine_act_stats")
    return out, part


def upsample_nearest2(x):
    ld = _nhwc_ld(x, half_ok=True)
    B, H, W, C = x.shape
    assert ld == C
    y = torch.empty((B, 2 * H, 2 * W, C), device=x.device, dtype=x.dtype)
    check(lib.ppst_upsample_nearest2_st(_p(x), _p(y), B, H, W, C, _ST[x.dtype], _stream()), "ppst_upsample_nearest2")
    return y


def gap_gmp(x, mask=None):
    ld = _nhwc_ld(x, half_ok=True)
    B, H, W, C = x.shape
    _chk(mask, "mask")
    ws = torch.empty(lib.ppst_gap_gmp_ws(B, H * W, C) // 4, device=x.device, dtype=torch.float32)
    out = torch.empty((B, 2 * C), device=x.device, dtype=torch.float32)
    check(lib.ppst_gap_gmp_st(_p(x), _p(mask), _p(out), _p(ws), B, H, W, C, ld, _ST[x.dtype], _stream()), "ppst_gap_gmp")
    return out


def avgpool(x, f, out=None):
    x_ld = _nhwc_ld(x)
    B, H, W, C = x.shape
    if out is None:
        out = torch.empty((B, H // f, W // f, C), device=x.device, dtype=torch.float32)
    y_ld = _nhwc_ld(out)
    check(lib.ppst_avgpool(_p(x), _p(out), B, H, W, C, x_ld, f, y_ld, _stream()), "ppst_avgpool")
    return out


def bilinear(x, OH, OW, out=None):
    x_ld = _nhwc_ld(x)
    B, H, W, C = x.shape
    if out is None:
        out = torch.empty((B, OH, OW, C), device=x.device, dtype=torch.float32)
    y_ld = _nhwc_ld(out)
    check(lib.ppst_bilinear(_p(x), _p(out), B, H, W, C, x_ld, OH, OW, y_ld, _stream()), "ppst_bilinear")
    return out


def head_tail(x, scale_shift, feat, feat1, act=ACT_NONE, prelu=None):
    x_ld = _nhwc_ld(x)
    B, H, W, C = x.shape
    P, D = H // feat.shape[1], H // feat1.shape[1]
    _chk(scale_shift, "scale_shift"); _chk(prelu, "prelu")
    check(lib.ppst_head_tail(_p(x), _p(scale_shift), _p(prelu), _p(feat), _p(feat1), B, H, W, C, x_ld, _nhwc_ld(feat), _nhwc_ld(feat1),
                             P, D, act, _stream()), "ppst_head_tail")


def maxpool2(x):
    ld = _nhwc_ld(x)
    B, H, W, C = x.shape
    assert ld == C
    y = torch.empty((B, H // 2, W // 2, C), device=x.device, dtype=torch.float32)
    check(lib.ppst_maxpool2(_p(x), _p(y), B, H, W, C, _stream()), "ppst_maxpool2")
    return y


def linear(x, w, bias=None, wscale=1.0, bscale=1.0, relu_in=False, act=ACT_NONE):
    _chk(x, "x"); _chk(w, "weight"); _chk(bias, "bias")
    x = x.contiguous()
    w = w.detach().contiguous()
    B, K = x.shape
    N = w.shape[0]
    assert w.numel() == N * K
    y = torch.empty((B, N), device=x.device, dtype=torch.float32)
    check(lib.ppst_linear(_p(x), _p(w), _p(bias), _p(y), B, K, N, float(wscale), float(bscale), 1 if relu_in else 0, act,
                          _stream()), "ppst_linear")
    return y


def l2norm_rows(x, eps, mode):
    _chk(x)
    x = x.contiguous()
    B, K = x.shape
    y = torch.empty_like(x)
    check(lib.ppst_l2norm_rows(_p(x), _p(y), B, K, float(eps), mode, _stream()), "ppst_l2norm_rows")
    return y


def lerp(a, b, r):
    _chk(a); _chk(b)
    a, b = a.contiguous(), b.contiguous()
    y = torch.empty_like(a)
    check(lib.ppst_lerp(_p(a), _p(b), _p(y), a.numel(), float(r), _stream()), "ppst_lerp")
    return y


def spatial_modulation(x, scale, bias, out_dtype=torch.float32):
    ld = _nhwc_ld(x)
    B, H, W, C = x.shape
    assert ld == C
    y = torch.empty(x.shape, device=x.device, dtype=out_dtype)
    check(lib.ppst_spatial_modulation_st(_p(x), _p(scale.contiguous()), _p(bias.contiguous()), _p(y), B, H * W, C, _ST[out_dtype],
                                         _stream()), "ppst_spatial_modulation")
    return y


def rselfcorr(fea, out=None):
    ld = _nhwc_ld(fea)
    B, H, W, C = fea.shape
    assert ld == C
    if out is None:
        out = torch.empty((B, H // 4, W // 4, 256), device=fea.device, dtype=torch.float32)
    out_ld = _nhwc_ld(out)
    check(lib.ppst_rselfcorr(_p(fea), _p(out), B, H, W, C, out_ld, _stream()), "ppst_rselfcorr")
    return out


def corr_prep(fea, ncenter=256):
    _chk(fea)
    fea = fea.contiguous()
    B, P, C = fea.shape
    y = torch.empty_like(fea)
    check(lib.ppst_corr_prep(_p(fea), _p(y), B, P, C, ncenter, _stream()), "ppst_corr_prep")
    return y


def unfold_rows(x, k):
    _chk(x)
    x = x.contiguous()
    B, H, W, C = x.shape
    out = torch.empty((B, H * W, C * k * k), device=x.device, dtype=torch.float32)
    check(lib.ppst_unfold_rows(_p(x), _p(out), B, H, W, C, int(k), _stream()), "ppst_unfold_rows")
    return out


def unfold_rows_bwd(g, shape, k):
    _chk(g)
    g = g.contiguous()
    B, H, W, C = shape
    dx = torch.empty((B, H, W, C), device=g.device, dtype=torch.float32)
    check(lib.ppst_unfold_rows_bwd(_p(g), _p(dx), B, H, W, C, int(k), _stream()), "ppst_unfold_rows_bwd")
    return dx


GEMM_MODE = {"value": None}


def _gemm_passes(mode, K):
    mode = GEMM_MODE["value"] or mode or "x6"
    if mode not in ("f32", "x6", "x3"):
        raise ValueError("gemm mode %r" % (mode,))
    if mode == "f32" or PRECISION["value"] == 2:
        return 0
    if mode == "x3" and K % 32 == 0:
        return 3
    return 6 if K % 16 == 0 else 0


def gemm_nt(A, Bm, alpha=1.0, mode=None):
    _chk(A); _chk(Bm)
    A, Bm = A.contiguous(), Bm.contiguous()
    b, M, K = A.shape
    N = Bm.shape[1]
    C = torch.empty((b, M, N), device=A.device, dtype=torch.float32)
    passes = _gemm_passes(mode, K)
    if passes:
        check(lib.ppst_gemm_nt_split(_p(A), _p(Bm), _p(C), b, M, N, K, float(alpha), passes, _stream()), "ppst_gemm_nt_split")
    else:
        check(lib.ppst_gemm_nt_f32(_p(A), _p(Bm), _p(C), b, M, N, K, float(alpha), _stream()), "ppst_gemm_nt_f32")
    return C


def gemm_nn(A, Bm, mode=None):
    _chk(A); _chk(Bm)
    A, Bm = A.contiguous(), Bm.contiguous()
    b, M, K = A.shape
    N = Bm.shape[2]
    C = torch.empty((b, M, N), device=A.device, dtype=torch.float32)
    passes = _gemm_passes(mode, K) if N % 4 == 0 else 0
    if passes:
        check(lib.ppst_gemm_nn_split(_p(A), _p(Bm), _p(C), b, M, N, K, N, N, passes, _stream()), "ppst_gemm_nn_split")
    else:
        check(lib.ppst_gemm_nn_f32(_p(A), _p(Bm), _p(C), b, M, N, K, N, N, _stream()), "ppst_gemm_nn_f32")
    return C


def softmax_rows_(x, div=1.0):
    _chk(x)
    assert x.is_contiguous()
    cols = x.shape[-1]
    check(lib.ppst_softmax_rows(_p(x), x.numel() // cols, cols, float(div), _stream()), "ppst_softmax_rows")
    return x


def unfold_patches(x, s):
    _chk(x)
    x = x.contiguous()
    B, C, H, W = x.shape
    y = torch.empty((B, (H // s) * (W // s), C * s * s), device=x.device, dtype=torch.float32)
    check(lib.ppst_unfold_patches(_p(x), _p(y), B, C, H, W, s, _stream()), "ppst_unfold_patches")
    return y


def fold_patches(x, C, H, W, s):
    _chk(x)
    x = x.contiguous()
    B = x.shape[0]
    y = torch.empty((B, C, H, W), device=x.device, dtype=torch.float32)
    check(lib.ppst_fold_patches(_p(x), _p(y), B, C, H, W, s, _stream()), "ppst_fold_patches")
    return y


def tensor2im_u8(x):
    _chk(x)
    x = x.contiguous()
    B, C, H, W = x.shape
    y = torch.empty((B, H, W, C), device=x.device, dtype=torch.uint8)
    check(lib.ppst_tensor2im_u8(_p(x), _p(y), B, C, H, W, _stream()), "ppst_tensor2im_u8")
    return y


def guided_filter(guide_u8, src_u8, r=30, eps=(0.02 * 255) ** 2, want_u8=False):
    for t in (guide_u8, src_u8):
        if not t.is_cuda or t.dtype != torch.uint8:
            raise RuntimeError("guided_filter needs CUDA uint8 tensors")
    guide_u8, src_u8 = guide_u8.contiguous(), src_u8.contiguous()
    B, H, W, _ = guide_u8.shape
    ws = torch.empty(lib.ppst_guided_filter_ws(B, H, W), device=guide_u8.device, dtype=torch.uint8)
    out = torch.empty((B, 3, H, W), device=guide_u8.device, dtype=torch.float32)
    out_u8 = torch.empty((B, H, W, 3), device=guide_u8.device, dtype=torch.uint8) if want_u8 else None
    check(lib.ppst_guided_filter(_p(guide_u8), _p(src_u8), _p(out), _p(out_u8), B, H, W, r, float(eps), _p(ws), _stream()),
          "ppst_guided_filter")
    return (out, out_u8) if want_u8 else out


PROF_ON = {"value": False}


def prof_enable(on):
    PROF_ON["value"] = bool(on)
    check(lib.ppst_prof_enable(1 if on else 0), "ppst_prof_enable")


def prof_collect():
    ms, n, fl = ctypes.c_double(0), ctypes.c_int64(0), ctypes.c_double(0)
    dropped = lib.ppst_prof_dropped()
    check(lib.ppst_prof_collect(ctypes.byref(ms), ctypes.byref(n), ctypes.byref(fl)), "ppst_prof_collect")
    if dropped:
        raise RuntimeError("conv profiling pool overflowed: %d launches were not timed (use fewer --steps)" % dropped)
    return ms.value, n.value, fl.value


def prof_detail():
    out = []
    i = 0
    while True:
        ms, fl = ctypes.c_double(0), ctypes.c_double(0)
        info = (ctypes.c_int * 8)()
        if lib.ppst_prof_detail(i, ctypes.byref(ms), ctypes.byref(fl), info) != 0:
            break
        out.append((ms.value, fl.value, tuple(info)))
        i += 1
    return out
```

Baseline: 159.5 swaps/s (all GPUs).

## Fuse blur downsample into strided 3x3 conv for residual down blocks

Adds a conv_blur kernel that applies the 3x3 blur taps on the fly while computing the following stride-2 3x3 conv, so the blurred space-to-depth intermediate is never written to and read back from memory. The shared 1x1 conv helpers move into a common header so the new kernel can reuse the epilogue. A per-shape table enables the fused path only for the (32, 64, unnormalized) case by default. The grid is capped at 256 blocks, and the fused path loses the s2d conv's weight-side layout, so it may compute more per output.

After: 160.0 swaps/s (all GPUs), median of 6. About the same (+0.4%).

```diff
diff --git a/include/ppst_hip.h b/include/ppst_hip.h
--- a/include/ppst_hip.h
+++ b/include/ppst_hip.h
@@ -143,6 +143,8 @@
 } ppst_conv_args;
 
 int ppst_conv2d_mfma(const ppst_conv_args* a, void* stream);
+int ppst_conv_blur(const ppst_conv_args* a, const void* blur_k, void* stream);
+int ppst_conv_blur_tiles(int out_h, int out_w);
 int64_t ppst_conv_pack_wino_bytes(int cout, int cin);
 int ppst_conv_pack_wino(const void* w, int64_t sn, int64_t sc, int64_t sy, int64_t sx, float scale, int cout, int cin,
                         void* out, void* stream);
diff --git a/ppst_amd/_lib.py b/ppst_amd/_lib.py
--- a/ppst_amd/_lib.py
+++ b/ppst_amd/_lib.py
@@ -66,6 +66,8 @@
     "ppst_conv_pack_batch": (i32, [vp, i32, i32, vp]),
     "ppst_upscale_weight_batch": (i32, [vp, i32, i32, vp]),
     "ppst_conv2d_mfma": (i32, [ctypes.POINTER(ConvArgs), vp]),
+    "ppst_conv_blur": (i32, [ctypes.POINTER(ConvArgs), vp, vp]),
+    "ppst_conv_blur_tiles": (i32, [i32, i32]),
     "ppst_has_experiments": (i32, []),
     "ppst_presplit": (i32, [vp, vp, i64, i32, i32, i32, vp]),
     "ppst_conv2d_f32": (i32, [ctypes.POINTER(ConvArgs), vp, i64, i64, i64, i64, f32, vp, vp, vp, vp]),
diff --git a/ppst_amd/build.py b/ppst_amd/build.py
--- a/ppst_amd/build.py
+++ b/ppst_amd/build.py
@@ -8,7 +8,7 @@
 OBJ = os.path.join(HERE, "csrc", "_obj")
 LIB = os.path.join(HERE, "libppst_hip.so")
 EXPERIMENTS = os.environ.get("PPST_EXPERIMENTS") == "1"
-SOURCES = ["upfirdn2d.hip", "fused_bias_act.hip", "elementwise.hip", "linear.hip", "conv_mfma.hip", "conv_mfma2.hip", "conv1x1.hip", "conv_wino.hip", "conv_f32.hip",
+SOURCES = ["upfirdn2d.hip", "fused_bias_act.hip", "elementwise.hip", "linear.hip", "conv_mfma.hip", "conv_mfma2.hip", "conv1x1.hip", "conv_blur.hip", "conv_wino.hip", "conv_f32.hip",
            "corr.hip", "guided_filter.hip", "train.hip", "train_g.hip", "imageio.hip", "smooth_filter.hip"] + (["conv_ksplit.hip"] if EXPERIMENTS else [])
 FLAGS = ["--offload-arch=gfx950", "-O3", "-fPIC", "-std=c++17", "-Wno-unused-result"] + (["-DPPST_EXPERIMENTS"] if EXPERIMENTS else [])
 FILE_FLAGS = {"conv_wino.hip": ["-fno-slp-vectorize"]}
@@ -22,7 +22,7 @@
     return "hipcc"
 
 
-HEADERS = [os.path.join(CSRC, "common.h"), os.path.join(CSRC, "rscl_common.h"), os.path.join(HERE, "..", "include", "ppst_hip.h")]
+HEADERS = [os.path.join(CSRC, "common.h"), os.path.join(CSRC, "conv1x1_common.h"), os.path.join(CSRC, "rscl_common.h"), os.path.join(HERE, "..", "include", "ppst_hip.h")]
 
 
 def _stale(target, deps):
diff --git a/ppst_amd/csrc/conv1x1.hip b/ppst_amd/csrc/conv1x1.hip
--- a/ppst_amd/csrc/conv1x1.hip
+++ b/ppst_amd/csrc/conv1x1.hip
@@ -1,193 +1,5 @@
-#include "common.h"
-
-struct C1Args {
-  const float* x;
-  const unsigned char* wpack;
-  const int4* steps;
-  float* y;
-  const float* bias;
-  const float* noise;
-  const float* prelu;
-  float* stats;
-  const float* residual;
-  float noise_weight, out_scale;
-  int B, hw, in_ld, out_ld, cout, nsteps, act, res_ld, n_tiles, tiles;
-  int in_h, in_w, out_h, out_w, tiles_x, pad_mode;
-  const float* in_ss;
-  const float* in_prelu;
-  int in_c, in_act;
-  const float* in_res;
-  int in_res_ld;
-};
-
-#define C1_GROUP 8
-#define C1_BLOB 8192
-
-typedef _Float16 __attribute__((ext_vector_type(8))) c1_half8;
-template <int PREC>
-__device__ __forceinline__ void c1_cvt(float v, unsigned short& h, unsigned short& l) {
-  if (PREC == 0) split_bf16(v, h, l);
-  else if (PREC == 3) { h = __builtin_bit_cast(unsigned short, (_Float16)v); l = 0; }
-  else { h = f2bf(v); l = 0; }
-}
-template <int PREC>
-__device__ __forceinline__ void c1_cvt8(const float (&v)[8], bf16x8& hi, bf16x8& lo) {
-  if (PREC == 3) {
-#pragma unroll
-    for (int j = 0; j < 8; ++j) {
-      unsigned short h, l;
-      c1_cvt<PREC>(v[j], h, l);
-      hi[j] = (short)h;
-      lo[j] = (short)l;
-    }
-    return;
-  }
-  uint2 h0, l0 = make_uint2(0u, 0u), h1, l1 = make_uint2(0u, 0u);
-  if (PREC == 0) {
-    split_bf16x4(make_float4(v[0], v[1], v[2], v[3]), h0, l0);
-    split_bf16x4(make_float4(v[4], v[5], v[6], v[7]), h1, l1);
-  } else {
-    h0 = f2bf_x4(make_float4(v[0], v[1], v[2], v[3]));
-    h1 = f2bf_x4(make_float4(v[4], v[5], v[6], v[7]));
-  }
-  hi = __builtin_bit_cast(bf16x8, make_uint4(h0.x, h0.y, h1.x, h1.y));
-  lo = __builtin_bit_cast(bf16x8, make_uint4(l0.x, l0.y, l1.x, l1.y));
-}
-template <int IOS>
-__device__ __forceinline__ void c1_unpack8(float4 r, float (&v)[8]) {
-  const float4 a = st_unpack4<IOS>(make_uint2(__float_as_uint(r.x), __float_as_uint(r.y)));
-  const float4 b = st_unpack4<IOS>(make_uint2(__float_as_uint(r.z), __float_as_uint(r.w)));
-  v[0] = a.x; v[1] = a.y; v[2] = a.z; v[3] = a.w; v[4] = b.x; v[5] = b.y; v[6] = b.z; v[7] = b.w;
-}
-template <int PREC>
-__device__ __forceinline__ f32x4 c1_mfma(bf16x8 bh, bf16x8 bl, bf16x8 xh, bf16x8 xl, f32x4 acc) {
-  if (PREC == 0) {
-    acc = __builtin_amdgcn_mfma_f32_16x16x32_bf16(bh, xl, acc, 0, 0, 0);
-    acc = __builtin_amdgcn_mfma_f32_16x16x32_bf16(bl, xh, acc, 0, 0, 0);
-    return __builtin_amdgcn_mfma_f32_16x16x32_bf16(bh, xh, acc, 0, 0, 0);
-  }
-  if (PREC == 3) return __builtin_amdgcn_mfma_f32_16x16x32_f16(__builtin_bit_cast(c1_half8, bh), __builtin_bit_cast(c1_half8, xh), acc, 0, 0, 0);
-  return __builtin_amdgcn_mfma_f32_16x16x32_bf16(bh, xh, acc, 0, 0, 0);
-}
-
-__device__ __forceinline__ int c1_pad(int i, int n, int mode) {
-  if (mode == PPST_PAD_REFLECT) {
-    if (i < 0) i = -i;
-    if (i >= n) i = 2 * (n - 1) - i;
-  }
-  return i < 0 ? 0 : (i >= n ? n - 1 : i);
-}
-
-template <int MT, int NT, bool TAPS, bool SPEC = true, int IOS = PPST_ST_F32>
-__device__ __forceinline__ void c1_epilogue(const C1Args& a, f32x4 (&acc)[MT][NT], float (&red)[8][NT > 4 ? 128 : 64][2], int b, int mblk,
-                                            int ntile, int pbase, int oy0, int ox, int tid, int wave, int r16, int g) {
-  const int act = a.act & 0xff;
-  const bool res_after = (a.act >> 8) & 1;
-  const float slope = (act == PPST_ACT_PRELU && a.prelu) ? a.prelu[0] : 0.f;
-  float4 s1[NT], s2[NT];
-#pragma unroll
-  for (int nt = 0; nt < NT; ++nt) { s1[nt] = make_float4(0.f, 0.f, 0.f, 0.f); s2[nt] = s1[nt]; }
-  const int64_t img = (int64_t)b * (TAPS ? a.out_h * a.out_w : a.hw);
-  constexpr int ES = IOS == PPST_ST_F32 ? 4 : 2;
-  unsigned char* const yb = (unsigned char*)a.y + img * a.out_ld * ES;
-  const float* const nzb = a.noise ? a.noise + img : nullptr;
-  const unsigned char* const rb = a.residual ? (const unsigned char*)a.residual + img * a.res_ld * ES : nullptr;
-  const int nbase = ntile * (NT > 4 ? 128 : 64) + g * 4;
-  float nzv[MT];
-  float4 bva[NT];
-  const __amdgpu_buffer_rsrc_t nrs = __builtin_amdgcn_make_buffer_rsrc((void*)(nzb ? (const void*)nzb : (const void*)yb), 0,
-                                                                       nzb ? (TAPS ? a.out_h * a.out_w : a.hw) * 4 : 0, 0x00020000);
-#pragma unroll
-  for (int mt = 0; mt < MT; ++mt) {
-    const int p = pbase + mt * 16 + r16;
-    const bool ok = TAPS ? (oy0 + mt < a.out_h && ox < a.out_w) : p < a.hw;
-    nzv[mt] = a.noise_weight * __builtin_bit_cast(float, __builtin_amdgcn_raw_buffer_load_b32(
-                                   nrs, ok ? (TAPS ? (oy0 + mt) * a.out_w + ox : p) * 4 : (int)0x80000000, 0, 0));
-  }
-#pragma unroll
-  for (int nt = 0; nt < NT; ++nt)
-    bva[nt] = __builtin_bit_cast(float4, __builtin_amdgcn_raw_buffer_load_b128(__builtin_amdgcn_make_buffer_rsrc((void*)(a.bias ? (const void*)a.bias : (const void*)a.y), 0, a.bias ? a.cout * 4 : 0, 0x00020000), (nbase + nt * 16) * 4, 0, 0));
-  auto epi_passes = [&](auto act_c, auto res_c) {
-#pragma clang fp contract(off)
-    const int ACT = act_c.value, RES = res_c.value;
-#pragma unroll
-  for (int mt = 0; mt < MT; ++mt) {
-    const int p = pbase + mt * 16 + r16;
-    if (TAPS ? (oy0 + mt >= a.out_h || ox >= a.out_w) : p >= a.hw) continue;
-    const int pin = TAPS ? (oy0 + mt) * a.out_w + ox : p;
-    const int yo = pin * a.out_ld, ro = pin * a.res_ld;
-    const float nz = nzv[mt];
-#pragma unroll
-    for (int nt = 0; nt < NT; ++nt) {
-      const int n0 = nbase + nt * 16;
-      if (n0 >= a.cout) continue;
-      float4 rv = make_float4(0.f, 0.f, 0.f, 0.f);
-      const float4 bv = bva[nt];
-      if (RES) rv = st_ld4<IOS>(rb, ro + n0);
-      float o[4] = {acc[mt][nt][0] + bv.x + nz, acc[mt][nt][1] + bv.y + nz, acc[mt][nt][2] + bv.z + nz, acc[mt][nt][3] + bv.w + nz};
-      const float r4[4] = {rv.x, rv.y, rv.z, rv.w};
-#pragma unroll
-      for (int c = 0; c < 4; ++c) {
-        float t = o[c];
-        if (RES == 1) t += r4[c];
-        if (ACT == PPST_ACT_LRELU) t = (t > 0.f ? t : t * 0.2f) * 1.41421356237309515f;
-        else if (ACT == PPST_ACT_PRELU) t = t >= 0.f ? t : t * slope;
-        if (RES == 2) t += r4[c];
-        o[c] = t * a.out_scale;
-      }
-      st_st4<IOS>(yb, yo + n0, make_float4(o[0], o[1], o[2], o[3]));
-      s1[nt].x += o[0]; s1[nt].y += o[1]; s1[nt].z += o[2]; s1[nt].w += o[3];
-      s2[nt].x += o[0] * o[0]; s2[nt].y += o[1] * o[1]; s2[nt].z += o[2] * o[2]; s2[nt].w += o[3] * o[3];
-    }
-  }
-  };
-  {
-    const int resm = a.residual ? (res_after ? 2 : 1) : 0;
-#define EPI_GO(A_)                                                                                    \
-  do {                                                                                                \
-    if (resm == 0) epi_passes(EpiC<A_>{}, EpiC<0>{});                                                 \
-    else if (resm == 1) epi_passes(EpiC<A_>{}, EpiC<1>{});                                            \
-    else epi_passes(EpiC<A_>{}, EpiC<2>{});                                                           \
-  } while (0)
-    if (!SPEC) epi_passes(EpiR{act}, EpiR{resm});
-    else if (act == PPST_ACT_LRELU) EPI_GO(PPST_ACT_LRELU);
-    else if (act == PPST_ACT_PRELU) EPI_GO(PPST_ACT_PRELU);
-    else EPI_GO(PPST_ACT_NONE);
-#undef EPI_GO
-  }
-  if (a.stats) {
-#pragma unroll
-    for (int nt = 0; nt < NT; ++nt) {
-      float4 u = s1[nt], w = s2[nt];
-      float* uv[8] = {&u.x, &u.y, &u.z, &u.w, &w.x, &w.y, &w.z, &w.w};
-#pragma unroll
-      for (int q = 0; q < 8; ++q) {
-        float t = *uv[q];
-        t += __builtin_bit_cast(float, __builtin_amdgcn_mov_dpp(__builtin_bit_cast(int, t), 0xB1, 0xf, 0xf, true));
-        t += __builtin_bit_cast(float, __builtin_amdgcn_mov_dpp(__builtin_bit_cast(int, t), 0x4E, 0xf, 0xf, true));
-        t += __builtin_bit_cast(float, __builtin_amdgcn_mov_dpp(__builtin_bit_cast(int, t), 0x141, 0xf, 0xf, true));
-        t += __builtin_bit_cast(float, __builtin_amdgcn_mov_dpp(__builtin_bit_cast(int, t), 0x140, 0xf, 0xf, true));
-        *uv[q] = t;
-      }
-      if (r16 == 0) {
-        float* r = &red[wave][nt * 16 + g * 4][0];
-        r[0] = u.x; r[1] = w.x; r[2] = u.y; r[3] = w.y; r[4] = u.z; r[5] = w.z; r[6] = u.w; r[7] = w.w;
-      }
-    }
-    __syncthreads();
-    if (tid < (NT > 4 ? 128 : 64)) {
-      const int n = ntile * (NT > 4 ? 128 : 64) + tid;
-      if (n < a.cout) {
-        float t0 = 0.f, t1 = 0.f;
-#pragma unroll
-        for (int wv = 0; wv < 8; ++wv) { t0 += red[wv][tid][0]; t1 += red[wv][tid][1]; }
-        float* o = a.stats + (((int64_t)b * a.tiles + mblk) * a.cout + n) * 2;
-        o[0] = t0;
-        o[1] = t1;
-      }
-    }
-  }
-}
+#include "conv1x1_common.h"
+
 
 template <int INSS, bool TAPS = false, int NT_ = 4, int PREC = 0, int IOS = PPST_ST_F32>
 __global__ __launch_bounds__(512, 4) void conv1x1_stream_kernel(C1Args a) {
diff --git a/ppst_amd/csrc/conv1x1_common.h b/ppst_amd/csrc/conv1x1_common.h
--- /dev/null
+++ b/ppst_amd/csrc/conv1x1_common.h
@@ -0,0 +1,191 @@
+#pragma once
+#include "common.h"
+
+struct C1Args {
+  const float* x;
+  const unsigned char* wpack;
+  const int4* steps;
+  float* y;
+  const float* bias;
+  const float* noise;
+  const float* prelu;
+  float* stats;
+  const float* residual;
+  float noise_weight, out_scale;
+  int B, hw, in_ld, out_ld, cout, nsteps, act, res_ld, n_tiles, tiles;
+  int in_h, in_w, out_h, out_w, tiles_x, pad_mode;
+  const float* in_ss;
+  const float* in_prelu;
+  int in_c, in_act;
+  const float* in_res;
+  int in_res_ld;
+};
+
+#define C1_GROUP 8
+#define C1_BLOB 8192
+
+typedef _Float16 __attribute__((ext_vector_type(8))) c1_half8;
+template <int PREC>
+__device__ __forceinline__ void c1_cvt(float v, unsigned short& h, unsigned short& l) {
+  if (PREC == 0) split_bf16(v, h, l);
+  else if (PREC == 3) { h = __builtin_bit_cast(unsigned short, (_Float16)v); l = 0; }
+  else { h = f2bf(v); l = 0; }
+}
+template <int PREC>
+__device__ __forceinline__ void c1_cvt8(const float (&v)[8], bf16x8& hi, bf16x8& lo) {
+  if (PREC == 3) {
+#pragma unroll
+    for (int j = 0; j < 8; ++j) {
+      unsigned short h, l;
+      c1_cvt<PREC>(v[j], h, l);
+      hi[j] = (short)h;
+      lo[j] = (short)l;
+    }
+    return;
+  }
+  uint2 h0, l0 = make_uint2(0u, 0u), h1, l1 = make_uint2(0u, 0u);
+  if (PREC == 0) {
+    split_bf16x4(make_float4(v[0], v[1], v[2], v[3]), h0, l0);
+    split_bf16x4(make_float4(v[4], v[5], v[6], v[7]), h1, l1);
+  } else {
+    h0 = f2bf_x4(make_float4(v[0], v[1], v[2], v[3]));
+    h1 = f2bf_x4(make_float4(v[4], v[5], v[6], v[7]));
+  }
+  hi = __builtin_bit_cast(bf16x8, make_uint4(h0.x, h0.y, h1.x, h1.y));
+  lo = __builtin_bit_cast(bf16x8, make_uint4(l0.x, l0.y, l1.x, l1.y));
+}
+template <int IOS>
+__device__ __forceinline__ void c1_unpack8(float4 r, float (&v)[8]) {
+  const float4 a = st_unpack4<IOS>(make_uint2(__float_as_uint(r.x), __float_as_uint(r.y)));
+  const float4 b = st_unpack4<IOS>(make_uint2(__float_as_uint(r.z), __float_as_uint(r.w)));
+  v[0] = a.x; v[1] = a.y; v[2] = a.z; v[3] = a.w; v[4] = b.x; v[5] = b.y; v[6] = b.z; v[7] = b.w;
+}
+template <int PREC>
+__device__ __forceinline__ f32x4 c1_mfma(bf16x8 bh, bf16x8 bl, bf16x8 xh, bf16x8 xl, f32x4 acc) {
+  if (PREC == 0) {
+    acc = __builtin_amdgcn_mfma_f32_16x16x32_bf16(bh, xl, acc, 0, 0, 0);
+    acc = __builtin_amdgcn_mfma_f32_16x16x32_bf16(bl, xh, acc, 0, 0, 0);
+    return __builtin_amdgcn_mfma_f32_16x16x32_bf16(bh, xh, acc, 0, 0, 0);
+  }
+  if (PREC == 3) return __builtin_amdgcn_mfma_f32_16x16x32_f16(__builtin_bit_cast(c1_half8, bh), __builtin_bit_cast(c1_half8, xh), acc, 0, 0, 0);
+  return __builtin_amdgcn_mfma_f32_16x16x32_bf16(bh, xh, acc, 0, 0, 0);
+}
+
+__device__ __forceinline__ int c1_pad(int i, int n, int mode) {
+  if (mode == PPST_PAD_REFLECT) {
+    if (i < 0) i = -i;
+    if (i >= n) i = 2 * (n - 1) - i;
+  }
+  return i < 0 ? 0 : (i >= n ? n - 1 : i);
+}
+
+template <int MT, int NT, bool TAPS, bool SPEC = true, int IOS = PPST_ST_F32>
+__device__ __forceinline__ void c1_epilogue(const C1Args& a, f32x4 (&acc)[MT][NT], float (&red)[8][NT > 4 ? 128 : 64][2], int b, int mblk,
+                                            int ntile, int pbase, int oy0, int ox, int tid, int wave, int r16, int g) {
+  const int act = a.act & 0xff;
+  const bool res_after = (a.act >> 8) & 1;
+  const float slope = (act == PPST_ACT_PRELU && a.prelu) ? a.prelu[0] : 0.f;
+  float4 s1[NT], s2[NT];
+#pragma unroll
+  for (int nt = 0; nt < NT; ++nt) { s1[nt] = make_float4(0.f, 0.f, 0.f, 0.f); s2[nt] = s1[nt]; }
+  const int64_t img = (int64_t)b * (TAPS ? a.out_h * a.out_w : a.hw);
+  constexpr int ES = IOS == PPST_ST_F32 ? 4 : 2;
+  unsigned char* const yb = (unsigned char*)a.y + img * a.out_ld * ES;
+  const float* const nzb = a.noise ? a.noise + img : nullptr;
+  const unsigned char* const rb = a.residual ? (const unsigned char*)a.residual + img * a.res_ld * ES : nullptr;
+  const int nbase = ntile * (NT > 4 ? 128 : 64) + g * 4;
+  float nzv[MT];
+  float4 bva[NT];
+  const __amdgpu_buffer_rsrc_t nrs = __builtin_amdgcn_make_buffer_rsrc((void*)(nzb ? (const void*)nzb : (const void*)yb), 0,
+                                                                       nzb ? (TAPS ? a.out_h * a.out_w : a.hw) * 4 : 0, 0x00020000);
+#pragma unroll
+  for (int mt = 0; mt < MT; ++mt) {
+    const int p = pbase + mt * 16 + r16;
+    const bool ok = TAPS ? (oy0 + mt < a.out_h && ox < a.out_w) : p < a.hw;
+    nzv[mt] = a.noise_weight * __builtin_bit_cast(float, __builtin_amdgcn_raw_buffer_load_b32(
+                                   nrs, ok ? (TAPS ? (oy0 + mt) * a.out_w + ox : p) * 4 : (int)0x80000000, 0, 0));
+  }
+#pragma unroll
+  for (int nt = 0; nt < NT; ++nt)
+    bva[nt] = __builtin_bit_cast(float4, __builtin_amdgcn_raw_buffer_load_b128(__builtin_amdgcn_make_buffer_rsrc((void*)(a.bias ? (const void*)a.bias : (const void*)a.y), 0, a.bias ? a.cout * 4 : 0, 0x00020000), (nbase + nt * 16) * 4, 0, 0));
+  auto epi_passes = [&](auto act_c, auto res_c) {
+#pragma clang fp contract(off)
+    const int ACT = act_c.value, RES = res_c.value;
+#pragma unroll
+  for (int mt = 0; mt < MT; ++mt) {
+    const int p = pbase + mt * 16 + r16;
+    if (TAPS ? (oy0 + mt >= a.out_h || ox >= a.out_w) : p >= a.hw) continue;
+    const int pin = TAPS ? (oy0 + mt) * a.out_w + ox : p;
+    const int yo = pin * a.out_ld, ro = pin * a.res_ld;
+    const float nz = nzv[mt];
+#pragma unroll
+    for (int nt = 0; nt < NT; ++nt) {
+      const int n0 = nbase + nt * 16;
+      if (n0 >= a.cout) continue;
+      float4 rv = make_float4(0.f, 0.f, 0.f, 0.f);
+      const float4 bv = bva[nt];
+      if (RES) rv = st_ld4<IOS>(rb, ro + n0);
+      float o[4] = {acc[mt][nt][0] + bv.x + nz, acc[mt][nt][1] + bv.y + nz, acc[mt][nt][2] + bv.z + nz, acc[mt][nt][3] + bv.w + nz};
+      const float r4[4] = {rv.x, rv.y, rv.z, rv.w};
+#pragma unroll
+      for (int c = 0; c < 4; ++c) {
+        float t = o[c];
+        if (RES == 1) t += r4[c];
+        if (ACT == PPST_ACT_LRELU) t = (t > 0.f ? t : t * 0.2f) * 1.41421356237309515f;
+        else if (ACT == PPST_ACT_PRELU) t = t >= 0.f ? t : t * slope;
+        if (RES == 2) t += r4[c];
+        o[c] = t * a.out_scale;
+      }
+      st_st4<IOS>(yb, yo + n0, make_float4(o[0], o[1], o[2], o[3]));
+      s1[nt].x += o[0]; s1[nt].y += o[1]; s1[nt].z += o[2]; s1[nt].w += o[3];
+      s2[nt].x += o[0] * o[0]; s2[nt].y += o[1] * o[1]; s2[nt].z += o[2] * o[2]; s2[nt].w += o[3] * o[3];
+    }
+  }
+  };
+  {
+    const int resm = a.residual ? (res_after ? 2 : 1) : 0;
+#define EPI_GO(A_)                                                                                    \
+  do {                                                                                                \
+    if (resm == 0) epi_passes(EpiC<A_>{}, EpiC<0>{});                                                 \
+    else if (resm == 1) epi_passes(EpiC<A_>{}, EpiC<1>{});                                            \
+    else epi_passes(EpiC<A_>{}, EpiC<2>{});                                                           \
+  } while (0)
+    if (!SPEC) epi_passes(EpiR{act}, EpiR{resm});
+    else if (act == PPST_ACT_LRELU) EPI_GO(PPST_ACT_LRELU);
+    else if (act == PPST_ACT_PRELU) EPI_GO(PPST_ACT_PRELU);
+    else EPI_GO(PPST_ACT_NONE);
+#undef EPI_GO
+  }
+  if (a.stats) {
+#pragma unroll
+    for (int nt = 0; nt < NT; ++nt) {
+      float4 u = s1[nt], w = s2[nt];
+      float* uv[8] = {&u.x, &u.y, &u.z, &u.w, &w.x, &w.y, &w.z, &w.w};
+#pragma unroll
+      for (int q = 0; q < 8; ++q) {
+        float t = *uv[q];
+        t += __builtin_bit_cast(float, __builtin_amdgcn_mov_dpp(__builtin_bit_cast(int, t), 0xB1, 0xf, 0xf, true));
+        t += __builtin_bit_cast(float, __builtin_amdgcn_mov_dpp(__builtin_bit_cast(int, t), 0x4E, 0xf, 0xf, true));
+        t += __builtin_bit_cast(float, __builtin_amdgcn_mov_dpp(__builtin_bit_cast(int, t), 0x141, 0xf, 0xf, true));
+        t += __builtin_bit_cast(float, __builtin_amdgcn_mov_dpp(__builtin_bit_cast(int, t), 0x140, 0xf, 0xf, true));
+        *uv[q] = t;
+      }
+      if (r16 == 0) {
+        float* r = &red[wave][nt * 16 + g * 4][0];
+        r[0] = u.x; r[1] = w.x; r[2] = u.y; r[3] = w.y; r[4] = u.z; r[5] = w.z; r[6] = u.w; r[7] = w.w;
+      }
+    }
+    __syncthreads();
+    if (tid < (NT > 4 ? 128 : 64)) {
+      const int n = ntile * (NT > 4 ? 128 : 64) + tid;
+      if (n < a.cout) {
+        float t0 = 0.f, t1 = 0.f;
+#pragma unroll
+        for (int wv = 0; wv < 8; ++wv) { t0 += red[wv][tid][0]; t1 += red[wv][tid][1]; }
+        float* o = a.stats + (((int64_t)b * a.tiles + mblk) * a.cout + n) * 2;
+        o[0] = t0;
+        o[1] = t1;
+      }
+    }
+  }
+}
diff --git a/ppst_amd/csrc/conv_blur.hip b/ppst_amd/csrc/conv_blur.hip
--- /dev/null
+++ b/ppst_amd/csrc/conv_blur.hip
@@ -0,0 +1,193 @@
+#include "conv1x1_common.h"
+
+#define CB_TR 8
+#define CB_TC 16
+#define CB_BR (2 * CB_TR + 1)
+#define CB_BC (2 * CB_TC + 1)
+#define CB_M 17
+#define CB_PLANE (CB_BR * 2 * 4 * CB_M)
+#define CB_PY 4
+#define CB_PX 3
+#define CB_BANDS ((CB_BR + CB_PY - 1) / CB_PY)
+
+struct CBArgs {
+  C1Args c;
+  const float* taps;
+  int nchunks;
+};
+
+__device__ __forceinline__ int cb_reflect(int i, int n) {
+  if (i < 0) i = -i;
+  if (i >= n) i = 2 * (n - 1) - i;
+  return i < 0 ? 0 : (i >= n ? n - 1 : i);
+}
+__device__ __forceinline__ int cb_clamp(int i, int n) { return i < 0 ? 0 : (i >= n ? n - 1 : i); }
+
+template <bool INSS>
+__global__ __launch_bounds__(512) void conv_blur_kernel(CBArgs p) {
+  const C1Args& a = p.c;
+  constexpr int MT = 1, NT = 4;
+  __shared__ uint4 sW[9 * C1_BLOB / 16];
+  __shared__ uint4 sA[2 * CB_PLANE];
+  __shared__ float red[8][64][2];
+  const int tid = threadIdx.x, lane = tid & 63, wave = __builtin_amdgcn_readfirstlane(tid >> 6);
+  const int r16 = lane & 15, g = lane >> 4;
+  const int total = a.B * a.tiles * a.n_tiles;
+  const int per = (total + (int)gridDim.x - 1) / (int)gridDim.x;
+  const int w_beg = blockIdx.x * per, w_end = w_beg + per < total ? w_beg + per : total;
+  const bool keep_w = p.nchunks == 1 && a.n_tiles == 1;
+  const bool reflect = a.pad_mode == PPST_PAD_REFLECT;
+  const int q = tid & 7, strip = (tid >> 3) % 11, band = (tid >> 3) / 11;
+  const int by0 = band * CB_PY, bx0 = strip * CB_PX;
+  float kf[9];
+#pragma unroll
+  for (int i = 0; i < 9; ++i) kf[i] = p.taps[8 - i];
+
+  for (int wid = w_beg; wid < w_end; ++wid) {
+    const int ntile = wid % a.n_tiles;
+    int mblk = wid / a.n_tiles;
+    const int b = mblk / a.tiles;
+    mblk -= b * a.tiles;
+    const int tyi = mblk / a.tiles_x, txi = mblk - tyi * a.tiles_x;
+    const float* xb = a.x + (int64_t)b * a.in_h * a.in_w * a.in_ld;
+    if (wid > w_beg) __syncthreads();
+
+    f32x4 acc[MT][NT];
+#pragma unroll
+    for (int j = 0; j < NT; ++j) acc[0][j] = (f32x4){0.f, 0.f, 0.f, 0.f};
+
+    for (int c = 0; c < p.nchunks; ++c) {
+      if (c) __syncthreads();
+      if (!keep_w || wid == w_beg) {
+        const uint4* src = (const uint4*)(a.wpack + ((int64_t)ntile * a.nsteps + c * 9) * C1_BLOB);
+#pragma unroll
+        for (int i = 0; i < 9; ++i) sW[i * 512 + tid] = src[i * 512 + tid];
+      }
+      if (band < CB_BANDS) {
+        const int Y0 = tyi * (2 * CB_TR) + by0 - 2, X0 = txi * (2 * CB_TC) + bx0 - 2;
+        int coff[CB_PX + 2];
+        bool cok[CB_PX + 2];
+#pragma unroll
+        for (int j = 0; j < CB_PX + 2; ++j) {
+          const int ix = X0 + j;
+          cok[j] = reflect || (ix >= 0 && ix < a.in_w);
+          coff[j] = (reflect ? cb_reflect(ix, a.in_w) : cb_clamp(ix, a.in_w)) * a.in_ld;
+        }
+        float4 sa = make_float4(1.f, 1.f, 1.f, 1.f), sb = make_float4(0.f, 0.f, 0.f, 0.f);
+        if (INSS) {
+          const float4* qp = (const float4*)(a.in_ss + ((int64_t)b * a.in_c + c * 32 + q * 4) * 2);
+          const float4 q0 = qp[0], q1 = qp[1];
+          sa = make_float4(q0.x, q0.z, q1.x, q1.z); sb = make_float4(q0.y, q0.w, q1.y, q1.w);
+        }
+        float4 fa[CB_PY][CB_PX];
+#pragma unroll
+        for (int py = 0; py < CB_PY; ++py)
+#pragma unroll
+          for (int i = 0; i < CB_PX; ++i) fa[py][i] = make_float4(0.f, 0.f, 0.f, 0.f);
+#pragma unroll
+        for (int ry = 0; ry < CB_PY + 2; ++ry) {
+          const int iy = Y0 + ry;
+          const bool yok = reflect || (iy >= 0 && iy < a.in_h);
+          const float* row = xb + (int64_t)(reflect ? cb_reflect(iy, a.in_h) : cb_clamp(iy, a.in_h)) * a.in_w * a.in_ld + c * 32 + q * 4;
+#pragma unroll
+          for (int j = 0; j < CB_PX + 2; ++j) {
+            float4 v = *(const float4*)(row + coff[j]);
+            if (INSS) {
+              v.x = sa.x * v.x + sb.x; v.y = sa.y * v.y + sb.y; v.z = sa.z * v.z + sb.z; v.w = sa.w * v.w + sb.w;
+              if (a.in_act == PPST_ACT_LRELU) {
+                v.x = (v.x > 0.f ? v.x : v.x * 0.2f) * 1.41421356237309515f; v.y = (v.y > 0.f ? v.y : v.y * 0.2f) * 1.41421356237309515f;
+                v.z = (v.z > 0.f ? v.z : v.z * 0.2f) * 1.41421356237309515f; v.w = (v.w > 0.f ? v.w : v.w * 0.2f) * 1.41421356237309515f;
+              }
+            }
+            if (!(yok && cok[j])) v = make_float4(0.f, 0.f, 0.f, 0.f);
+#pragma unroll
+            for (int py = 0; py < CB_PY; ++py) {
+              const int ky = ry - py;
+              if (ky < 0 || ky > 2) continue;
+#pragma unroll
+              for (int i = 0; i < CB_PX; ++i) {
+                const int kx = j - i;
+                if (kx < 0 || kx > 2) continue;
+                const float f = kf[ky * 3 + kx];
+                fa[py][i].x += v.x * f; fa[py][i].y += v.y * f; fa[py][i].z += v.z * f; fa[py][i].w += v.w * f;
+              }
+            }
+          }
+        }
+        uint2* const sA2 = (uint2*)sA;
+#pragma unroll
+        for (int py = 0; py < CB_PY; ++py) {
+          const int by = by0 + py;
+          if (by >= CB_BR) continue;
+#pragma unroll
+          for (int i = 0; i < CB_PX; ++i) {
+            const int bx = bx0 + i;
+            uint2 hi, lo;
+            split_bf16x4(fa[py][i], hi, lo);
+            const int u = ((by * 2 + (bx & 1)) * 4 + (q >> 1)) * CB_M + (bx >> 1);
+            sA2[u * 2 + (q & 1)] = hi;
+            sA2[(CB_PLANE + u) * 2 + (q & 1)] = lo;
+          }
+        }
+      }
+      __syncthreads();
+#pragma unroll
+      for (int ky = 0; ky < 3; ++ky)
+#pragma unroll
+        for (int kx = 0; kx < 3; ++kx) {
+          const int u = (((2 * wave + ky) * 2 + (kx & 1)) * 4 + g) * CB_M + r16 + (kx >> 1);
+          const bf16x8 xh = __builtin_bit_cast(bf16x8, sA[u]), xl = __builtin_bit_cast(bf16x8, sA[CB_PLANE + u]);
+          const unsigned char* bs = (const unsigned char*)sW + (ky * 3 + kx) * C1_BLOB + g * 1024 + r16 * 16;
+#pragma unroll
+          for (int nt = 0; nt < NT; ++nt) {
+            const bf16x8 bh = *(const bf16x8*)(bs + nt * 256);
+            const bf16x8 bl = *(const bf16x8*)(bs + nt * 256 + 4096);
+            acc[0][nt] = c1_mfma<0>(bh, bl, xh, xl, acc[0][nt]);
+          }
+        }
+    }
+    c1_epilogue<MT, NT, true, true, PPST_ST_F32>(a, acc, red, b, mblk, ntile, 0, tyi * CB_TR + wave, txi * CB_TC + r16, tid, wave, r16, g);
+  }
+}
+
+extern "C" int ppst_conv_blur_tiles(int out_h, int out_w) { return cdiv(out_h, CB_TR) * cdiv(out_w, CB_TC); }
+
+extern "C" int ppst_conv_blur(const ppst_conv_args* a, const void* blur_k, void* stream) {
+  if (!a || !a->x || !a->wpack || !a->y || !blur_k) return PPST_ENULL;
+  if (a->precision != 0 || a->io_st != PPST_ST_F32) return PPST_EUNSUPPORTED;
+  const int act = a->act & 0xff;
+  if (a->B < 0 || a->in_h < 2 || a->in_w < 2 || a->nsteps <= 0 || a->nsteps % 9 || a->cout <= 0 || a->cout % 4 || a->bn != 64 ||
+      a->n_groups != 1 || (a->pad_mode != PPST_PAD_ZERO && a->pad_mode != PPST_PAD_REFLECT) ||
+      a->out_h != (a->in_h - 2) / 2 + 1 || a->out_w != (a->in_w - 2) / 2 + 1 || a->in_ld < (a->nsteps / 9) * 32 || a->in_ld % 4 ||
+      a->out_ld < a->cout || a->out_ld % 4 || (a->residual && (a->res_ld < a->cout || a->res_ld % 4)) ||
+      (act != PPST_ACT_NONE && act != PPST_ACT_LRELU && act != PPST_ACT_PRELU) || (act == PPST_ACT_PRELU && !a->prelu) ||
+      (a->in_act != PPST_ACT_NONE && a->in_act != PPST_ACT_LRELU) || (a->in_act != PPST_ACT_NONE && !a->in_scale_shift) ||
+      (a->in_scale_shift && a->in_c < (a->nsteps / 9) * 32) || a->in_res || a->ksplit > 1)
+    return PPST_EINVAL;
+  if ((((uintptr_t)a->x | (uintptr_t)a->y | (uintptr_t)a->residual | (uintptr_t)a->wpack | (uintptr_t)a->in_scale_shift | (uintptr_t)a->bias) % 16))
+    return PPST_EINVAL;
+  if ((int64_t)a->out_h * a->out_w * a->out_ld >= (1ll << 31) || (int64_t)a->out_h * a->out_w * a->res_ld >= (1ll << 31) ||
+      (int64_t)a->in_w * a->in_ld >= (1ll << 31))
+    return PPST_EINVAL;
+  if (a->B == 0) return PPST_OK;
+  CBArgs p;
+  C1Args& k = p.c;
+  k.x = (const float*)a->x; k.wpack = (const unsigned char*)a->wpack; k.steps = nullptr; k.y = (float*)a->y;
+  k.bias = (const float*)a->bias; k.noise = (const float*)a->noise; k.prelu = (const float*)a->prelu;
+  k.stats = (float*)a->stats; k.residual = (const float*)a->residual;
+  k.noise_weight = a->noise_weight; k.out_scale = a->out_scale;
+  k.B = a->B; k.hw = a->out_h * a->out_w; k.in_ld = a->in_ld; k.out_ld = a->out_ld; k.cout = a->cout; k.nsteps = a->nsteps;
+  k.act = a->act; k.res_ld = a->res_ld; k.n_tiles = cdiv(a->cout, 64);
+  k.tiles_x = cdiv(a->out_w, CB_TC); k.tiles = cdiv(a->out_h, CB_TR) * k.tiles_x;
+  k.in_h = a->in_h; k.in_w = a->in_w; k.out_h = a->out_h; k.out_w = a->out_w; k.pad_mode = a->pad_mode;
+  k.in_ss = (const float*)a->in_scale_shift; k.in_prelu = nullptr; k.in_c = a->in_c; k.in_act = a->in_act;
+  k.in_res = nullptr; k.in_res_ld = 0;
+  p.taps = (const float*)blur_k; p.nchunks = a->nsteps / 9;
+  int64_t blocks = (int64_t)a->B * k.tiles * k.n_tiles;
+  if (blocks > 0x7fffffff) return PPST_EINVAL;
+  if (blocks > 256) blocks = 256;
+  hipStream_t st = as_stream(stream);
+  if (k.in_ss) PPST_LAUNCH((conv_blur_kernel<true>), dim3((unsigned)blocks), dim3(512), 0, st, p);
+  else PPST_LAUNCH((conv_blur_kernel<false>), dim3((unsigned)blocks), dim3(512), 0, st, p);
+  return PPST_LAUNCH_CHECK();
+}
diff --git a/ppst_amd/networks/base_network.py b/ppst_amd/networks/base_network.py
--- a/ppst_amd/networks/base_network.py
+++ b/ppst_amd/networks/base_network.py
@@ -130,10 +130,15 @@
         pad_c = (ks - 2) + 2
         pad_s = (ks - 2) + 0
         xs, _ = ops.blur_nhwc(x, self.p(p + "skip.Blur.kernel"), (pad_s + 1) // 2, pad_s // 2, ops.PAD_ZERO, down=2)
+        fuse = ops.blur_conv_ok(w2, x, k, normed=bool(norm))
         if not norm:
             y1 = self.plan(p + "conv1.Conv.weight", scale=sc1)(x, bias=self.p(p + "conv1.Act.bias"), act=ops.ACT_LRELU,
                                                                 pad_mode=conv_pad)
             skip = self.plan(p + "skip.Conv.weight", scale=scs)(xs)
+            if fuse:
+                return ops.blur_conv(self.plan(p + "conv2.Conv.weight", "conv", sc1), y1, k, blur_pad_mode,
+                                     bias=self.p(p + "conv2.Act.bias"), act=ops.ACT_LRELU, residual=skip, res_after_act=True,
+                                     out_scale=INV_SQRT2)
             xb, bhw = ops.blur_nhwc(y1, k, (pad_c + 1) // 2, pad_c // 2, blur_pad_mode, s2d=True)
             ohw = ((bhw[0] - 3) // 2 + 1, (bhw[1] - 3) // 2 + 1)
             return self.plan(p + "conv2.Conv.weight", "s2d", sc1)(
@@ -142,9 +147,14 @@
         y1, st1 = self.plan(p + "conv1.Conv.weight", scale=sc1)(x, stats=True, pad_mode=conv_pad)
         ss1 = ops.in_finalize(st1, H * W, post_bias=self.p(p + "conv1.Act.bias"))
         ys, sts = self.plan(p + "skip.Conv.weight", scale=scs)(xs, stats=True)
-        xb, bhw = ops.blur_nhwc(y1, k, (pad_c + 1) // 2, pad_c // 2, blur_pad_mode, s2d=True, in_ss=ss1, in_act=ops.ACT_LRELU)
-        ohw = ((bhw[0] - 3) // 2 + 1, (bhw[1] - 3) // 2 + 1)
-        y2, st2 = self.plan(p + "conv2.Conv.weight", "s2d", sc1)(xb, stats=True, out_hw=ohw)
+        if fuse:
+            y2, st2 = ops.blur_conv(self.plan(p + "conv2.Conv.weight", "conv", sc1), y1, k, blur_pad_mode, stats=True,
+                                    in_ss=ss1, in_act=ops.ACT_LRELU)
+            ohw = tuple(y2.shape[1:3])
+        else:
+            xb, bhw = ops.blur_nhwc(y1, k, (pad_c + 1) // 2, pad_c // 2, blur_pad_mode, s2d=True, in_ss=ss1, in_act=ops.ACT_LRELU)
+            ohw = ((bhw[0] - 3) // 2 + 1, (bhw[1] - 3) // 2 + 1)
+            y2, st2 = self.plan(p + "conv2.Conv.weight", "s2d", sc1)(xb, stats=True, out_hw=ohw)
         cnt = ohw[0] * ohw[1]
         ss_s = ops.in_finalize(sts, cnt)
         ss2 = ops.in_finalize(st2, cnt, post_bias=self.p(p + "conv2.Act.bias"))
diff --git a/ppst_amd/ops.py b/ppst_amd/ops.py
--- a/ppst_amd/ops.py
+++ b/ppst_amd/ops.py
@@ -44,6 +44,9 @@
         BATCH_AWARE["value"] = self.prev
 WINO = {"value": True, "min_blocks": 16, "fill": 0, "ksplit_fill": 64}
 FUSE_TAIL = {"value": os.environ.get("PPST_FUSE_TAIL", "1") != "0", "torgb": os.environ.get("PPST_FUSE_TORGB", "0") == "1"}
+BLUR_CONV = {"value": os.environ.get("PPST_BLUR_CONV", "1") != "0",
+             "shapes": {(32, 64, False): True, (32, 64, True): False, (64, 128, False): False, (64, 128, True): False,
+                        (128, 256, False): False, (128, 256, True): False}}
 FAT_MIN_BLOCKS = 32
 
 
@@ -767,6 +770,48 @@
         return out
 
 
+def blur_conv_ok(weight, x, kernel, normed=False):
+    return bool(BLUR_CONV["value"] and PRECISION["value"] == 0 and x.dtype == torch.float32
+                and tuple(kernel.shape) == (3, 3) and tuple(weight.shape[2:]) == (3, 3)
+                and BLUR_CONV["shapes"].get((weight.shape[1], weight.shape[0], bool(normed)), False))
+
+
+def blur_conv(plan, x, kernel, pad_mode=PAD_ZERO, bias=None, act=ACT_NONE, stats=False, residual=None, res_after_act=False,
+              out_scale=1.0, in_ss=None, in_act=ACT_NONE):
+    if plan.kind != "conv" or plan.k != 3 or plan.precision != 0:
+        raise RuntimeError("blur_conv needs the plain 3x3 plan of the weight in precision mode 0")
+    ld = _nhwc_ld(x, "blur_conv input")
+    B, H, W, C = x.shape
+    if ld != C or C != plan.cin:
+        raise RuntimeError("blur_conv needs a dense (B, H, W, %d) tensor, got %s" % (plan.cin, tuple(x.shape)))
+    _chk(kernel, "kernel")
+    if tuple(kernel.shape) != (3, 3) or H < 2 or W < 2:
+        raise RuntimeError("blur_conv: 3 x 3 blur taps and an input of at least 2 x 2 pixels")
+    oh, ow = (H - 2) // 2 + 1, (W - 2) // 2 + 1
+    out = torch.empty((B, oh, ow, plan.cout), device=x.device, dtype=torch.float32)
+    if residual is not None and tuple(residual.shape) != tuple(out.shape):
+        raise RuntimeError("residual must match the output shape %s, got %s" % (tuple(out.shape), tuple(residual.shape)))
+    if in_ss is not None and (in_ss.dim() != 3 or in_ss.shape[0] != B or in_ss.shape[1] < C or in_ss.shape[2] != 2 or not in_ss.is_contiguous()):
+        raise RuntimeError("in_ss must be a contiguous (B=%d, >=%d, 2) table, got %s" % (B, C, tuple(in_ss.shape)))
+    for t, n in ((bias, "bias"), (in_ss, "in_ss")):
+        _chk(t, n)
+    st = torch.empty((B, lib.ppst_conv_blur_tiles(oh, ow), plan.cout, 2), device=x.device, dtype=torch.float32) if stats else None
+    a = _lib.ConvArgs()
+    a.x, a.wpack, a.y = _p(x), _p(plan.pack_for(64)), _p(out)
+    a.bias, a.stats, a.residual = _p(bias), _p(st), _p(residual)
+    a.res_ld = _nhwc_ld(residual, "residual") if residual is not None else 0
+    a.out_scale = float(out_scale)
+    a.B, a.in_h, a.in_w, a.in_ld = B, H, W, ld
+    a.out_h, a.out_w, a.out_ld, a.cout = oh, ow, plan.cout, plan.cout
+    a.nsteps, a.n_groups, a.pad_mode, a.bn = plan.nsteps, 1, pad_mode, 64
+    a.out_sy = a.out_sx = 1
+    a.act = act | (0x100 if res_after_act else 0)
+    a.in_scale_shift, a.in_act = _p(in_ss), in_act
+    a.in_c = in_ss.shape[1] if in_ss is not None else 0
+    check(lib.ppst_conv_blur(ctypes.byref(a), _p(kernel.contiguous()), _stream()), "ppst_conv_blur")
+    return (out, st) if stats else out
+
+
 class _KsWorkspace:
     __slots__ = ("scratch", "flags", "ptrs", "launches")
 
```
